# ginolhac/mapDamage

Hardware: AMD Instinct MI355X
Metric: reads/sec (misincorporation+comp tables) (higher is better)
Workload: dtype u8

## Files before the change

include/mdx.h:

```cpp
#ifndef MDX_H
#define MDX_H

#include <stdint.h>

#ifdef __cplusplus
extern "C" {
#endif

#define MDX_ABI_VERSION 6

#define MDX_OK 0
#define MDX_ERR_ARG (-1)
#define MDX_ERR_HIP (-2)
#define MDX_ERR_STATE (-3)
#define MDX_ERR_MASK_INDEX (-4)
#define MDX_ERR_LGD_OVERFLOW (-5)
#define MDX_ERR_BAD_READ (-6)

#define MDX_ERR_UNSUPPORTED (-8)
#define MDX_ERR_COMM (-7)

#define MDX_FLAG_QUAL_ABOVE_MIN 0x8000
#define MDX_FLAG_HAS_QUAL 0x4000

// ... 85 lines not shown
                           const int32_t *iv_start, const int32_t *iv_end, const int32_t *iv_group, int32_t rest_group);
int mdx_strata_groups(const mdx_ctx *ctx);
int mdx_strata_kept(mdx_ctx *ctx, uint64_t *kept);
int64_t mdx_merged_words(const mdx_ctx *ctx);
int mdx_finish_merged(mdx_ctx *ctx, const uint64_t *d_tables, uint64_t *d_merged);
int mdx_finish_merged_host(mdx_ctx *ctx, uint64_t *merged);
int mdx_lgd_copies(const mdx_ctx *ctx);

int mdx_reset(mdx_ctx *ctx);

int mdx_timing_enable(mdx_ctx *ctx, int enable);
int mdx_timing_read(mdx_ctx *ctx, int64_t *n_launches, double *total_ms);

int mdx_genome_composition(mdx_ctx *ctx, uint64_t *counts);

int mdx_rescale_set_model(mdx_ctx *ctx, const uint8_t *lut, const double *term, int32_t len5p, int32_t len3p);
int mdx_rescale_host(mdx_ctx *ctx, const mdx_batch *batch, const int32_t *mtid, const int32_t *mpos,
                     uint8_t *qual_out, double *mr_raw, uint8_t *status);
int mdx_rescale_device(mdx_ctx *ctx, const mdx_batch *dev_batch, const int32_t *d_mtid, const int32_t *d_mpos,
                       uint8_t *d_qual_out, double *d_mr_raw, uint8_t *d_status);
int mdx_tabulate_rescale_device(mdx_ctx *ctx, const mdx_batch *dev_batch, const int32_t *d_mtid, const int32_t *d_mpos,
                                uint8_t *d_qual_out, double *d_mr_raw, uint8_t *d_status);
int mdx_rescale_patches_device(mdx_ctx *ctx, const mdx_batch *dev_batch, const int32_t *d_mtid, const int32_t *d_mpos,
                               uint64_t *d_patch, int64_t patch_cap, int32_t n_parts, uint64_t *d_n_patch, double *d_mr_raw,
                               uint8_t *d_status);
int mdx_tabulate_rescale_patches_device(mdx_ctx *ctx, const mdx_batch *dev_batch, const int32_t *d_mtid, const int32_t *d_mpos,
                                        uint64_t *d_patch, int64_t patch_cap, int32_t n_parts, uint64_t *d_n_patch, double *d_mr_raw,
                                        uint8_t *d_status);
int mdx_rescale_expand_device(mdx_ctx *ctx, const mdx_batch *dev_batch, const uint64_t *d_patch, int64_t patch_cap, int32_t n_parts,
                              const uint64_t *d_n_patch, uint8_t *d_qual_out);
int mdx_rescale_timing_read(mdx_ctx *ctx, int64_t *n_launches, double *total_ms);
int64_t mdx_fused_launches(const mdx_ctx *ctx);
int64_t mdx_packed_launches(const mdx_ctx *ctx);
int64_t mdx_geo_spec_launches(const mdx_ctx *ctx);
int64_t mdx_libsorts(const mdx_ctx *ctx);
int mdx_last_launch_geometry(const mdx_ctx *ctx, int32_t out[4]);
int64_t mdx_rescale_summary_words(const mdx_ctx *ctx);
int mdx_rescale_summary(mdx_ctx *ctx, uint64_t *words);

typedef struct mdx_source mdx_source;
int mdx_source_open(const char *path, mdx_source **out);
const char *mdx_source_error(const mdx_source *source);
int mdx_source_is_stream(const mdx_source *source);
int mdx_source_peek(mdx_source *source, uint8_t *buf, int32_t n, int32_t *got);
int64_t mdx_source_read(mdx_source *source, uint8_t *buf, int64_t cap);
int mdx_source_seek(mdx_source *source, int64_t offset);
void mdx_source_close(mdx_source *source);

typedef struct mdx_bam mdx_bam;
int mdx_bam_read(const char *path, int threads, mdx_bam **out);
int mdx_bam_read_source(mdx_source *source, int threads, mdx_bam **out);
void mdx_bam_free(mdx_bam *bam);
const char *mdx_bam_error(const mdx_bam *bam);
const char *mdx_bam_header_text(const mdx_bam *bam);
int32_t mdx_bam_n_ref(const mdx_bam *bam);
const char *mdx_bam_ref_name(const mdx_bam *bam, int32_t i);
int64_t mdx_bam_ref_length(const mdx_bam *bam, int32_t i);
int mdx_bam_batch(const mdx_bam *bam, mdx_batch *view, const int32_t **mtid, const int32_t **mpos,
                  const int32_t **rg_index, const uint8_t **has_mr);
const uint8_t *mdx_bam_qmin(const mdx_bam *bam);

typedef struct mdx_record_filter {
    int32_t min_mapq;
    uint32_t require_flags, exclude_flags;
    int32_t min_length, max_length;
} mdx_record_filter;
// ... 99 lines not shown
```

mapdamage_amd/csrc/mdx_bamio.cpp:

```cpp
#include "../../include/mdx.h"
#ifndef MDX_HOST_ONLY
#include "mdx_internal.h"
#endif
#include "mdx_filter.h"
#include "mdx_crc32.h"

#include <fcntl.h>
#include <poll.h>
#include <sys/mman.h>
#include <sys/stat.h>
#include <unistd.h>
#include <zlib.h>

#include <algorithm>
#include <atomic>
#include <cerrno>
#include <chrono>
#include <condition_variable>
#include <functional>
#include <cstdlib>
#include <cstdio>
#include <cstring>
#include <mutex>
#include <string>
// ... 1363 lines not shown
    int pf_cur = -1;
    size_t pf_in0 = 0, pf_bytes = 0;
    void *d_crc_tables = nullptr;
    struct Buf { void *p = nullptr; size_t cap = 0; };
    struct Slab {
        bool ready = false;
        int64_t chunk_bytes = 0;
        size_t b0 = 0, b1 = 0, b2 = 0;
        size_t slab_bytes = 0, unc_bytes = 0, out0 = 0, in0 = 0, nh = 0, ahead = 0;
        size_t rec_cap = 0, cig_cap = 0, seq_cap = 0;
        bool more_file = false;
        std::vector<uint32_t> blk, crcs;
        int pf_used = -1;
        hipEvent_t ev_infl0 = nullptr, ev_infl = nullptr;
        double t_host = 0, frac_host = 0;
        bool timed = false;
        Buf comp, blk_d, crc, status, unc, cnt, pre, rec_off, flag, lib, tid, pos, tlen, mtid, mpos,
            cigar_off, cigar, seq_off, seq, qual, small, info, forced, arena;
    } slab[2];
    int cur = 0;
    int view_slab = 0;
    mdx_batch last_view{};
    const int32_t *last_mtid = nullptr, *last_mpos = nullptr;
    bool reserve(Buf &b, size_t bytes) {
        if (bytes <= b.cap) return true;
        if (b.p) (void)hipFree(b.p);
        b.p = nullptr; b.cap = 0;
        const size_t want = bytes + bytes / 8 + 256;
        if (hipMalloc(&b.p, want) != hipSuccess) { error = "out of device memory"; return false; }
        b.cap = want;
        return true;
    }
    bool drain() {
        bool ok = true;
        if (infl_stream) ok = hipStreamSynchronize(infl_stream) == hipSuccess && ok;
        if (copy_stream) ok = hipStreamSynchronize(copy_stream) == hipSuccess && ok;
        if (stream) ok = hipStreamSynchronize(stream) == hipSuccess && ok;
        return ok;
    }
};

int mdx_gbam_open_source(mdx_ctx *ctx, mdx_source *source, mdx_gbam **out) {
    try {
        if (!ctx || !source || !out) return MDX_ERR_ARG;
        mdx_gbam *g = new (std::nothrow) mdx_gbam();
        if (!g) return MDX_ERR_ARG;
        *out = g;
        g->ctx = ctx;
        void *st = nullptr;
        if (mdx_ctx_stream(ctx, &st, &g->device) != MDX_OK) { g->error = "no context"; return MDX_ERR_ARG; }
        g->stream = (hipStream_t)st;
        int rc = mdx_bam_open_source(source, 4, &g->hs);
        if (rc != MDX_OK) { g->error = g->hs ? g->hs->head.error : "cannot open"; return rc; }
        size_t k = 0;
        for (;;) {
            while (k < g->blocks.size() && g->blocks[k].out_off + g->blocks[k].out_size <= g->hs->header_bytes) k++;
            if (k < g->blocks.size() || g->whole_file_scanned()) break;
            if (!g->scan_to(g->scanned + ((size_t)1 << 20))) return MDX_ERR_ARG;
        }
        g->next_block = k;
        g->phase = k < g->blocks.size() ? g->hs->header_bytes - g->blocks[k].out_off : 0;
        g->host_share = g_host_share.load();
        if (const char *e = std::getenv("MDX_GBAM_HOST_SHARE")) {
            g->host_share = std::min(0.9, std::max(0.0, std::atof(e)));
            g->host_share_fixed = true;
        }
        if (const char *e = std::getenv("MDX_GBAM_NO_LOOKAHEAD")) g->no_ahead = *e && *e != '0';
// ... 38 lines not shown
            void *st = nullptr;
            (void)mdx_ctx_stream(ctx, &st, &g->device);
            g->stream = (hipStream_t)st;
            g->error = err;
            return MDX_ERR_ARG;
        }
        const int rc = mdx_gbam_open_source(ctx, file, out);
        mdx_source_close(file);
        return rc;
    } catch (const std::exception &e) {
        if (out && *out) (*out)->error = std::string("mdx_gbam_open: ") + e.what();
        return MDX_ERR_ARG;
    } catch (...) {
        return MDX_ERR_ARG;
    }
}

const mdx_bam *mdx_gbam_header(const mdx_gbam *g) { return (g && g->hs) ? &g->hs->head : nullptr; }
const char *mdx_gbam_error(const mdx_gbam *g) { return g ? g->error.c_str() : "null handle"; }

int mdx_gbam_configure(mdx_gbam *g, int32_t n_rg, const char *const *rg_ids, const int32_t *lib_of_rg, int32_t lib_default,
                       int want_qual, int want_mate) {
    try {
        if (!g || n_rg < 0 || (n_rg > 0 && (!rg_ids || !lib_of_rg))) return MDX_ERR_ARG;
        g->rg_names.clear(); g->rg_off.assign(1, 0); g->lib_of_rg.clear();
        for (int i = 0; i < n_rg; i++) {
            const size_t len = std::strlen(rg_ids[i]);
            g->rg_names.insert(g->rg_names.end(), (const uint8_t *)rg_ids[i], (const uint8_t *)rg_ids[i] + len);
            g->rg_off.push_back((uint32_t)g->rg_names.size());
            g->lib_of_rg.push_back(lib_of_rg[i]);
        }
        g->lib_default = lib_default;
        g->want_qual = want_qual != 0; g->want_mate = want_mate != 0;
        if (hipSetDevice(g->device) != hipSuccess) return MDX_ERR_HIP;
        g->d_rg_names = g->d_rg_off = g->d_lib_of_rg = nullptr;
        if (n_rg > 0) {
            const size_t b_off = g->rg_off.size() * 4, b_lib = g->lib_of_rg.size() * 4, b_nm = g->rg_names.size() + 1;
            const size_t need = b_off + b_lib + b_nm;
            if (g->d_rg && g->d_rg_cap < need) { rg_buffer_give(g->device, g->d_rg, g->d_rg_cap); g->d_rg = nullptr; g->d_rg_cap = 0; }
            if (!g->d_rg) g->d_rg = rg_buffer_take(g->device, need, g->d_rg_cap);
            if (!g->d_rg) { g->error = "out of device memory"; return MDX_ERR_HIP; }
            std::vector<uint8_t> img(need, 0);
            std::memcpy(img.data(), g->rg_off.data(), b_off);
            std::memcpy(img.data() + b_off, g->lib_of_rg.data(), b_lib);
            std::memcpy(img.data() + b_off + b_lib, g->rg_names.data(), g->rg_names.size());
            if (hipMemcpy(g->d_rg, img.data(), need, hipMemcpyHostToDevice) != hipSuccess) { g->error = "upload of the read-group tables failed"; return MDX_ERR_HIP; }
            g->d_rg_off = g->d_rg; g->d_lib_of_rg = (char *)g->d_rg + b_off; g->d_rg_names = (char *)g->d_rg + b_off + b_lib;
        }
        return MDX_OK;
    } catch (...) {
        return MDX_ERR_ARG;
    }
}

static size_t slab_want(const mdx_gbam *g, size_t b0, int64_t chunk_bytes) {
    size_t want = chunk_bytes < 65536 ? 65536 : (size_t)chunk_bytes;
    if (g->hs->file->is_stream()) return want;
    const size_t fsz = g->hs->file->size();
    const size_t in0 = b0 < g->blocks.size() ? (size_t)g->blocks[b0].in_off : g->scanned;
    if (fsz > in0) {
        const size_t rem = fsz - in0, n = (rem + want - 1) / want;
        if (n > 1) want = (rem + n - 1) / n;
        if (want < 65536) want = 65536;
    }
    return want;
}
static size_t slab_end_block(const mdx_gbam *g, size_t b0, size_t want, size_t *slab_bytes_out) {
// ... 419 lines not shown
    view->flag = c.flag; view->lib = c.lib; view->tid = c.tid; view->pos = c.pos; view->tlen = c.tlen;
    view->cigar_off = c.cigar_off; view->cigar = c.cigar; view->seq_off = c.seq_off; view->seq = c.seq; view->qual = c.qual;
    view->seq_format = c.fold ? MDX_SEQ_4BITQ : g->seq_format; view->reserved = 0; view->lowq = nullptr; view->libsort = nullptr;
    if (c.minqual > 0) {
        uint32_t counters[2] = {0, 0};
        if (hipMemcpyAsync(counters, d_counters, 8, hipMemcpyDeviceToHost, st) != hipSuccess || hipStreamSynchronize(st) != hipSuccess) return MDX_ERR_HIP;
        if (counters[0]) g->no_qual_seen = true;
        if (counters[1] == 0) { view->qual = nullptr; view->seq_format = g->seq_format; }
    }
    g->records_read += tot[0];
    if (d_mtid) *d_mtid = c.mtid;
    if (d_mpos) *d_mpos = c.mpos;
    g->last_view = *view; g->last_mtid = c.mtid; g->last_mpos = c.mpos;
    g->next_block = b1;
    g->phase = next_phase;
    g->phase_known = have;
    g->slabs_done++;
    g->view_reads = view->n_reads;
    s.ready = false;
    return MDX_OK;
}

int mdx_gbam_next(mdx_gbam *g, int64_t chunk_bytes, mdx_batch *view, const int32_t **d_mtid, const int32_t **d_mpos) {
    try {
        if (!g || !view) return MDX_ERR_ARG;
        std::memset(view, 0, sizeof(*view));
        if (d_mtid) *d_mtid = nullptr;
        if (d_mpos) *d_mpos = nullptr;
        if (!g->scan_to((g->next_block < g->blocks.size() ? g->blocks[g->next_block].in_off : g->scanned) + slab_want(g, g->next_block, chunk_bytes) + 65536)) return MDX_ERR_ARG;
        if (g->next_block >= g->blocks.size()) {
            if (g->phase_known && g->phase != 0) { g->error = "truncated BAM file: the last record is incomplete"; return MDX_ERR_ARG; }
            return MDX_OK;
        }
        if (hipSetDevice(g->device) != hipSuccess) return MDX_ERR_HIP;
        if (const char *fail = std::getenv("MDX_GBAM_FAIL_AT")) {
            if (g->slabs_done == std::atoi(fail)) { g->error = "MDX_GBAM_FAIL_AT"; return MDX_ERR_UNSUPPORTED; }
        }
        GbamLaps laps(g);
        GbamTrace tr;
        mdx_gbam::Slab &s = g->slab[g->cur], &n = g->slab[g->cur ^ 1];
        size_t ahead = (size_t)256 << 10;
        for (;;) {
            if (!(s.ready && s.b0 == g->next_block && s.chunk_bytes == chunk_bytes && s.ahead == ahead)) {
                const int rc = gbam_half_a(g, s, g->next_block, chunk_bytes, ahead, laps, tr);
                if (rc != MDX_OK) { (void)g->drain(); return rc; }
            }
            tr.mark("A");
            if (!g->no_ahead && !laps.on && s.b1 < g->blocks.size() && !(n.ready && n.b0 == s.b1 && n.chunk_bytes == chunk_bytes)) {
                const std::string keep = g->error;
                if (gbam_half_a(g, n, s.b1, chunk_bytes, (size_t)256 << 10, laps, tr) != MDX_OK) {
                    (void)g->drain();
                    n.ready = false; g->pf_cur = -1; g->error = keep;
                }
                tr.mark("A-next");
            }
            bool grow = false;
            const int rc = gbam_half_b(g, s, view, d_mtid, d_mpos, &grow, laps, tr);
            if (rc != MDX_OK) { (void)g->drain(); s.ready = n.ready = false; return rc; }
            if (!grow) break;
            if (!g->drain()) return MDX_ERR_HIP;
            s.ready = false;
            ahead *= 8;
        }
        g->view_slab = g->cur;
        g->cur ^= 1;
        mdx_source *src = g->hs->file;
        int64_t keep = 0, ph = 0;
// ... 81 lines not shown
            if (g->slab[0].ready || g->slab[1].ready) {
                (void)hipSetDevice(g->device);
                if (!g->drain()) return MDX_ERR_HIP;
                g->slab[0].ready = g->slab[1].ready = false;
            }
        }
        const size_t want = slab_want(g, g->next_block, chunk_bytes);
        if (!g->scan_to((g->next_block < g->blocks.size() ? g->blocks[g->next_block].in_off : g->scanned) + want + 65536)) return MDX_ERR_ARG;
        if (g->next_block >= g->blocks.size()) return MDX_OK;
        if (g->phase_known && !g->next_verified) {
            g->error = "the first record behind BGZF block " + std::to_string(g->next_block) + " cannot be found without the slab in front of it";
            return MDX_ERR_UNSUPPORTED;
        }
        const size_t b0 = g->next_block, in0 = g->blocks[b0].in_off;
        size_t b1 = b0, unc_bytes = 0;
        while (b1 < g->blocks.size() && (b1 == b0 || (g->blocks[b1].in_off - in0 < want && unc_bytes + g->blocks[b1].out_size < 0xE0000000ull))) {
            unc_bytes += g->blocks[b1].out_size;
            b1++;
        }
        g->next_block = b1;
        g->phase_known = false;
        g->phase = 0;
        return MDX_OK;
    } catch (...) {
        return MDX_ERR_ARG;
    }
}

int mdx_gbam_fixups(const mdx_gbam *g) { return g ? g->fixups : 0; }

int mdx_gbam_view_flags(mdx_gbam *g, uint16_t *flags, int64_t n) {
    if (!g || n < 0 || n != g->view_reads || (n > 0 && !flags)) return MDX_ERR_ARG;
    if (n == 0) return MDX_OK;
    if (hipSetDevice(g->device) != hipSuccess) return MDX_ERR_HIP;
    if (hipMemcpyAsync(flags, g->slab[g->view_slab].flag.p, (size_t)n * 2, hipMemcpyDeviceToHost, g->stream) != hipSuccess ||
        hipStreamSynchronize(g->stream) != hipSuccess) { g->error = "copy of the flag column failed"; return MDX_ERR_HIP; }
    return MDX_OK;
}

int mdx_gbam_view_set_flags(mdx_gbam *g, const uint16_t *flags, int64_t n) {
    if (!g || n < 0 || n != g->view_reads || (n > 0 && !flags)) return MDX_ERR_ARG;
    if (n == 0) return MDX_OK;
    if (hipSetDevice(g->device) != hipSuccess) return MDX_ERR_HIP;
    if (hipMemcpyAsync(g->slab[g->view_slab].flag.p, flags, (size_t)n * 2, hipMemcpyHostToDevice, g->stream) != hipSuccess ||
        hipStreamSynchronize(g->stream) != hipSuccess) { g->error = "copy of the flag column failed"; return MDX_ERR_HIP; }
    return MDX_OK;
}

int mdx_gbam_tell(const mdx_gbam *g, int64_t *comp_off, int64_t *phase) {
    if (!g || !comp_off || !phase || !g->hs) return MDX_ERR_ARG;
    if (!g->phase_known) return MDX_ERR_STATE;
    const size_t k = g->next_block;
    *comp_off = k >= g->blocks.size() ? (int64_t)g->scanned : (k == 0 ? 0 : (int64_t)(g->blocks[k - 1].in_off + g->blocks[k - 1].in_size + 8));
    *phase = (int64_t)g->phase;
    return MDX_OK;
}

int mdx_gbam_set_seq_format(mdx_gbam *g, int32_t seq_format) {
    if (!g || (seq_format != MDX_SEQ_ASCII && seq_format != MDX_SEQ_4BIT)) return MDX_ERR_ARG;
    g->seq_format = seq_format;
    return MDX_OK;
}

int mdx_gbam_missing_qualities(const mdx_gbam *g) { return (g && g->no_qual_seen) ? 1 : 0; }

int mdx_gbam_set_record_filter(mdx_gbam *g, const mdx_record_filter *filter) {
    if (!g) return MDX_ERR_ARG;
    if (!mdx_record_filter_valid(filter)) { g->error = "mdx_gbam_set_record_filter: a value out of range (MAPQ 0..255, flags 0..65535, lengths >= 0, min <= max)"; return MDX_ERR_ARG; }
    if (g->slabs_done > 0 || g->records_read > 0) { g->error = "mdx_gbam_set_record_filter: behind the first mdx_gbam_next"; return MDX_ERR_STATE; }
    const bool on = mdx_record_filter_active(filter);
    if (on && !g->d_filter_counts) {
        if (hipSetDevice(g->device) != hipSuccess || hipMalloc((void **)&g->d_filter_counts, 5 * sizeof(unsigned long long)) != hipSuccess ||
            hipMemset(g->d_filter_counts, 0, 5 * sizeof(unsigned long long)) != hipSuccess) {
            g->error = "mdx_gbam_set_record_filter: no device memory for the counts";
            return MDX_ERR_HIP;
        }
    }
    g->filter_on = on;
    g->filter = on ? *filter : mdx_record_filter{};
    return MDX_OK;
}

int mdx_gbam_filter_counts(const mdx_gbam *g, uint64_t out[6]) {
    if (!g || !out) return MDX_ERR_ARG;
    unsigned long long dropped[5] = {0, 0, 0, 0, 0};
    if (g->d_filter_counts) {
        if (hipSetDevice(g->device) != hipSuccess || hipStreamSynchronize(g->stream) != hipSuccess ||
            hipMemcpy(dropped, g->d_filter_counts, sizeof(dropped), hipMemcpyDeviceToHost) != hipSuccess) return MDX_ERR_HIP;
    }
    out[0] = g->records_read;
    for (int k = 0; k < 5; k++) out[1 + k] = dropped[k];
    return MDX_OK;
}

int mdx_gbam_at_end(const mdx_gbam *g) { return (!g || (g->next_block >= g->blocks.size() && g->whole_file_scanned())) ? 1 : 0; }

void mdx_gbam_close(mdx_gbam *g) {
    if (!g) return;
    const bool timing = std::getenv("MDX_BAM_TIMING") != nullptr;
    auto t_last = std::chrono::steady_clock::now();
    auto lap = [&](const char *what) {
        if (!timing) return;
        const auto now = std::chrono::steady_clock::now();
        std::fprintf(stderr, "mdx_gbam_close %-11s %.2f ms\n", what, std::chrono::duration<double, std::milli>(now - t_last).count());
        t_last = now;
    };
    (void)hipSetDevice(g->device);
    (void)g->drain();
    lap("sync");
    host_buffer_give(g->hbuf, g->hbuf_cap);
    for (auto &sl : g->slab) {
        if (sl.ev_infl0) (void)hipEventDestroy(sl.ev_infl0);
        if (sl.ev_infl) (void)hipEventDestroy(sl.ev_infl);
    }
    if (g->ev_free) (void)hipEventDestroy(g->ev_free);
    if (g->infl_stream) (void)hipStreamDestroy(g->infl_stream);
    pin_give(g->pin_bad);
    {
        const int big = g->slab[1].arena.cap > g->slab[0].arena.cap ? 1 : 0;
        mdx_ctx_scratch_give(g->ctx, g->slab[big].arena.p, g->slab[big].arena.cap, g->d_crc_tables, g->copy_stream, nullptr);
// ... 72 lines not shown
            }
            if (rc != MDX_OK) break;
            if (written + (int64_t)at > out_cap) { rc = MDX_ERR_ARG; break; }
            if (!ok(hipMemcpyAsync(B.d_off, offs.data(), (size_t)nb * 8, hipMemcpyHostToDevice, st))) break;
            mdx_k_bgzf_gather(src, bytes, B.d_slots, B.d_sizes, B.d_off, nb, B.d_tab, B.d_out, st);
            if (!ok(hipGetLastError()) || !ok(hipMemcpyAsync(out + written, B.d_out, (size_t)at, hipMemcpyDeviceToHost, st)) ||
                !ok(hipStreamSynchronize(st))) break;
            written += (int64_t)at;
        }
        if (rc == MDX_OK) *out_len = written;
    } catch (...) {
        rc = MDX_ERR_ARG;
    }
    return rc;
}

int mdx_bgzf_deflate(mdx_ctx *ctx, const uint8_t *data, int64_t n, uint8_t *out, int64_t out_cap, int64_t *out_len) {
    if (!ctx || n < 0 || (n > 0 && !data) || !out || !out_len) return MDX_ERR_ARG;
    void *st_ = nullptr;
    int device = 0;
    if (mdx_ctx_stream(ctx, &st_, &device) != MDX_OK) return MDX_ERR_ARG;
    return bgzf_deflate_impl((hipStream_t)st_, device, data, nullptr, n, out, out_cap, out_len);
}

int mdx_gbam_write_rescaled(mdx_gbam *g, const uint64_t *d_patch, int64_t patch_cap, int32_t n_parts, const uint64_t *d_n_patch,
                            const float *mr, const uint8_t *rescaled, uint8_t *out, int64_t out_cap, int64_t *out_len, int64_t *mr_clash) {
    if (!g || !out || !out_len || patch_cap < 0 || (n_parts > 0 && (!d_patch || !d_n_patch))) return MDX_ERR_ARG;
    *out_len = 0;
    if (mr_clash) *mr_clash = -1;
    const int64_t n = g->view_reads;
    if (n == 0) return MDX_OK;
    if (!mr || !rescaled) return MDX_ERR_ARG;
    try {
        if (hipSetDevice(g->device) != hipSuccess) return MDX_ERR_HIP;
        hipStream_t st = g->stream;
        mdx_gbam::Slab &s = g->slab[g->view_slab];
        uint8_t *d_resc = nullptr, *d_stream = nullptr;
        float *d_mr = nullptr;
        uint32_t *d_sizes = nullptr;
        unsigned long long *d_off = nullptr;
        int *d_clash = nullptr;
        int rc = MDX_OK;
        auto ok = [&](hipError_t e) { if (e != hipSuccess) { rc = MDX_ERR_HIP; g->error = std::string("write_rescaled: ") + hipGetErrorString(e); (void)hipGetLastError(); } return e == hipSuccess; };
        std::vector<uint32_t> sizes((size_t)n);
        std::vector<unsigned long long> offs((size_t)n);
        const int no_clash = 0x7FFFFFFF;
        int clash = no_clash;
        if (ok(hipMalloc((void **)&d_resc, (size_t)n)) && ok(hipMalloc((void **)&d_mr, (size_t)n * 4)) && ok(hipMalloc((void **)&d_sizes, (size_t)n * 4)) &&
            ok(hipMalloc((void **)&d_off, (size_t)n * 8)) && ok(hipMalloc((void **)&d_clash, 4)) &&
            ok(hipMemcpyAsync(d_resc, rescaled, (size_t)n, hipMemcpyHostToDevice, st)) && ok(hipMemcpyAsync(d_mr, mr, (size_t)n * 4, hipMemcpyHostToDevice, st)) &&
            ok(hipMemcpyAsync(d_clash, &no_clash, 4, hipMemcpyHostToDevice, st))) {
            if (n_parts > 0)
                mdx_k_gbam_patch_qual((uint8_t *)s.unc.p, (const uint32_t *)s.rec_off.p, (const uint32_t *)s.seq_off.p, (uint32_t)n,
                                      (const unsigned long long *)d_patch, (const unsigned long long *)d_n_patch, patch_cap, n_parts, st);
            mdx_k_gbam_out_sizes((const uint8_t *)s.unc.p, (const uint32_t *)s.rec_off.p, d_resc, (uint32_t)n, d_sizes, st);
            if (ok(hipGetLastError()) && ok(hipMemcpyAsync(sizes.data(), d_sizes, (size_t)n * 4, hipMemcpyDeviceToHost, st)) && ok(hipStreamSynchronize(st))) {
                unsigned long long total = 0;
                for (int64_t i = 0; i < n; i++) { offs[(size_t)i] = total; total += sizes[(size_t)i]; }
                if (ok(hipMalloc((void **)&d_stream, (size_t)total + 64)) && ok(hipMemcpyAsync(d_off, offs.data(), (size_t)n * 8, hipMemcpyHostToDevice, st))) {
                    mdx_k_gbam_write_back((const uint8_t *)s.unc.p, (const uint32_t *)s.rec_off.p, d_off, d_resc, d_mr, (uint32_t)n, d_stream, d_clash, st);
                    if (ok(hipGetLastError()) && ok(hipMemcpyAsync(&clash, d_clash, 4, hipMemcpyDeviceToHost, st)) && ok(hipStreamSynchronize(st))) {
                        if (clash != no_clash) {
                            if (mr_clash) *mr_clash = clash;
                            g->error = "record " + std::to_string(clash) + " of the slab is to be rescaled and has an MR tag already";
                            rc = MDX_ERR_BAD_READ;
                        } else {
                            rc = bgzf_deflate_impl(st, g->device, nullptr, d_stream, (int64_t)total, out, out_cap, out_len);
                            if (rc != MDX_OK) g->error = "the BGZF writer failed (output buffer too small?)";
                        }
                    }
                }
            }
        }
        for (void *p : {(void *)d_resc, (void *)d_mr, (void *)d_sizes, (void *)d_off, (void *)d_clash, (void *)d_stream}) if (p) (void)hipFree(p);
        return rc;
    } catch (const std::exception &e) {
        g->error = std::string("mdx_gbam_write_rescaled: ") + e.what();
        return MDX_ERR_ARG;
    }
}

int mdx_gbam_record_name(mdx_gbam *g, int64_t index, char *buf, int32_t cap) {
    if (!g || !buf || cap < 1 || index < 0 || index >= g->view_reads) return MDX_ERR_ARG;
    buf[0] = 0;
    if (hipSetDevice(g->device) != hipSuccess) return MDX_ERR_HIP;
    mdx_gbam::Slab &s = g->slab[g->view_slab];
    uint32_t off = 0;
    uint8_t head[12];
    if (hipMemcpy(&off, (const uint32_t *)s.rec_off.p + index, 4, hipMemcpyDeviceToHost) != hipSuccess ||
        hipMemcpy(head, (const uint8_t *)s.unc.p + off, 12, hipMemcpyDeviceToHost) != hipSuccess) return MDX_ERR_HIP;
    const int len = std::min<int>(head[8], cap - 1);
    if (len > 0 && hipMemcpy(buf, (const uint8_t *)s.unc.p + off + 32, (size_t)len, hipMemcpyDeviceToHost) != hipSuccess) return MDX_ERR_HIP;
    buf[len] = 0;
    return MDX_OK;
}

int mdx_gbam_rescale_slab(mdx_gbam *g, uint8_t *out, int64_t out_cap, int64_t *out_len, int64_t *counts, int64_t *mr_clash) {
    if (!g || !out || !out_len) return MDX_ERR_ARG;
    *out_len = 0;
    if (mr_clash) *mr_clash = -1;
    const int64_t n = g->view_reads;
    if (n == 0) return MDX_OK;
    const mdx_batch &v = g->last_view;
    if (!v.qual || !g->last_mtid || !g->last_mpos || v.seq_format != MDX_SEQ_ASCII) {
        g->error = "mdx_gbam_rescale_slab: the handle must be configured with qualities and mate columns, the seq column ASCII";
        return MDX_ERR_STATE;
    }
    try {
        if (hipSetDevice(g->device) != hipSuccess) return MDX_ERR_HIP;
        hipStream_t st = g->stream;
        const int parts = 256;
        const int64_t cap = std::max<int64_t>(4096, 8 * n / parts);
        uint64_t *d_patch = nullptr, *d_count = nullptr;
        double *d_mr = nullptr;
        uint8_t *d_status = nullptr;
        int rc = MDX_OK;
        auto ok = [&](hipError_t e) { if (e != hipSuccess) { rc = MDX_ERR_HIP; g->error = std::string("rescale_slab: ") + hipGetErrorString(e); (void)hipGetLastError(); } return e == hipSuccess; };
        std::vector<double> mr_raw((size_t)n);
        std::vector<uint8_t> status((size_t)n), rescaled((size_t)n);
        std::vector<float> mr((size_t)n);
        std::vector<uint64_t> cnt((size_t)parts);
        if (ok(hipMalloc((void **)&d_count, (size_t)parts * 8)) && ok(hipMalloc((void **)&d_mr, (size_t)n * 8)) && ok(hipMalloc((void **)&d_status, (size_t)n))) {
            if (ok(hipMalloc((void **)&d_patch, (size_t)parts * (size_t)cap * 8))) {
                rc = mdx_rescale_patches_device(g->ctx, &v, g->last_mtid, g->last_mpos, d_patch, cap, parts, d_count, d_mr, d_status);
                if (rc != MDX_OK) g->error = std::string("rescale kernels: ") + mdx_last_error(g->ctx);
                else if (ok(hipMemcpyAsync(cnt.data(), d_count, (size_t)parts * 8, hipMemcpyDeviceToHost, st)) && ok(hipStreamSynchronize(st))) {
                    uint64_t fullest = 0;
                    for (uint64_t c_ : cnt) fullest = std::max(fullest, c_);
                    if ((int64_t)fullest > cap) { g->error = "rescale_slab: more rescaled bytes than the list holds"; rc = MDX_ERR_ARG; }
                }
            }
        }
        if (rc == MDX_OK) {
            int64_t bad = -1;
            rc = mdx_sync(g->ctx, &bad);
            if (rc != MDX_OK) { g->error = std::string("rescale kernels: ") + mdx_last_error(g->ctx); if (mr_clash && rc == MDX_ERR_BAD_READ) *mr_clash = -2 - bad; }
        }
        if (rc == MDX_OK && ok(hipMemcpyAsync(mr_raw.data(), d_mr, (size_t)n * 8, hipMemcpyDeviceToHost, st)) &&
            ok(hipMemcpyAsync(status.data(), d_status, (size_t)n, hipMemcpyDeviceToHost, st)) && ok(hipStreamSynchronize(st))) {
            for (int64_t i = 0; i < n; i++) {
                const uint8_t stv = status[(size_t)i];
                rescaled[(size_t)i] = (stv == 2 || stv == 3) ? 1 : 0;
// ... 56 lines not shown
```

mapdamage_amd/csrc/mdx_capi.cpp:

```cpp
#include "../../include/mdx.h"
#include "mdx_internal.h"

#include <dlfcn.h>

#include <chrono>

#include <cstdio>
#include <cstdlib>
#include <cstring>
#include <mutex>
#include <new>
#include <string>
#include <thread>
#include <utility>
#include <vector>

namespace {

constexpr size_t kLdsLimit = MDX_LDS_LIMIT;
#ifdef MDX_WAVE_CLK
static unsigned long long *g_dbg_clk = nullptr;
extern "C" int mdx_dbg_clk_read(unsigned long long *out, int n) {
    if (!g_dbg_clk) return -1;
    (void)hipDeviceSynchronize();
    return (int)hipMemcpy(out, g_dbg_clk, (size_t)n * 24, hipMemcpyDeviceToHost);
}
extern "C" int mdx_dbg_phase_read(unsigned long long *out, int reset) {
    if (!g_dbg_clk) return -1;
    (void)hipDeviceSynchronize();
    std::vector<unsigned long long> h((size_t)16 * 8192);
    int rc = (int)hipMemcpy(h.data(), g_dbg_clk + 3 * 20000, h.size() * 8, hipMemcpyDeviceToHost);
    for (int q = 0; q < 16; q++) out[q] = 0;
    for (size_t w = 0; w < 8192; w++) for (int q = 0; q < 16; q++) out[q] += h[16 * w + q];
    if (reset) rc |= (int)hipMemset(g_dbg_clk + 3 * 20000, 0, h.size() * 8);
    return rc;
}
#endif
// ... 99 lines not shown
    MdxPkConfig pk = {512, 0};
    bool tile_ctr_clean = false;
    bool pkm_prepared = false;
    DevBuf lowq;
    DevBuf libsort;
    DevBuf libsort_scratch;
    const void *libsort_checked = nullptr;
    uint64_t libsort_checked_sig = 0;
    DevBuf ml_partials;
    int n_groups = 0;
    int32_t *d_group_of_tid = nullptr;
    unsigned long long *d_strata_kept = nullptr;
    int strata_n_contig = 0;
    void *d_regions = nullptr;
    MdxRegions regions = {};
    DevBuf strata_key;
    bool counted = false;
    int lgd_copies = MDX_LGD_COPIES;
    int64_t n_libsorts = 0;
    int64_t n_fused = 0;
    int64_t n_packed = 0;
    int64_t n_geo_spec = 0;
    int64_t fuse_list_cap = 0;
    int32_t last_geom[4] = {0, 0, 0, 0};
    void *pin[2] = {nullptr, nullptr};
    hipEvent_t pin_done[2] = {nullptr, nullptr};
    bool pin_busy[2] = {false, false};
    uint8_t *d_lut = nullptr;
    double *d_term = nullptr;
    unsigned long long *d_subs = nullptr;
    std::vector<uint8_t> h_lut;
    bool key0_plain = false;
    int len5p = 0, len3p = 0;
    bool timing = false;
    std::vector<std::pair<hipEvent_t, hipEvent_t>> events;
    std::vector<std::pair<hipEvent_t, hipEvent_t>> rs_events;
    std::string err;
};

namespace {

int fail(mdx_ctx *c, int code, const std::string &msg) {
    if (c) c->err = msg;
    return code;
}

#define RCCL_TRY(ctx, r, call)                                                                  \
    do {                                                                                        \
        int e_ = (call);                                                                        \
        if (e_ != 0)                                                                            \
            return fail((ctx), MDX_ERR_COMM, std::string(#call) + ": " + (r)->GetErrorString(e_)); \
    } while (0)

#define HIP_TRY(ctx, call)                                                                     \
    do {                                                                                       \
        hipError_t e_ = (call);                                                                \
        if (e_ != hipSuccess)                                                                  \
            return fail((ctx), MDX_ERR_HIP, std::string(#call) + ": " + hipGetErrorString(e_)); \
    } while (0)

int64_t lgd_words(const mdx_ctx *c) { return (int64_t)c->cfg.nlib * 4 * c->cfg.lgd_max; }
int64_t mis_words(const mdx_ctx *c) { return (int64_t)c->cfg.nlib * 4 * c->cfg.length * MDX_N_MIS_COLS; }
int64_t comp_words(const mdx_ctx *c) { return (int64_t)c->cfg.nlib * 4 * (c->cfg.length + c->cfg.around) * 4; }

int zero_accumulators(mdx_ctx *c) {
    HIP_TRY(c, hipMemsetAsync(c->d_raw, 0, (size_t)c->dims.w_total * 8, c->stream));
    HIP_TRY(c, hipMemsetAsync(c->d_lgd_dense, 0, (size_t)lgd_words(c) * 8 * c->lgd_copies, c->stream));
    HIP_TRY(c, hipMemsetAsync(c->d_n_lgd_over, 0, 8, c->stream));
    HIP_TRY(c, hipMemsetAsync(c->d_err, 0xFF, 8, c->stream));
    if (c->d_strata_kept) HIP_TRY(c, hipMemsetAsync(c->d_strata_kept, 0, (size_t)c->cfg.nlib * 8, c->stream));
    return MDX_OK;
}

}

extern "C" {

int mdx_abi_version(void) { return MDX_ABI_VERSION; }

int mdx_pack_seq(const uint8_t *ascii, int64_t n_bases, uint8_t *packed, int32_t threads) {
    if (n_bases < 0 || (n_bases > 0 && (!ascii || !packed))) return MDX_ERR_ARG;
    uint8_t lut[256];
    std::memset(lut, 0, sizeof lut);
    lut['A'] = 1; lut['C'] = 2; lut['T'] = 4; lut['G'] = 8;
    const int64_t nb = (n_bases + 1) / 2;
    int nt = threads > 0 ? threads : (int)std::thread::hardware_concurrency();
    if (nt < 1) nt = 1;
    if (nb < (int64_t)1 << 20) nt = 1;
    auto work = [&](int64_t lo, int64_t hi) {
        for (int64_t i = lo; i < hi; i++) {
            const uint8_t a = lut[ascii[2 * i]], b = 2 * i + 1 < n_bases ? lut[ascii[2 * i + 1]] : 0;
            packed[i] = (uint8_t)(a | (b << 4));
        }
    };
    if (nt == 1) { work(0, nb); return MDX_OK; }
    std::vector<std::thread> pool;
    for (int t = 0; t < nt; t++) pool.emplace_back(work, nb * t / nt, nb * (t + 1) / nt);
    for (auto &th : pool) th.join();
    return MDX_OK;
}

const char *mdx_strerror(int code) {
    switch (code) {
// ... 15 lines not shown
    if (cfg->length < 1 || cfg->around < 0 || cfg->minqual < 0 || cfg->minqual > 93 || cfg->nlib < 1 ||
        cfg->lgd_max < 1 || cfg->lgd_over_cap < 0)
        return MDX_ERR_ARG;
    mdx_ctx *c = new (std::nothrow) mdx_ctx();
    if (!c) return MDX_ERR_ARG;
    c->cfg = *cfg;
    const bool trace = getenv("MDX_INIT_TRACE") != nullptr;
    auto t_last = std::chrono::steady_clock::now();
    auto lap = [&](const char *what) {
        if (!trace) return;
        const auto now = std::chrono::steady_clock::now();
        std::fprintf(stderr, "mdx_create %-14s %.1f ms\n", what, std::chrono::duration<double, std::milli>(now - t_last).count());
        t_last = now;
    };
    int ndev = 0;
    if (hipGetDeviceCount(&ndev) != hipSuccess || ndev <= 0 || cfg->device < 0 || cfg->device >= ndev) {
        delete c;
        return MDX_ERR_HIP;
    }
    *out = c;
    if (cfg->nlib > 65535)
        return fail(c, MDX_ERR_ARG, "more than 65535 tables (libraries x reference groups): the 16-bit library column names "
                                    "no more, 0xFFFF being the record without a library");
    HIP_TRY(c, hipSetDevice(cfg->device));
    hipDeviceProp_t prop;
    HIP_TRY(c, hipGetDeviceProperties(&prop, cfg->device));
    c->n_cu = prop.multiProcessorCount > 0 ? prop.multiProcessorCount : 256;
    if (const char *e = getenv("MDX_TEST_CUS")) {
        const int n = atoi(e);
        if (n >= 1 && n < c->n_cu) c->n_cu = n;
    }
    HIP_TRY(c, hipStreamCreateWithFlags(&c->own_stream, hipStreamNonBlocking));
    c->stream = c->own_stream;
    lap("context, stream");

    const int lgd_lds = mdx_k_lgd_lds(cfg->length, cfg->around, cfg->lgd_max);
    if ((int64_t)cfg->nlib * (4LL * cfg->length * 29 + 8LL * (2LL * cfg->around + 512) +
                              4LL * lgd_lds + 128) > 0x7FFFFFF0LL || cfg->length > (1 << 24) || cfg->around > (1 << 24))
        return fail(c, MDX_ERR_ARG, "table too large (nlib * length)");
    c->dims = mdx_make_dims(cfg->length, cfg->around, cfg->nlib, cfg->lgd_max, lgd_lds);
    int group = cfg->nlib;
    while (group > 1 && mdx_k_lds_bytes(mdx_make_dims(cfg->length, cfg->around, group, cfg->lgd_max, lgd_lds)) > kLdsLimit)
        group--;
    const MdxDims gdims = mdx_make_dims(cfg->length, cfg->around, group, cfg->lgd_max, lgd_lds);
    c->lds_bytes = mdx_k_lds_bytes(gdims);
    if (c->lds_bytes <= kLdsLimit) {
        c->mode = MDX_MODE_LDS;
        c->lib_group = group;
        c->max_grid = c->n_cu * (2048 / mdx_k_block_threads());
        HIP_TRY(c, mdx_k_prepare(c->lds_bytes));
        {
            const MdxDims d1 = mdx_make_dims(cfg->length, cfg->around, 1, cfg->lgd_max, lgd_lds);
            c->pk = mdx_k_pk_config(d1, kLdsLimit);
            HIP_TRY(c, mdx_k_prepare_packed(mdx_k_pk_lds_bytes(d1, c->pk)));
            if (const char *e = getenv("MDX_DEBUG_PK")) if (*e && *e != '0')
                fprintf(stderr, "[mdx] packed kernels: blocks of %d threads, %zu bytes of LDS, columns %s\n", c->pk.threads, mdx_k_pk_lds_bytes(d1, c->pk),
                        c->pk.pfl ? "prefetched into the LDS" : "by plain loads");
        }
        lap("kernels");
        HIP_TRY(c, hipMalloc((void **)&c->d_partials, (size_t)c->max_grid * gdims.w_total * 4));
    } else {
        c->mode = MDX_MODE_GLOBAL;
        c->max_grid = c->n_cu * (2048 / mdx_k_block_threads());
    }
    HIP_TRY(c, hipMalloc((void **)&c->d_raw, (size_t)c->dims.w_total * 8));
    c->lgd_copies = mdx_lgd_copies_for(cfg->nlib, cfg->lgd_max);
    HIP_TRY(c, hipMalloc((void **)&c->d_lgd_dense, (size_t)lgd_words(c) * 8 * c->lgd_copies));
    HIP_TRY(c, hipMalloc((void **)&c->d_lgd_over, (size_t)(cfg->lgd_over_cap > 0 ? cfg->lgd_over_cap : 1) * 32));
    HIP_TRY(c, hipMalloc((void **)&c->d_n_lgd_over, 8));
    HIP_TRY(c, hipMalloc((void **)&c->d_err, 8));
    int rc = zero_accumulators(c);
    if (rc != MDX_OK) return rc;
    HIP_TRY(c, hipStreamSynchronize(c->stream));
    lap("accumulators");
    return MDX_OK;
}

void mdx_destroy(mdx_ctx *c) {
    if (!c) return;
    (void)hipSetDevice(c->cfg.device);
    if (c->stream) (void)hipStreamSynchronize(c->stream);
    if (c->comm && c->comm_owned && rccl()) (void)rccl()->CommDestroy(c->comm);
    for (auto &ev : c->events) { (void)hipEventDestroy(ev.first); (void)hipEventDestroy(ev.second); }
    for (auto &ev : c->rs_events) { (void)hipEventDestroy(ev.first); (void)hipEventDestroy(ev.second); }
    for (auto &set : c->st) for (auto &b : set) b.release();
    for (int i = 0; i < 2; i++) {
        if (c->st_copied[i]) (void)hipEventDestroy(c->st_copied[i]);
        if (c->st_done[i]) (void)hipEventDestroy(c->st_done[i]);
    }
    if (c->copy_stream) (void)hipStreamDestroy(c->copy_stream);
    if (c->gbam_arena) (void)hipFree(c->gbam_arena);
    if (c->gbam_tables) (void)hipFree(c->gbam_tables);
    if (c->gbam_stream) (void)hipStreamDestroy((hipStream_t)c->gbam_stream);
    if (c->gbam_event) (void)hipEventDestroy((hipEvent_t)c->gbam_event);
    c->lists.release();
    c->unpacked.release();
    c->lowq.release();
    c->libsort.release();
    c->libsort_scratch.release();
    c->strata_key.release();
    c->ml_partials.release();
    c->rs_part.release();
    c->rs_lists.release();
    c->rs_in.release();
    for (int i = 0; i < 2; i++) {
        if (c->pin[i]) (void)hipHostFree(c->pin[i]);
        if (c->pin_done[i]) (void)hipEventDestroy(c->pin_done[i]);
    }
    void *ptrs[] = {c->d_ref, c->d_ref4, c->d_contig_off, c->d_raw, c->d_lgd_dense, c->d_lgd_over,
                    c->d_n_lgd_over, c->d_err, c->d_partials, c->d_lut, c->d_term, c->d_subs, c->d_tile_ctr, c->d_group_of_tid, c->d_regions, c->d_strata_kept};
    for (void *p : ptrs) if (p) (void)hipFree(p);
    if (c->own_stream) (void)hipStreamDestroy(c->own_stream);
    delete c;
}

const char *mdx_last_error(const mdx_ctx *c) { return c ? c->err.c_str() : "null context"; }

int mdx_set_stream(mdx_ctx *c, void *hip_stream) {
    if (!c) return MDX_ERR_ARG;
    HIP_TRY(c, hipStreamSynchronize(c->stream));
    c->stream = hip_stream ? (hipStream_t)hip_stream : c->own_stream;
    return MDX_OK;
}

static const size_t kRefPad = 256;
static int ref_begin(mdx_ctx *c, int64_t n, int32_t n_contig) {
    HIP_TRY(c, hipSetDevice(c->cfg.device));
    HIP_TRY(c, hipStreamSynchronize(c->stream));
    if (c->d_ref) { (void)hipFree(c->d_ref); c->d_ref = nullptr; }
    if (c->d_ref4) { (void)hipFree(c->d_ref4); c->d_ref4 = nullptr; }
    if (c->d_contig_off) { (void)hipFree(c->d_contig_off); c->d_contig_off = nullptr; }
    c->n_contig = 0; c->ref_len = 0;
    HIP_TRY(c, hipMalloc((void **)&c->d_ref, (size_t)n + 2 * kRefPad + 1));
    HIP_TRY(c, hipMalloc((void **)&c->d_contig_off, (size_t)(n_contig + 1) * 8));
    HIP_TRY(c, hipMemsetAsync(c->d_ref, 0x85, (size_t)n + 2 * kRefPad + 1, c->stream));
    return MDX_OK;
}
static int ref_finish(mdx_ctx *c, const int64_t *contig_off, int32_t n_contig, int64_t n) {
    const size_t n4 = ((size_t)n + 2 * kRefPad + 1) / 2;
    static const bool no_ref2 = [] { const char *e = getenv("MDX_NO_REF2"); return e && *e && *e != '0'; }();
    const size_t kCopyB = ((size_t)1 << 31) + 64;
    static const size_t ref2_min = [] { const char *e = getenv("MDX_REF2_MIN"); return e && *e ? (size_t)strtoull(e, nullptr, 10) : (size_t)64 << 20; }();
    c->ref2 = n4 >= ref2_min && n4 + 128 <= ((size_t)1 << 31) - 64 && !no_ref2;
    hipError_t e = hipMemcpyAsync(c->d_contig_off, contig_off, (size_t)(n_contig + 1) * 8, hipMemcpyHostToDevice, c->stream);
    if (e == hipSuccess) {
        e = hipMalloc((void **)&c->d_ref4, (c->ref2 ? kCopyB : 0) + n4 + 64);
        if (e != hipSuccess && c->ref2) { (void)hipGetLastError(); c->ref2 = false; e = hipMalloc((void **)&c->d_ref4, n4 + 64); }
    }
    if (e == hipSuccess) e = hipMemsetAsync(c->d_ref4, 0, n4 + 64, c->stream);
    if (e == hipSuccess) { mdx_k_encode_ref4(c->d_ref, c->d_ref4, (int64_t)(2 * n4), c->stream); e = hipGetLastError(); }
    if (e == hipSuccess && c->ref2) e = hipMemcpyAsync(c->d_ref4 + kCopyB, c->d_ref4, n4 + 64, hipMemcpyDeviceToDevice, c->stream);
    if (e == hipSuccess) e = hipStreamSynchronize(c->stream);
    if (e != hipSuccess) {
        (void)hipFree(c->d_ref); c->d_ref = nullptr;
        return fail(c, MDX_ERR_HIP, std::string("set_reference: ") + hipGetErrorString(e));
    }
    c->n_contig = n_contig;
    c->ref_len = n;
    return MDX_OK;
}

int mdx_set_reference(mdx_ctx *c, const uint8_t *bases, const int64_t *contig_off, int32_t n_contig) {
    if (!c || !contig_off || n_contig < 1) return fail(c, MDX_ERR_ARG, "set_reference: bad arguments");
    for (int i = 0; i < n_contig; i++)
        if (contig_off[i + 1] < contig_off[i]) return fail(c, MDX_ERR_ARG, "contig_off not monotone");
    const int64_t n = contig_off[n_contig];
    if (contig_off[0] != 0 || (n > 0 && !bases)) return fail(c, MDX_ERR_ARG, "set_reference: bad arguments");
    int rc = ref_begin(c, n, n_contig);
    if (rc != MDX_OK) return rc;
    uint8_t *tmp = nullptr;
    HIP_TRY(c, hipMalloc((void **)&tmp, (size_t)n + 1));
    hipError_t e = n > 0 ? hipMemcpyAsync(tmp, bases, (size_t)n, hipMemcpyHostToDevice, c->stream) : hipSuccess;
    if (e == hipSuccess) { mdx_k_encode_ref(tmp, c->d_ref + kRefPad, n, c->stream); e = hipGetLastError(); }
    rc = e == hipSuccess ? ref_finish(c, contig_off, n_contig, n) : fail(c, MDX_ERR_HIP, std::string("set_reference: ") + hipGetErrorString(e));
    (void)hipStreamSynchronize(c->stream);
    (void)hipFree(tmp);
    return rc;
}

int mdx_set_reference_fasta(mdx_ctx *c, const char *fasta_path, int32_t n_contig, const char *const *names, int32_t missing_ok,
                            int64_t *lengths) {
    if (!c || !fasta_path || !names || n_contig < 1) return fail(c, MDX_ERR_ARG, "set_reference_fasta: bad arguments");
    try {
        HIP_TRY(c, hipSetDevice(c->cfg.device));
        struct Arg { mdx_ctx *c; int32_t n_contig; int rc; } arg{c, n_contig, MDX_OK};
        std::vector<int64_t> contig_off;
        std::string err;
        const int rc = mdx_fasta_to_device(fasta_path, n_contig, names, missing_ok, lengths, contig_off, err, c->stream,
            [](void *a_, int64_t n) -> uint8_t * {
                Arg *a = (Arg *)a_;
                a->rc = ref_begin(a->c, n, a->n_contig);
                return a->rc == MDX_OK ? a->c->d_ref + kRefPad : nullptr;
            }, &arg);
        if (arg.rc != MDX_OK) return arg.rc;
        if (rc != MDX_OK) {
            if (c->d_ref) { (void)hipFree(c->d_ref); c->d_ref = nullptr; }
            return fail(c, rc, "set_reference_fasta: " + err);
        }
        return ref_finish(c, contig_off.data(), n_contig, contig_off[(size_t)n_contig]);
    } catch (const std::exception &e) {
        return fail(c, MDX_ERR_ARG, std::string("set_reference_fasta: ") + e.what());
    }
}

int mdx_reference_fetch(mdx_ctx *c, int32_t tid, int64_t start, int64_t end, uint8_t *out) {
    if (!c || !out) return MDX_ERR_ARG;
    if (!c->d_ref) return fail(c, MDX_ERR_STATE, "mdx_set_reference has not been called");
    if (tid < 0 || tid >= c->n_contig || start < 0 || end < start) return fail(c, MDX_ERR_ARG, "reference_fetch: bad range");
    HIP_TRY(c, hipSetDevice(c->cfg.device));
    int64_t off[2];
    HIP_TRY(c, hipMemcpy(off, c->d_contig_off + tid, 16, hipMemcpyDeviceToHost));
    if (start + off[0] > off[1] || end + off[0] > off[1]) return fail(c, MDX_ERR_ARG, "reference_fetch: beyond the contig's end");
    if (end > start) HIP_TRY(c, hipMemcpy(out, c->d_ref + kRefPad + off[0] + start, (size_t)(end - start), hipMemcpyDeviceToHost));
    for (int64_t i = 0; i < end - start; i++) if (out[i] & 0x80) out[i] = out[i] == 0x84 ? '-' : 'N';
    return MDX_OK;
}

// ... 33 lines not shown
}
static int strata_view(mdx_ctx *c, const mdx_batch *b, mdx_batch *out, bool count) {
    *out = *b;
    if (c->n_groups <= 0 || b->n_reads == 0) return MDX_OK;
    HIP_TRY(c, c->strata_key.reserve((size_t)b->n_reads * 2 + 64));
    if (c->d_regions)
        mdx_k_strata_region_key(b->n_reads, b->flag, b->lib, b->tid, b->pos, b->cigar_off, b->cigar, b->n_cigar, c->regions, c->n_groups,
                                c->cfg.nlib / c->n_groups, (uint16_t *)c->strata_key.p, count ? c->d_strata_kept : nullptr, c->stream);
    else
        mdx_k_strata_key(b->n_reads, b->flag, b->lib, b->tid, c->d_group_of_tid, c->strata_n_contig, c->n_groups, c->cfg.nlib / c->n_groups,
                         (uint16_t *)c->strata_key.p, count ? c->d_strata_kept : nullptr, c->stream);
    HIP_TRY(c, hipGetLastError());
    out->lib = (const uint16_t *)c->strata_key.p;
    return MDX_OK;
}

static int build_libsort(mdx_ctx *c, const mdx_batch *b, void *blob) {
    MdxLibSort ls;
    mdx_k_libsort_layout(blob, b->n_reads, b->n_cigar, b->n_bases, c->cfg.nlib, &ls);
    const uint64_t sig = libsort_signature(b->n_reads, b->n_cigar, b->n_bases, c->cfg.nlib, c->n_groups);
    HIP_TRY(c, hipMemcpyAsync((char *)blob + 8, &sig, 8, hipMemcpyHostToDevice, c->stream));
    HIP_TRY(c, c->libsort_scratch.reserve(mdx_k_libsort_scratch_bytes(b->n_reads, c->cfg.nlib)));
    mdx_k_libsort(b->n_reads, b->n_cigar, b->n_bases, b->flag, b->lib, b->tid, b->pos, b->tlen, b->cigar_off, b->cigar, b->seq_off, b->seq,
                  c->cfg.nlib, c->libsort_scratch.p, ls, c->stream);
    HIP_TRY(c, hipGetLastError());
    return MDX_OK;
}

int mdx_batch_upload(mdx_ctx *c, const mdx_batch *h, mdx_batch *dv) {
    int rc = check_batch(c, h);
    if (rc != MDX_OK) return rc;
    if (!dv) return MDX_ERR_ARG;
    HIP_TRY(c, hipSetDevice(c->cfg.device));
    std::memset(dv, 0, sizeof(*dv));
    dv->n_reads = h->n_reads; dv->n_cigar = h->n_cigar; dv->n_bases = h->n_bases;
    dv->seq_format = h->seq_format;
    const int64_t n = h->n_reads;
    struct Col { const void *src; const void **dst; size_t bytes; } cols[] = {
        {h->flag, (const void **)&dv->flag, (size_t)n * 2},
        {h->lib, (const void **)&dv->lib, (size_t)n * 2},
        {h->tid, (const void **)&dv->tid, (size_t)n * 4},
        {h->pos, (const void **)&dv->pos, (size_t)n * 4},
        {h->tlen, (const void **)&dv->tlen, (size_t)n * 4},
        {h->cigar_off, (const void **)&dv->cigar_off, (size_t)(n + 1) * 4},
        {h->cigar, (const void **)&dv->cigar, (size_t)h->n_cigar * 4},
        {h->seq_off, (const void **)&dv->seq_off, (size_t)(n + 1) * 4},
        {h->seq, (const void **)&dv->seq, seq_bytes(h)},
        {h->qual, (const void **)&dv->qual, h->qual ? (size_t)h->n_bases : 0},
    };
    for (auto &col : cols) {
        if (!col.src || n == 0) continue;
        void *p = nullptr;
        HIP_TRY(c, hipMalloc(&p, col.bytes + 64));
        *col.dst = p;
        HIP_TRY(c, hipMemcpyAsync(p, col.src, col.bytes, hipMemcpyHostToDevice, c->stream));
    }
    if (dv->qual && n > 0) {
        mdx_k_mark_has_qual(const_cast<uint16_t *>(dv->flag), dv->seq_off, dv->qual, n, c->stream);
        HIP_TRY(c, hipGetLastError());
    }
    static const bool no_batch_lowq = [] { const char *e = getenv("MDX_NO_BATCH_LOWQ"); return e && *e && *e != '0'; }();
    if (c->cfg.minqual > 0 && dv->qual && h->seq_format == MDX_SEQ_4BIT && h->n_bases > 0 && c->mode == MDX_MODE_LDS && !no_batch_lowq) {
        mdx_k_fold_mask(dv->seq, const_cast<uint8_t *>(dv->seq), dv->qual, nullptr, h->n_bases, c->cfg.minqual, c->stream);
        HIP_TRY(c, hipGetLastError());
        dv->seq_format = MDX_SEQ_4BITQ;
    }
    static const bool no_batch_sort = [] { const char *e = getenv("MDX_NO_BATCH_LIBSORT"); return e && *e && *e != '0'; }();
    if (c->cfg.nlib > 1 && h->seq_format != MDX_SEQ_ASCII && n > 0 && c->mode == MDX_MODE_LDS && !no_batch_sort) {
        void *p = nullptr;
        HIP_TRY(c, hipMalloc(&p, mdx_k_libsort_bytes(n, h->n_cigar, h->n_bases, c->cfg.nlib)));
        dv->libsort = (const uint8_t *)p;
        mdx_batch keyed;
        rc = strata_view(c, dv, &keyed, false);
        if (rc != MDX_OK) return rc;
        rc = build_libsort(c, &keyed, p);
        if (rc != MDX_OK) return rc;
    }
    HIP_TRY(c, hipStreamSynchronize(c->stream));
    return MDX_OK;
}

int mdx_batch_fold(mdx_ctx *c, mdx_batch *b) {
    int rc = check_batch(c, b);
    if (rc != MDX_OK) return rc;
    if (c->cfg.minqual <= 0) return fail(c, MDX_ERR_STATE, "mdx_batch_fold: the context has no --min-basequal");
    if (b->seq_format == MDX_SEQ_4BITQ) return MDX_OK;
    if (b->seq_format != MDX_SEQ_4BIT) return fail(c, MDX_ERR_ARG, "mdx_batch_fold: the seq column is not MDX_SEQ_4BIT");
    if (!b->qual && !b->lowq) return fail(c, MDX_ERR_ARG, "mdx_batch_fold: neither qualities nor a bitmap of the low ones");
    if (b->libsort) return fail(c, MDX_ERR_ARG, "mdx_batch_fold: the batch brings mdx_batch::libsort, built from the column as it was");
    if (b->n_bases == 0) { b->seq_format = MDX_SEQ_4BITQ; return MDX_OK; }
    HIP_TRY(c, hipSetDevice(c->cfg.device));
    mdx_k_fold_mask(b->seq, const_cast<uint8_t *>(b->seq), b->qual, b->lowq, b->n_bases, c->cfg.minqual, c->stream);
    HIP_TRY(c, hipGetLastError());
    b->seq_format = MDX_SEQ_4BITQ;
    return MDX_OK;
}

int mdx_batch_free(mdx_ctx *c, mdx_batch *dv) {
    if (!c || !dv) return MDX_ERR_ARG;
    HIP_TRY(c, hipStreamSynchronize(c->stream));
    if (dv->libsort && dv->libsort == c->libsort_checked) c->libsort_checked = nullptr;
    const void *ptrs[] = {dv->flag, dv->lib, dv->tid, dv->pos, dv->tlen, dv->cigar_off,
                          dv->cigar, dv->seq_off, dv->seq, dv->qual, dv->lowq, dv->libsort};
    for (const void *p : ptrs) if (p) (void)hipFree(const_cast<void *>(p));
    std::memset(dv, 0, sizeof(*dv));
    return MDX_OK;
}

static int tabulate_impl(mdx_ctx *c, const mdx_batch *b_in, const MdxFuse *fuse, int *fused_grid) {
    int rc = check_batch(c, b_in);
    if (rc != MDX_OK) return rc;
    if (!c->d_ref) return fail(c, MDX_ERR_STATE, "mdx_set_reference has not been called");
    if (b_in->n_reads == 0) return MDX_OK;
    HIP_TRY(c, hipSetDevice(c->cfg.device));
    const bool force_ref64 = [] { const char *e = getenv("MDX_FORCE_REF64"); return e && *e && *e != '0'; }();
    const bool ref32 = c->ref_len + 1024 < (int64_t)0xFFFFFFFFLL && !force_ref64;
    static const bool no_packed = [] { const char *e = getenv("MDX_NO_PACKED"); return e && *e && *e != '0'; }();
    static const bool no_pkm = [] { const char *e = getenv("MDX_NO_PACKED_MASK"); return e && *e && *e != '0'; }();
    const bool folded = b_in->seq_format == MDX_SEQ_4BITQ;
    const bool want_mask = c->cfg.minqual > 0 && (b_in->qual != nullptr || folded);
    const bool packed = b_in->seq_format != MDX_SEQ_ASCII && c->mode == MDX_MODE_LDS && c->dims.fast_ok() && ref32 &&
                        (fuse ? (c->cfg.nlib == 1 && !folded) : !(want_mask && no_pkm)) && !no_packed;
    const bool pmask = packed && !fuse && want_mask;
    static const bool no_ml = [] { const char *e = getenv("MDX_NO_ML"); return e && *e && *e != '0'; }();
    const bool ml = packed && !fuse && c->cfg.nlib > 1 && !no_ml;
    mdx_batch b_key;
    if (c->n_groups > 0) {
        if (fuse) return fail(c, MDX_ERR_ARG, "the fused tabulate-and-rescale calls count one library: not on a context with mdx_set_strata");
        if (c->strata_n_contig != c->n_contig)
            return fail(c, MDX_ERR_ARG, std::string(c->d_regions ? "mdx_set_strata_regions" : "mdx_set_strata") + " named " + std::to_string(c->strata_n_contig) + " sequences, the reference has " +
                                        std::to_string(c->n_contig));
        if (!(ml && b_in->libsort)) {
            rc = strata_view(c, b_in, &b_key, true);
            if (rc != MDX_OK) return rc;
            b_in = &b_key;
        }
    }
    c->counted = true;
    mdx_batch b_ascii;
    const mdx_batch *b = b_in;
    if (!packed) {
        rc = ascii_view(c, b_in, &b_ascii);
        if (rc != MDX_OK) return rc;
        b = &b_ascii;
    }
    MdxTabArgs a{};
    a.ref4 = c->d_ref4;
    a.ref2 = c->ref2 ? 1 : 0;
    a.seq_packed = packed ? 1 : 0;
    a.n_reads = b->n_reads;
    a.flag = b->flag; a.lib = b->lib; a.tid = b->tid; a.pos = b->pos; a.tlen = b->tlen;
    a.cigar_off = b->cigar_off; a.cigar = b->cigar; a.seq_off = b->seq_off; a.seq = b->seq; a.qual = b->qual;
    a.ref = c->d_ref + 256;
    a.contig_off = c->d_contig_off;
    a.n_contig = c->n_contig;
    a.minqual = c->cfg.minqual;
    a.dims = c->dims;
    a.partials = c->d_partials;
// ... 1 lines not shown
    a.lgd_dense = c->d_lgd_dense;
    a.lgd_copies = c->lgd_copies;
    a.lgd_over = c->d_lgd_over;
    a.lgd_over_cap = c->cfg.lgd_over_cap;
    a.n_lgd_over = c->d_n_lgd_over;
    a.err = c->d_err;
    a.record_base = c->record_base;
#ifdef MDX_WAVE_CLK
    if (!g_dbg_clk) {
        (void)hipMalloc((void **)&g_dbg_clk, 3 * 8 * 20000 + 16 * 8 * 8192);
        (void)hipMemset(g_dbg_clk, 0, 3 * 8 * 20000 + 16 * 8 * 8192);
    }
    a.dbg_clk = g_dbg_clk;
#endif
    a.stage_off = mdx_k_stage_off(c->dims);
    a.queue_off = mdx_k_queue_off(c->dims);
    a.n_bases = b->n_bases;
    a.ref32 = ref32 ? 1 : 0;
    const bool mask = c->cfg.minqual > 0 && b->qual != nullptr;
    const int wpb = (packed ? c->pk.threads : mdx_k_block_threads()) / 64;
    const int64_t ntiles = (b->n_reads + 63) / 64;
    const int64_t want = (ntiles + wpb - 1) / wpb;
    if (b->n_reads >= (int64_t)1 << 30) return fail(c, MDX_ERR_ARG, "batch of 2^30 records or more; split it");
    a.nlib_total = c->cfg.nlib;
    int group = packed ? 1 : (c->mode == MDX_MODE_LDS ? c->lib_group : c->cfg.nlib);
    const MdxDims dims1 = mdx_make_dims(c->cfg.length, c->cfg.around, 1, c->cfg.lgd_max, c->dims.lgd_lds);
    if (ml) {
        group = c->cfg.nlib < MDX_ML_MAX_LIBS ? c->cfg.nlib : MDX_ML_MAX_LIBS;
        int per_cu = (int)(kLdsLimit / mdx_k_pk_lds_bytes(dims1, c->pk));
        if (per_cu > mdx_k_pk_blocks_per_cu(c->pk.threads)) per_cu = mdx_k_pk_blocks_per_cu(c->pk.threads);
        const int pools = (c->n_cu * per_cu) / 2;
        if (group > pools) group = pools > 0 ? pools : 1;
    }
    for (int lo = 0; lo < c->cfg.nlib; lo += group) {
        const int gn = c->cfg.nlib - lo < group ? c->cfg.nlib - lo : group;
        a.lib_lo = lo;
        a.n_libs = ml ? gn : 0;
        size_t lds = 0;
        int max_grid = c->max_grid;
        if (c->mode == MDX_MODE_LDS) {
            a.dims = ml ? dims1 : (gn == c->cfg.nlib ? c->dims : mdx_make_dims(c->cfg.length, c->cfg.around, gn, c->cfg.lgd_max, c->dims.lgd_lds));
            a.raw = c->d_raw + (size_t)lo * c->dims.w_lib;
            a.lgd_dense = c->d_lgd_dense + (size_t)lo * 4 * c->cfg.lgd_max;
            lds = packed ? mdx_k_pk_lds_bytes(a.dims, c->pk) : mdx_k_lds_bytes(a.dims);
            int per_cu = (int)(kLdsLimit / lds);
            const int by_threads = packed ? mdx_k_pk_blocks_per_cu(c->pk.threads) : 2048 / mdx_k_block_threads();
            if (per_cu > by_threads) per_cu = by_threads;
            max_grid = c->n_cu * per_cu;
        }
        a.stage_off = mdx_k_stage_off(a.dims);
        a.queue_off = packed ? mdx_k_pk_queue_off(a.dims, c->pk.threads) : mdx_k_queue_off(a.dims);
        a.pfl_off = packed && !fuse && c->pk.pfl ? mdx_k_pk_pfl_off(a.dims, c->pk.threads) : 0;
        int grid = (int)(want < max_grid ? want : max_grid);
        if (ml && grid < 2 * gn) grid = 2 * gn < max_grid ? 2 * gn : max_grid;
        if (ml && (grid & 1)) grid += grid + 1 <= max_grid ? 1 : -1;
        int wpb_l = wpb;
        if (fuse) {
            const int npos = 1 + fuse->len5p + fuse->len3p;
            a.rs = *fuse;
            a.queue_off = mdx_k_fuse_queue_off(a.dims);
            if (packed) {
                a.rs.qcap = MDX_PK_QCAP;
                a.rs.tcb_off = mdx_k_pkf_tcb_off(a.dims);
                lds = mdx_k_pkf_lds_bytes(a.dims, npos);
            } else {
                a.rs.qcap = mdx_k_fuse_qcap(a.dims, npos, kLdsLimit);
                a.rs.tcb_off = mdx_k_fuse_tcb_off(a.dims, a.rs.qcap);
                lds = mdx_k_fuse_lds_bytes(a.dims, npos, a.rs.qcap);
            }
            wpb_l = mdx_k_fuse_block_threads() / 64;
            const int64_t want_f = (ntiles + wpb_l - 1) / wpb_l;
            grid = (int)(want_f < c->n_cu ? want_f : c->n_cu);
            size_t &prepared = packed ? c->pkf_prepared : c->fuse_prepared;
            if (!prepared || prepared < lds) {
                HIP_TRY(c, packed ? mdx_k_pkf_prepare(lds) : mdx_k_fuse_prepare(lds));
                prepared = lds;
            }
        }
        {
            const int64_t nwaves = (int64_t)grid * wpb_l;
            const int64_t T = mdx_tile_records(a.dims, a.pfl_off != 0);
            const int64_t n_tiles = (b->n_reads + T - 1) / T;
            const int64_t n_pools = mdx_n_pools((unsigned)grid);
            const int64_t chunk = MDX_POOL_CHUNK;
            const int64_t pool_tiles = ((n_tiles + n_pools * chunk - 1) / (n_pools * chunk)) * chunk, pool_waves = (grid / n_pools) * wpb_l;
            const bool quota = fuse || (pmask && !ml);
            a.tile_quota = quota ? (int)(2 * ((pool_tiles + pool_waves - 1) / pool_waves) + 2) : 0x7FFFFFFF;
            a.list_cap = fuse ? (int64_t)a.tile_quota * T + 128 : 0;
            a.round_tiles = MDX_ROUND_TILES;
            a.ring_size = MDX_LIST_RING;
            if (quota) while ((int64_t)a.ring_size < (int64_t)a.tile_quota * T + 128) a.ring_size *= 2;
            if (!c->d_tile_ctr) {
                HIP_TRY(c, hipMalloc((void **)&c->d_tile_ctr, (size_t)MDX_CTR_WORDS * 4));
                HIP_TRY(c, hipMemsetAsync(c->d_tile_ctr, 0, (size_t)MDX_CTR_WORDS * 4, c->stream));
            }
            if (n_pools * MDX_CTR_PAD > MDX_CTR_WORDS / 2 || n_pools * MDX_CTR_PAD > MDX_CTR_WORDS) return fail(c, MDX_ERR_STATE, "more blocks than tile counters");
            a.tile_ctr = c->d_tile_ctr;
            {
                const size_t list_bytes = (size_t)nwaves * (size_t)MDX_WAVE_SCRATCH(a.ring_size) * 16;
                if (c->lists.reserve(list_bytes) != hipSuccess)
                    return fail(c, MDX_ERR_HIP, "the per-wavefront lists of this launch (" + std::to_string(list_bytes >> 20) + " MiB) could not be allocated" +
                                (quota ? ": tabulate the batch in smaller pieces" : ""));
            }
            a.lists = (uint4 *)c->lists.p;
            c->last_geom[0] = grid; c->last_geom[1] = wpb_l; c->last_geom[2] = (int32_t)n_tiles; c->last_geom[3] = (int32_t)n_pools;
        }
        hipEvent_t e0 = nullptr, e1 = nullptr;
        if (c->timing) {
            HIP_TRY(c, hipEventCreate(&e0));
            HIP_TRY(c, hipEventCreate(&e1));
            HIP_TRY(c, hipEventRecord(e0, c->stream));
        }
        mdx_batch b_fold;
        const mdx_batch *bs = b;
        if (pmask && !folded) {
            if (lo == 0) {
                HIP_TRY(c, c->lowq.reserve(((size_t)b->n_bases + 1) / 2 + 64));
                const bool bits = b->lowq != nullptr;
                if (b->libsort) return fail(c, MDX_ERR_ARG, "mdx_batch::libsort of a MDX_SEQ_4BIT batch under --min-basequal: upload the batch with the context it is tabulated with");
                mdx_k_fold_mask(b->seq, (uint8_t *)c->lowq.p, b->qual, bits ? b->lowq : nullptr, b->n_bases, c->cfg.minqual, c->stream);
                HIP_TRY(c, hipGetLastError());
            }
            a.seq = (const uint8_t *)c->lowq.p;
            b_fold = *b;
            b_fold.seq = a.seq;
            bs = &b_fold;
        }
        if (pmask && !c->pkm_prepared) {
            HIP_TRY(c, mdx_k_prepare_packed_masked(mdx_k_pk_lds_bytes(dims1, c->pk)));
            c->pkm_prepared = true;
        }
        if (ml) {
            const void *blob = b->libsort;
            if (blob) {
                if (blob != c->libsort_checked) {
                    uint64_t sig = 0;
                    HIP_TRY(c, hipMemcpyAsync(&sig, (const char *)blob + 8, 8, hipMemcpyDeviceToHost, c->stream));
                    HIP_TRY(c, hipStreamSynchronize(c->stream));
                    c->libsort_checked = blob;
                    c->libsort_checked_sig = sig;
                }
                if (c->libsort_checked_sig != libsort_signature(b->n_reads, b->n_cigar, b->n_bases, c->cfg.nlib, c->n_groups))
                    return fail(c, MDX_ERR_ARG, "mdx_batch::libsort was built for another batch or a context with another number of libraries: "
                                                "upload the batch with the context that tabulates it, whole");
            }
            if (!blob) {
                if (lo == 0) {
                    HIP_TRY(c, c->libsort.reserve(mdx_k_libsort_bytes(b->n_reads, b->n_cigar, b->n_bases, c->cfg.nlib)));
                    rc = build_libsort(c, bs, c->libsort.p);
                    if (rc != MDX_OK) return rc;
                    c->n_libsorts++;
                }
                blob = c->libsort.p;
            }
            MdxLibSort ls;
            mdx_k_libsort_layout(const_cast<void *>(blob), b->n_reads, b->n_cigar, b->n_bases, c->cfg.nlib, &ls);
            if (c->n_groups > 0 && b->libsort && lo == 0) mdx_k_strata_kept_from_sort(ls.lib_start, c->cfg.nlib, c->d_strata_kept, c->stream);
            a.flag = ls.flag; a.tid = ls.tid; a.pos = ls.pos; a.tlen = ls.tlen;
            a.cigar_off = ls.cigar_off; a.cigar = ls.cigar; a.seq_off = ls.seq_off; a.seq = ls.seq;
            a.perm = ls.perm; a.lib_start = ls.lib_start; a.sort_bad = ls.bad;
            HIP_TRY(c, c->ml_partials.reserve((size_t)mdx_n_pools((unsigned)grid) * 16));
            a.ml_plan = (const uint4 *)c->ml_partials.p;
            mdx_k_ml_plan(ls.lib_start, lo, gn, mdx_tile_records(a.dims, a.pfl_off != 0), grid, c->ml_partials.p, c->stream);
        }
        const size_t n_ctr = (size_t)mdx_n_pools((unsigned)grid);
        if (!c->tile_ctr_clean || n_ctr > 4096) HIP_TRY(c, hipMemsetAsync(c->d_tile_ctr, 0, n_ctr * MDX_CTR_PAD * 4, c->stream));
        c->tile_ctr_clean = false;
        if (fuse) {
            HIP_TRY(c, hipMemsetAsync(fuse->mr_raw, 0xFF, (size_t)b->n_reads * 8, c->stream));
            const int64_t nwaves = (int64_t)grid * wpb_l;
            HIP_TRY(c, c->rs_in.reserve((size_t)nwaves * (size_t)(a.list_cap + 1) * 4));
            a.rs.gen_count = (uint32_t *)c->rs_in.p;
            a.rs.gen_list = a.rs.gen_count + nwaves;
            if (packed) { mdx_k_tabulate_packed_fused(a, grid, lds, c->stream); c->n_packed++; }
            else mdx_k_tabulate_fused(a, grid, lds, c->stream);
            c->fuse_list_cap = a.list_cap;
            if (fused_grid) *fused_grid = grid;
        } else if (packed) {
            if (pmask) mdx_k_tabulate_packed_masked(a, grid, c->pk.threads, lds, c->stream);
            else if (mdx_k_tabulate_packed(a, grid, c->pk.threads, lds, c->stream)) c->n_geo_spec++;
            c->n_packed++;
        } else {
            mdx_k_tabulate(a, c->mode, mask, grid, lds, c->stream);
        }
        if (c->timing) {
            HIP_TRY(c, hipEventRecord(e1, c->stream));
            c->events.emplace_back(e0, e1);
        }
        HIP_TRY(c, hipGetLastError());
        if (c->mode == MDX_MODE_LDS) {
            if (ml) mdx_k_reduce_partials(c->d_partials, a.raw, c->d_raw + c->dims.w_total - 1, a.dims.w_total, grid, c->stream, c->d_tile_ctr, gn, c->dims.w_lib, a.ml_plan);
            else
            mdx_k_reduce_partials(c->d_partials, a.raw, c->d_raw + c->dims.w_total - 1, a.dims.w_total, grid, c->stream, c->d_tile_ctr);
            c->tile_ctr_clean = a.dims.w_total >= 4096 && n_ctr <= 4096;
            HIP_TRY(c, hipGetLastError());
        }
    }
    return MDX_OK;
}

int mdx_tabulate_device(mdx_ctx *c, const mdx_batch *b) { return tabulate_impl(c, b, nullptr, nullptr); }

int mdx_tabulate_host(mdx_ctx *c, const mdx_batch *h) {
    int rc = check_batch(c, h);
    if (rc != MDX_OK) return rc;
    if (h->n_reads == 0) return MDX_OK;
    HIP_TRY(c, hipSetDevice(c->cfg.device));
    const int64_t n = h->n_reads;
    const void *src[10] = {h->flag, h->lib, h->tid, h->pos, h->tlen, h->cigar_off, h->cigar, h->seq_off, h->seq, h->qual};
    const size_t bytes[10] = {(size_t)n * 2, (size_t)n * 2, (size_t)n * 4, (size_t)n * 4, (size_t)n * 4,
                              (size_t)(n + 1) * 4, (size_t)h->n_cigar * 4, (size_t)(n + 1) * 4,
                              seq_bytes(h), h->qual ? (size_t)h->n_bases : 0};
    constexpr size_t PIN_BYTES = (size_t)16 << 20;
    if (!c->copy_stream) HIP_TRY(c, hipStreamCreateWithFlags(&c->copy_stream, hipStreamNonBlocking));
    for (int i = 0; i < 2; i++) {
        if (!c->pin[i]) HIP_TRY(c, hipHostMalloc(&c->pin[i], PIN_BYTES, hipHostMallocDefault));
        if (!c->pin_done[i]) HIP_TRY(c, hipEventCreateWithFlags(&c->pin_done[i], hipEventDisableTiming));
        if (!c->st_copied[i]) HIP_TRY(c, hipEventCreateWithFlags(&c->st_copied[i], hipEventDisableTiming));
        if (!c->st_done[i]) HIP_TRY(c, hipEventCreateWithFlags(&c->st_done[i], hipEventDisableTiming));
    }
    const int s = c->st_turn;
    DevBuf *const st = c->st[s];
    const bool stage_fold = c->cfg.minqual > 0 && h->qual && h->seq_format == MDX_SEQ_4BIT && h->n_bases > 0 && c->mode == MDX_MODE_LDS;
    bool grow = false;
    for (int i = 0; i < 10; i++) grow = grow || (src[i] && bytes[i] + 64 > st[i].cap);
    if (c->st_busy[s]) {
        if (grow) HIP_TRY(c, hipEventSynchronize(c->st_done[s]));
        else HIP_TRY(c, hipStreamWaitEvent(c->copy_stream, c->st_done[s], 0));
    }
    int turn = 0;
    for (int i = 0; i < 10; i++) {
        if (!src[i] || bytes[i] == 0) continue;
        HIP_TRY(c, st[i].reserve(bytes[i] + 64));
        for (size_t off = 0; off < bytes[i]; off += PIN_BYTES) {
            const size_t len = bytes[i] - off < PIN_BYTES ? bytes[i] - off : PIN_BYTES;
            if (c->pin_busy[turn]) HIP_TRY(c, hipEventSynchronize(c->pin_done[turn]));
            std::memcpy(c->pin[turn], (const uint8_t *)src[i] + off, len);
            HIP_TRY(c, hipMemcpyAsync((uint8_t *)st[i].p + off, c->pin[turn], len, hipMemcpyHostToDevice, c->copy_stream));
            HIP_TRY(c, hipEventRecord(c->pin_done[turn], c->copy_stream));
            c->pin_busy[turn] = true;
            turn ^= 1;
        }
    }
    if (stage_fold) {
        mdx_k_fold_mask((const uint8_t *)st[8].p, (uint8_t *)st[8].p, (const uint8_t *)st[9].p, nullptr, h->n_bases, c->cfg.minqual, c->copy_stream);
        HIP_TRY(c, hipGetLastError());
    }
    HIP_TRY(c, hipEventRecord(c->st_copied[s], c->copy_stream));
    HIP_TRY(c, hipStreamWaitEvent(c->stream, c->st_copied[s], 0));
    mdx_batch dv = *h;
    dv.lowq = nullptr;
    dv.libsort = nullptr;
    if (stage_fold) dv.seq_format = MDX_SEQ_4BITQ;
    dv.flag = (const uint16_t *)st[0].p; dv.lib = (const uint16_t *)st[1].p;
    dv.tid = (const int32_t *)st[2].p; dv.pos = (const int32_t *)st[3].p;
    dv.tlen = (const int32_t *)st[4].p; dv.cigar_off = (const uint32_t *)st[5].p;
    dv.cigar = (const uint32_t *)st[6].p; dv.seq_off = (const uint32_t *)st[7].p;
    dv.seq = (const uint8_t *)st[8].p; dv.qual = h->qual ? (const uint8_t *)st[9].p : nullptr;
    rc = mdx_tabulate_device(c, &dv);
    HIP_TRY(c, hipEventRecord(c->st_done[s], c->stream));
    c->st_busy[s] = true;
    c->st_turn = s ^ 1;
    return rc;
}

int mdx_set_record_base(mdx_ctx *c, int64_t base) {
    if (!c || base < 0) return MDX_ERR_ARG;
    c->record_base = base;
    return MDX_OK;
}

int mdx_sync(mdx_ctx *c, int64_t *bad_read) {
    if (!c) return MDX_ERR_ARG;
    HIP_TRY(c, hipSetDevice(c->cfg.device));
    HIP_TRY(c, hipStreamSynchronize(c->stream));
    unsigned long long err = 0, nover = 0;
    HIP_TRY(c, hipMemcpy(&err, c->d_err, 8, hipMemcpyDeviceToHost));
    HIP_TRY(c, hipMemcpy(&nover, c->d_n_lgd_over, 8, hipMemcpyDeviceToHost));
    if (err != ~0ull) {
        if (bad_read) *bad_read = (int64_t)(err >> 8);
        const int code = -(int)(err & 0xFF);
        char msg[160];
        std::snprintf(msg, sizeof msg, "record %lld (index within its batch + the record base): %s", (long long)(err >> 8), mdx_strerror(code));
        return fail(c, code, msg);
    }
    if ((int64_t)nover > c->cfg.lgd_over_cap) return fail(c, MDX_ERR_LGD_OVERFLOW, mdx_strerror(MDX_ERR_LGD_OVERFLOW));
    return MDX_OK;
}

int64_t mdx_table_words(const mdx_ctx *c) {
    if (!c) return 0;
    return mis_words(c) + comp_words(c) + lgd_words(c) + 2;
}

int mdx_finish_device(mdx_ctx *c, uint64_t *d_tables) {
    if (!c || !d_tables) return MDX_ERR_ARG;
    HIP_TRY(c, hipSetDevice(c->cfg.device));
    mdx_k_finalize(c->d_raw, c->d_lgd_dense, c->d_n_lgd_over, c->dims, c->lgd_copies, (unsigned long long *)d_tables, c->stream);
    HIP_TRY(c, hipGetLastError());
    return MDX_OK;
}

int mdx_comm_unique_id(uint8_t *id) {
    if (!id) return MDX_ERR_ARG;
    const Rccl *r = rccl();
    if (!r) return MDX_ERR_COMM;
    RcclId u;
    if (r->GetUniqueId(&u) != 0) return MDX_ERR_COMM;
    std::memcpy(id, u.internal, MDX_COMM_ID_BYTES);
    return MDX_OK;
}

int mdx_comm_init(mdx_ctx *c, const uint8_t *id, int32_t nranks, int32_t rank) {
    if (!c || !id || nranks < 1 || rank < 0 || rank >= nranks) return fail(c, MDX_ERR_ARG, "comm_init: bad arguments");
    if (c->comm) return fail(c, MDX_ERR_STATE, "a communicator is already attached");
    const Rccl *r = rccl();
    if (!r) return fail(c, MDX_ERR_COMM, g_rccl.err);
    HIP_TRY(c, hipSetDevice(c->cfg.device));
    RcclId u;
    std::memcpy(u.internal, id, MDX_COMM_ID_BYTES);
    void *comm = nullptr;
    RCCL_TRY(c, r, r->CommInitRank(&comm, nranks, u, rank));
    c->comm = comm; c->comm_owned = true; c->comm_size = nranks; c->comm_rank = rank;
    return MDX_OK;
}

int mdx_comm_adopt(mdx_ctx *c, void *rccl_comm, int32_t nranks, int32_t rank) {
    if (!c || !rccl_comm || nranks < 1 || rank < 0 || rank >= nranks) return fail(c, MDX_ERR_ARG, "comm_adopt: bad arguments");
    if (c->comm) return fail(c, MDX_ERR_STATE, "a communicator is already attached");
    if (!rccl()) return fail(c, MDX_ERR_COMM, g_rccl.err);
    c->comm = rccl_comm; c->comm_owned = false; c->comm_size = nranks; c->comm_rank = rank;
    return MDX_OK;
}

int mdx_comm_size(const mdx_ctx *c) { return c && c->comm ? c->comm_size : 0; }

int mdx_comm_count(mdx_ctx *c) {
    if (!c) return MDX_ERR_ARG;
    if (!c->comm) return 0;
    const Rccl *r = rccl();
    if (!r) return fail(c, MDX_ERR_COMM, g_rccl.err);
    int n = 0;
    RCCL_TRY(c, r, r->CommCount(c->comm, &n));
    return n;
}

int mdx_finish_allreduce(mdx_ctx *c, uint64_t *d_tables) {
    if (!c || !d_tables) return MDX_ERR_ARG;
    if (!c->comm) return fail(c, MDX_ERR_STATE, "mdx_comm_init / mdx_comm_adopt first");
    const Rccl *r = rccl();
    int rc = mdx_finish_device(c, d_tables);
    if (rc != MDX_OK) return rc;
    RCCL_TRY(c, r, r->AllReduce(d_tables, d_tables, (size_t)mdx_table_words(c), kNcclUint64, kNcclSum, c->comm, c->stream));
    return MDX_OK;
}

int mdx_finish(mdx_ctx *c, uint64_t *mis, uint64_t *comp, uint64_t *lgd, int64_t *lgd_over,
               int64_t lgd_over_cap, int64_t *n_lgd_over, int64_t *n_kept) {
    if (!c) return MDX_ERR_ARG;
    int rc = mdx_sync(c, nullptr);
    const Rccl *r = c->comm ? rccl() : nullptr;
    const int64_t words = mdx_table_words(c);
    uint64_t *d = nullptr;
// ... 60 lines not shown
        if (e == hipSuccess && lgd) e = hipMemcpy(lgd, d + nm + nc, (size_t)nl * 8, hipMemcpyDeviceToHost);
        uint64_t tail[2] = {0, 0};
        if (e == hipSuccess) e = hipMemcpy(tail, d + nm + nc + nl, 16, hipMemcpyDeviceToHost);
        if (e == hipSuccess) {
            if (n_kept) *n_kept = (int64_t)tail[0];
            int64_t nov = (int64_t)tail[1];
            if (n_lgd_over) *n_lgd_over = nov;
            if (lgd_over && nov > 0) {
                if (r) {
                    nov = (int64_t)gathered.size() / 4;
                    if (nov > lgd_over_cap) {
                        if (n_lgd_over) *n_lgd_over = nov;
                        (void)hipFree(d);
                        return fail(c, MDX_ERR_LGD_OVERFLOW, "the out-of-range fragment lengths of all ranks exceed the "
                                    "caller's lgd_over buffer (give it comm_size x lgd_over_cap entries)");
                    }
                    if (n_lgd_over) *n_lgd_over = nov;
                    std::memcpy(lgd_over, gathered.data(), (size_t)nov * 32);
                } else {
                    if (nov > lgd_over_cap) nov = lgd_over_cap;
                    e = hipMemcpy(lgd_over, c->d_lgd_over, (size_t)nov * 32, hipMemcpyDeviceToHost);
                }
            }
        }
        if (e != hipSuccess) rc = fail(c, MDX_ERR_HIP, hipGetErrorString(e));
    }
    (void)hipFree(d);
    return rc;
}

int mdx_reset(mdx_ctx *c) {
    if (!c) return MDX_ERR_ARG;
    HIP_TRY(c, hipSetDevice(c->cfg.device));
    int rc = zero_accumulators(c);
    if (rc != MDX_OK) return rc;
    HIP_TRY(c, hipStreamSynchronize(c->stream));
    c->err.clear();
    c->counted = false;
    return MDX_OK;
}

int mdx_set_strata(mdx_ctx *c, int32_t n_groups, const int32_t *group_of_tid, int32_t n_contig) {
    if (!c) return MDX_ERR_ARG;
    if (n_groups < 1 || n_contig < 1 || !group_of_tid) return fail(c, MDX_ERR_ARG, "set_strata: bad arguments");
    if (c->cfg.nlib % n_groups != 0)
        return fail(c, MDX_ERR_ARG, "set_strata: the context's " + std::to_string(c->cfg.nlib) + " tables are no multiple of " +
                                    std::to_string(n_groups) + " groups (create it with nlib = libraries x groups)");
    for (int32_t t = 0; t < n_contig; t++)
        if (group_of_tid[t] < 0 || group_of_tid[t] >= n_groups)
            return fail(c, MDX_ERR_ARG, "set_strata: the group of sequence " + std::to_string(t) + " is outside [0, n_groups)");
    if (c->counted) return fail(c, MDX_ERR_STATE, "set_strata: records have been counted already (mdx_reset first)");
    if (c->d_regions) return fail(c, MDX_ERR_STATE, "set_strata: the context has region strata (mdx_set_strata_regions); a context has one kind");
    HIP_TRY(c, hipSetDevice(c->cfg.device));
    HIP_TRY(c, hipStreamSynchronize(c->stream));
    if (c->d_group_of_tid) { (void)hipFree(c->d_group_of_tid); c->d_group_of_tid = nullptr; }
    c->n_groups = 0;
    HIP_TRY(c, hipMalloc((void **)&c->d_group_of_tid, (size_t)n_contig * 4));
    HIP_TRY(c, hipMemcpy(c->d_group_of_tid, group_of_tid, (size_t)n_contig * 4, hipMemcpyHostToDevice));
    if (!c->d_strata_kept) {
        HIP_TRY(c, hipMalloc((void **)&c->d_strata_kept, (size_t)c->cfg.nlib * 8));
        HIP_TRY(c, hipMemset(c->d_strata_kept, 0, (size_t)c->cfg.nlib * 8));
    }
    c->n_groups = n_groups;
    c->strata_n_contig = n_contig;
    return MDX_OK;
}

int mdx_set_strata_regions(mdx_ctx *c, int32_t n_groups, int32_t n_contig, const int64_t *iv_off, const int32_t *iv_start,
                           const int32_t *iv_end, const int32_t *iv_group, int32_t rest_group) {
    if (!c) return MDX_ERR_ARG;
    if (n_groups < 1 || n_contig < 1 || !iv_off) return fail(c, MDX_ERR_ARG, "set_strata_regions: bad arguments");
    if (c->cfg.nlib % n_groups != 0)
        return fail(c, MDX_ERR_ARG, "set_strata_regions: the context's " + std::to_string(c->cfg.nlib) + " tables are no multiple of " +
                                    std::to_string(n_groups) + " groups (create it with nlib = libraries x groups)");
    if (rest_group < 0 || rest_group >= n_groups) return fail(c, MDX_ERR_ARG, "set_strata_regions: rest_group is outside [0, n_groups)");
    if (iv_off[0] != 0) return fail(c, MDX_ERR_ARG, "set_strata_regions: iv_off[0] is not 0");
    for (int32_t t = 0; t < n_contig; t++)
        if (iv_off[t + 1] < iv_off[t])
            return fail(c, MDX_ERR_ARG, "set_strata_regions: the offsets decrease at sequence " + std::to_string(t));
    const int64_t n_iv = iv_off[n_contig];
    if (n_iv > 0 && (!iv_start || !iv_end || !iv_group)) return fail(c, MDX_ERR_ARG, "set_strata_regions: bad arguments");
    for (int32_t t = 0; t < n_contig; t++)
        for (int64_t k = iv_off[t]; k < iv_off[t + 1]; k++) {
            const std::string which = "set_strata_regions: interval " + std::to_string(k) + " (sequence " + std::to_string(t) + ", [" +
                                      std::to_string(iv_start[k]) + ", " + std::to_string(iv_end[k]) + ")) ";
            if (iv_start[k] < 0 || iv_start[k] >= iv_end[k]) return fail(c, MDX_ERR_ARG, which + "is not 0 <= start < end");
            if (k > iv_off[t] && iv_end[k - 1] > iv_start[k])
                return fail(c, MDX_ERR_ARG, which + "begins before interval " + std::to_string(k - 1) + " ends: not sorted and disjoint");
            if (iv_group[k] < 0 || iv_group[k] >= n_groups)
                return fail(c, MDX_ERR_ARG, which + "has group " + std::to_string(iv_group[k]) + ", outside [0, n_groups)");
        }
    if (c->counted) return fail(c, MDX_ERR_STATE, "set_strata_regions: records have been counted already (mdx_reset first)");
    if (c->d_group_of_tid) return fail(c, MDX_ERR_STATE, "set_strata_regions: the context has tid strata (mdx_set_strata); a context has one kind");
    HIP_TRY(c, hipSetDevice(c->cfg.device));
    HIP_TRY(c, hipStreamSynchronize(c->stream));
    if (c->d_regions) { (void)hipFree(c->d_regions); c->d_regions = nullptr; }
    c->n_groups = 0;
    const size_t off_bytes = ((size_t)(n_contig + 1) * 8 + 15) & ~(size_t)15, col_bytes = ((size_t)n_iv * 4 + 15) & ~(size_t)15;
    HIP_TRY(c, hipMalloc(&c->d_regions, off_bytes + 3 * col_bytes + 64));
    char *p = (char *)c->d_regions;
    HIP_TRY(c, hipMemcpy(p, iv_off, (size_t)(n_contig + 1) * 8, hipMemcpyHostToDevice));
    const int32_t *cols[3] = {iv_start, iv_end, iv_group};
    for (int k = 0; k < 3 && n_iv > 0; k++)
        HIP_TRY(c, hipMemcpy(p + off_bytes + k * col_bytes, cols[k], (size_t)n_iv * 4, hipMemcpyHostToDevice));
    c->regions.iv_off = (const int64_t *)p;
    c->regions.iv_start = (const int32_t *)(p + off_bytes);
    c->regions.iv_end = (const int32_t *)(p + off_bytes + col_bytes);
    c->regions.iv_group = (const int32_t *)(p + off_bytes + 2 * col_bytes);
    c->regions.rest_group = rest_group;
    c->regions.n_contig = n_contig;
    if (!c->d_strata_kept) {
        HIP_TRY(c, hipMalloc((void **)&c->d_strata_kept, (size_t)c->cfg.nlib * 8));
        HIP_TRY(c, hipMemset(c->d_strata_kept, 0, (size_t)c->cfg.nlib * 8));
    }
    c->n_groups = n_groups;
    c->strata_n_contig = n_contig;
    return MDX_OK;
}

int mdx_strata_groups(const mdx_ctx *c) { return c ? c->n_groups : 0; }

int mdx_strata_kept(mdx_ctx *c, uint64_t *kept) {
    if (!c || !kept) return MDX_ERR_ARG;
    if (c->n_groups <= 0) return fail(c, MDX_ERR_STATE, "strata_kept: mdx_set_strata has not been called");
    HIP_TRY(c, hipSetDevice(c->cfg.device));
    HIP_TRY(c, hipStreamSynchronize(c->stream));
    HIP_TRY(c, hipMemcpy(kept, c->d_strata_kept, (size_t)c->cfg.nlib * 8, hipMemcpyDeviceToHost));
    return MDX_OK;
}
int mdx_lgd_copies(const mdx_ctx *c) { return c ? c->lgd_copies : 0; }

int64_t mdx_merged_words(const mdx_ctx *c) {
    if (!c) return 0;
    const int64_t g = c->n_groups > 0 ? c->n_groups : 1;
    return (mis_words(c) + comp_words(c) + lgd_words(c)) / g + 2;
}

int mdx_finish_merged_host(mdx_ctx *c, uint64_t *merged) {
    if (!c || !merged) return MDX_ERR_ARG;
    int rc = mdx_sync(c, nullptr);
    if (rc != MDX_OK) return rc;
    const int64_t words = mdx_table_words(c), m_words = mdx_merged_words(c);
    uint64_t *d = nullptr;
    HIP_TRY(c, hipMalloc((void **)&d, (size_t)(words + m_words) * 8));
    rc = mdx_finish_device(c, d);
    if (rc == MDX_OK) rc = mdx_finish_merged(c, d, d + words);
    if (rc == MDX_OK) {
        hipError_t e = hipStreamSynchronize(c->stream);
        if (e == hipSuccess) e = hipMemcpy(merged, d + words, (size_t)m_words * 8, hipMemcpyDeviceToHost);
        if (e != hipSuccess) rc = fail(c, MDX_ERR_HIP, hipGetErrorString(e));
    }
    (void)hipFree(d);
    return rc;
}

int mdx_finish_merged(mdx_ctx *c, const uint64_t *d_tables, uint64_t *d_merged) {
    if (!c || !d_tables || !d_merged) return MDX_ERR_ARG;
    if (d_tables == d_merged) return fail(c, MDX_ERR_ARG, "finish_merged: the merged block needs a buffer of its own");
    HIP_TRY(c, hipSetDevice(c->cfg.device));
    const int g = c->n_groups > 0 ? c->n_groups : 1;
    mdx_k_merge_strata((const unsigned long long *)d_tables, (unsigned long long *)d_merged, c->cfg.nlib / g, g,
                       (int64_t)4 * c->cfg.length * MDX_N_MIS_COLS, (int64_t)4 * (c->cfg.length + c->cfg.around) * 4,
                       (int64_t)4 * c->cfg.lgd_max, c->stream);
    HIP_TRY(c, hipGetLastError());
    return MDX_OK;
}

int mdx_timing_enable(mdx_ctx *c, int enable) {
    if (!c) return MDX_ERR_ARG;
    c->timing = enable != 0;
    return MDX_OK;
}

int mdx_timing_read(mdx_ctx *c, int64_t *n_launches, double *total_ms) {
    if (!c) return MDX_ERR_ARG;
    HIP_TRY(c, hipStreamSynchronize(c->stream));
    double tot = 0;
    int64_t n = 0;
    for (auto &ev : c->events) {
        float ms = 0;
        if (hipEventElapsedTime(&ms, ev.first, ev.second) == hipSuccess) { tot += ms; n++; }
        (void)hipEventDestroy(ev.first);
        (void)hipEventDestroy(ev.second);
    }
    c->events.clear();
    if (n_launches) *n_launches = n;
    if (total_ms) *total_ms = tot;
    return MDX_OK;
}

int mdx_table_mode(const mdx_ctx *c) { return c ? c->mode : -1; }

void mdx_ctx_scratch_give(mdx_ctx *c, void *arena, size_t cap, void *tables, void *stream, void *event) {
    if (!c) {
        if (arena) (void)hipFree(arena);
        if (tables) (void)hipFree(tables);
        if (stream) (void)hipStreamDestroy((hipStream_t)stream);
        if (event) (void)hipEventDestroy((hipEvent_t)event);
        return;
    }
    if (arena) {
        if (c->gbam_arena && c->gbam_arena_cap >= cap) (void)hipFree(arena);
        else { if (c->gbam_arena) (void)hipFree(c->gbam_arena); c->gbam_arena = arena; c->gbam_arena_cap = cap; }
    }
    if (tables) { if (c->gbam_tables) (void)hipFree(tables); else c->gbam_tables = tables; }
    if (stream) { if (c->gbam_stream) (void)hipStreamDestroy((hipStream_t)stream); else c->gbam_stream = stream; }
    if (event) { if (c->gbam_event) (void)hipEventDestroy((hipEvent_t)event); else c->gbam_event = event; }
}
void mdx_ctx_scratch_take(mdx_ctx *c, void **arena, size_t *cap, void **tables, void **stream, void **event) {
    *arena = nullptr; *cap = 0; *tables = nullptr; *stream = nullptr; *event = nullptr;
    if (!c) return;
    *arena = c->gbam_arena; *cap = c->gbam_arena_cap; *tables = c->gbam_tables; *stream = c->gbam_stream; *event = c->gbam_event;
    c->gbam_arena = nullptr; c->gbam_arena_cap = 0; c->gbam_tables = nullptr; c->gbam_stream = nullptr; c->gbam_event = nullptr;
}

int mdx_ctx_minqual(const mdx_ctx *c) { return c ? c->cfg.minqual : -1; }

int mdx_ctx_stream(mdx_ctx *c, void **stream, int *device) {
    if (!c) return MDX_ERR_ARG;
    if (stream) *stream = (void *)c->stream;
    if (device) *device = c->cfg.device;
    return MDX_OK;
}

int mdx_rescale_set_model(mdx_ctx *c, const uint8_t *lut, const double *term, int32_t len5p, int32_t len3p) {
    if (!c || !lut || !term || len5p < 0 || len3p < 0 || len5p + len3p > 100000) return fail(c, MDX_ERR_ARG, "rescale model");
    HIP_TRY(c, hipSetDevice(c->cfg.device));
    HIP_TRY(c, hipStreamSynchronize(c->stream));
    if (c->d_lut) { (void)hipFree(c->d_lut); c->d_lut = nullptr; }
    if (c->d_term) { (void)hipFree(c->d_term); c->d_term = nullptr; }
    if (c->d_subs) { (void)hipFree(c->d_subs); c->d_subs = nullptr; }
    const size_t npos = (size_t)1 + len5p + len3p;
    HIP_TRY(c, hipMalloc((void **)&c->d_lut, 2 * npos * 94));
    HIP_TRY(c, hipMalloc((void **)&c->d_term, 2 * npos * 8));
    HIP_TRY(c, hipMemcpy(c->d_lut, lut, 2 * npos * 94, hipMemcpyHostToDevice));
    HIP_TRY(c, hipMemcpy(c->d_term, term, 2 * npos * 8, hipMemcpyHostToDevice));
    c->len5p = len5p; c->len3p = len3p;
    c->h_lut.assign(lut, lut + 2 * npos * 94);
    c->key0_plain = true;
    for (int sub = 0; sub < 2; sub++) {
        if (term[(size_t)sub * npos] != 0.0) c->key0_plain = false;
        for (int q = 0; q < 94; q++)
            if (lut[((size_t)sub * npos) * 94 + q] != (uint8_t)q) c->key0_plain = false;
    }
    const size_t sub_bytes = (size_t)(756 + 2 * npos * 94) * 8;
    HIP_TRY(c, hipMalloc((void **)&c->d_subs, sub_bytes));
    HIP_TRY(c, hipMemset(c->d_subs, 0, sub_bytes));
    return MDX_OK;
}

int64_t mdx_rescale_summary_words(const mdx_ctx *c) {
    return (c && c->d_subs) ? 756 + 2 * (int64_t)(1 + c->len5p + c->len3p) * 94 : 0;
}

int mdx_rescale_summary(mdx_ctx *c, uint64_t *words) {
    if (!c || !words) return MDX_ERR_ARG;
    if (!c->d_subs) return fail(c, MDX_ERR_STATE, "rescale_set_model first");
    HIP_TRY(c, hipSetDevice(c->cfg.device));
    HIP_TRY(c, hipStreamSynchronize(c->stream));
    const int64_t nw = mdx_rescale_summary_words(c);
    HIP_TRY(c, hipMemcpy(words, c->d_subs, (size_t)nw * 8, hipMemcpyDeviceToHost));
    const int64_t npos = 1 + (int64_t)c->len5p + c->len3p;
    for (int t4 = 0; t4 < 4; t4++) {
        uint64_t *before = words + 4 + (t4 * 2 + 0) * 94, *after = words + 4 + (t4 * 2 + 1) * 94;
        if (t4 & 1) {
            for (int q = 0; q < 94; q++) after[q] = before[q];
            continue;
        }
        for (int q = 0; q < 94; q++) before[q] = after[q] = 0;
        const int sub = t4 >> 1;
        for (int64_t key = 0; key < npos; key++)
            for (int q = 0; q < 94; q++) {
                const uint64_t n = words[756 + (sub * npos + key) * 94 + q];
                if (!n) continue;
                before[q] += n;
                const uint8_t nq = c->h_lut[(size_t)((sub * npos + key) * 94 + q)];
                after[nq < 94 ? nq : 93] += n;
            }
    }
    return MDX_OK;
}

struct RsOut { uint8_t *qual_out; uint64_t *patch; int64_t patch_cap; int32_t parts; uint64_t *n_patch; };
static bool parts_ok(int32_t n) { return n >= 1 && n <= 65535 && (n & (n - 1)) == 0; }

static int rescale_device_impl(mdx_ctx *c, const mdx_batch *b_in, const int32_t *d_mtid, const int32_t *d_mpos, const RsOut &o,
                               double *d_mr_raw, uint8_t *d_status, bool zero_count) {
    uint8_t *const d_qual_out = o.qual_out;
    int rc = check_batch(c, b_in);
    if (rc != MDX_OK) return rc;
    mdx_batch b_ascii;
    rc = ascii_view(c, b_in, &b_ascii);
    if (rc != MDX_OK) return rc;
    const mdx_batch *b = &b_ascii;
    if (!c->d_ref || !c->d_lut) return fail(c, MDX_ERR_STATE, "set_reference and rescale_set_model first");
    if (!b->qual || !d_mtid || !d_mpos || !d_mr_raw || !d_status) return fail(c, MDX_ERR_ARG, "null column");
    if (o.patch ? (!o.n_patch || o.patch_cap < 0 || !parts_ok(o.parts) || d_qual_out) : !d_qual_out) return fail(c, MDX_ERR_ARG, "null column");
    if (d_qual_out == b->qual) return fail(c, MDX_ERR_ARG, "qual_out must not be the batch's own quality column");
    if (b->n_bases > 0xFFFF0000LL) return fail(c, MDX_ERR_ARG, "batch exceeds 32-bit offsets; split it");
    if (b->n_reads == 0) return MDX_OK;
    HIP_TRY(c, hipSetDevice(c->cfg.device));
    MdxRescaleArgs a{};
    a.n_reads = b->n_reads; a.n_bases = b->n_bases; a.flag = b->flag; a.tid = b->tid; a.pos = b->pos; a.mtid = d_mtid; a.mpos = d_mpos;
    a.cigar_off = b->cigar_off; a.cigar = b->cigar; a.seq_off = b->seq_off; a.seq = b->seq; a.qual = b->qual;
    a.ref = c->d_ref + 256; a.contig_off = c->d_contig_off; a.n_contig = c->n_contig;
    a.lut = c->d_lut; a.term = c->d_term; a.len5p = c->len5p; a.len3p = c->len3p; a.key0_plain = c->key0_plain ? 1 : 0;
    a.qual_out = d_qual_out; a.mr_raw = d_mr_raw; a.status = d_status; a.err = c->d_err; a.subs = c->d_subs;
    a.patch = (unsigned long long *)o.patch; a.n_patch = (unsigned long long *)o.n_patch; a.patch_cap = o.patch_cap; a.patch_parts = o.parts;
    if (o.patch && zero_count) HIP_TRY(c, hipMemsetAsync(o.n_patch, 0, (size_t)o.parts * 8, c->stream));
    HIP_TRY(c, c->rs_part.reserve(mdx_k_rescale_part_bytes(c->len5p, c->len3p, c->n_cu)));
    a.subs_part = (uint32_t *)c->rs_part.p;
    int64_t list_waves = 0, list_cap = 0;
    mdx_k_rescale_lists(b->n_reads, c->n_cu, &list_waves, &list_cap);
    HIP_TRY(c, c->rs_lists.reserve((size_t)list_waves * (size_t)(list_cap + 1) * 4));
    a.gen_count = (uint32_t *)c->rs_lists.p;
    a.gen_list = a.gen_count + list_waves;
    a.gen_cap = list_cap;
    hipEvent_t e0 = nullptr, e1 = nullptr;
    if (c->timing && hipEventCreate(&e0) == hipSuccess && hipEventCreate(&e1) == hipSuccess)
        (void)hipEventRecord(e0, c->stream);
    mdx_k_rescale(a, c->n_cu, c->stream);
    if (e0 && e1) {
        (void)hipEventRecord(e1, c->stream);
        c->rs_events.emplace_back(e0, e1);
    }
    HIP_TRY(c, hipGetLastError());
    return MDX_OK;
}

int mdx_rescale_device(mdx_ctx *c, const mdx_batch *b_in, const int32_t *d_mtid, const int32_t *d_mpos, uint8_t *d_qual_out,
                       double *d_mr_raw, uint8_t *d_status) {
    if (!d_qual_out) return fail(c, MDX_ERR_ARG, "null column");
    return rescale_device_impl(c, b_in, d_mtid, d_mpos, RsOut{d_qual_out, nullptr, 0, 0, nullptr}, d_mr_raw, d_status, true);
}

int mdx_rescale_patches_device(mdx_ctx *c, const mdx_batch *b_in, const int32_t *d_mtid, const int32_t *d_mpos, uint64_t *d_patch,
                               int64_t patch_cap, int32_t n_parts, uint64_t *d_n_patch, double *d_mr_raw, uint8_t *d_status) {
    if (!d_patch || !d_n_patch || patch_cap < 0 || !parts_ok(n_parts)) return fail(c, MDX_ERR_ARG, "patch list: null, or n_parts not a power of two");
    return rescale_device_impl(c, b_in, d_mtid, d_mpos, RsOut{nullptr, d_patch, patch_cap, n_parts, d_n_patch}, d_mr_raw, d_status, true);
}

int mdx_rescale_expand_device(mdx_ctx *c, const mdx_batch *b, const uint64_t *d_patch, int64_t patch_cap, int32_t n_parts,
                              const uint64_t *d_n_patch, uint8_t *d_qual_out) {
    int rc = check_batch(c, b);
    if (rc != MDX_OK) return rc;
    if (!b->qual || !d_patch || !d_n_patch || !d_qual_out || patch_cap < 0 || !parts_ok(n_parts)) return fail(c, MDX_ERR_ARG, "null column");
    HIP_TRY(c, hipSetDevice(c->cfg.device));
    mdx_k_rescale_expand(b->qual, d_qual_out, b->n_bases, (const unsigned long long *)d_patch, (const unsigned long long *)d_n_patch, patch_cap, n_parts, c->stream);
    HIP_TRY(c, hipGetLastError());
    return MDX_OK;
}

static bool fuse_applies(const mdx_ctx *c, const mdx_batch *b, bool packed_form = false) {
    const char *env = getenv("MDX_NO_FUSE");
    const bool off = env && *env && *env != '0';
    if (off || c->mode != MDX_MODE_LDS || c->lib_group != c->cfg.nlib || !c->dims.fast_ok()) return false;
    { const char *e = getenv("MDX_FORCE_REF64"); if (e && *e && *e != '0') return false; }
    if (c->cfg.minqual > 0 || !(c->ref_len + 1024 < (int64_t)0xFFFFFFFFLL)) return false;
    const int npos = 1 + c->len5p + c->len3p;
    if (!c->key0_plain || npos > 32 || !c->d_subs) return false;
    if (packed_form) {
        static const bool no_packed = [] { const char *e = getenv("MDX_NO_PACKED"); return e && *e && *e != '0'; }();
        static const bool no_pkf = [] { const char *e = getenv("MDX_NO_PACKED_FUSE"); return e && *e && *e != '0'; }();
        if (no_packed || no_pkf || c->cfg.nlib != 1 || mdx_k_pkf_lds_bytes(c->dims, npos) > kLdsLimit) return false;
        return b->n_reads > 0 && b->n_bases <= 0xFFFF0000LL;
    }
    if (mdx_k_fuse_lds_bytes(c->dims, npos, 64) > kLdsLimit) return false;
    if ((size_t)mdx_k_fuse_tcb_off(c->dims, 160) * 4 + (size_t)c->dims.nlib * c->dims.w_tc * 4 > ((size_t)1 << 18)) return false;
    return b->n_reads > 0 && b->n_bases <= 0xFFFF0000LL;
}

static int tabulate_rescale_impl(mdx_ctx *c, const mdx_batch *b_in, const int32_t *d_mtid, const int32_t *d_mpos,
                                 const RsOut &o, double *d_mr_raw, uint8_t *d_status) {
    uint8_t *const d_qual_out = o.qual_out;
    int rc = check_batch(c, b_in);
    if (rc != MDX_OK) return rc;
    if (c->n_groups > 0) return fail(c, MDX_ERR_ARG, "the fused tabulate-and-rescale calls count one library: not on a context with mdx_set_strata");
    const bool args_ok = c->d_ref && c->d_lut && b_in->qual && d_mtid && d_mpos && d_mr_raw && d_status &&
                         (o.patch ? (o.n_patch != nullptr && !d_qual_out && parts_ok(o.parts))
                                  : (d_qual_out && d_qual_out != b_in->qual && (((uintptr_t)d_qual_out ^ (uintptr_t)b_in->qual) & 15) == 0));
    if (o.patch && o.n_patch && parts_ok(o.parts)) HIP_TRY(c, hipMemsetAsync(o.n_patch, 0, (size_t)o.parts * 8, c->stream));
    const bool pkf = args_ok && b_in->seq_format == MDX_SEQ_4BIT && b_in->n_bases > 0 && fuse_applies(c, b_in, true);
    mdx_batch b_ascii;
    if (pkf) {
        b_ascii = *b_in;
        HIP_TRY(c, c->unpacked.reserve((size_t)b_in->n_bases + 64));
        b_ascii.seq = (const uint8_t *)c->unpacked.p;
        b_ascii.seq_format = MDX_SEQ_ASCII;
    } else {
        rc = ascii_view(c, b_in, &b_ascii);
        if (rc != MDX_OK) return rc;
    }
    const mdx_batch *b = &b_ascii;
    if (!pkf && (!args_ok || !fuse_applies(c, b))) {
        rc = mdx_tabulate_device(c, b_in);
        if (rc != MDX_OK) return rc;
        return rescale_device_impl(c, b, d_mtid, d_mpos, o, d_mr_raw, d_status, false);
    }
    HIP_TRY(c, hipSetDevice(c->cfg.device));
    const int npos = 1 + c->len5p + c->len3p, n_cnt = 752 + 2 * npos * 94;
    MdxFuse f{};
    f.mtid = d_mtid; f.mpos = d_mpos; f.qual_out = d_qual_out; f.mr_raw = d_mr_raw; f.status = d_status;
    f.patch = (unsigned long long *)o.patch; f.n_patch = (unsigned long long *)o.n_patch; f.patch_cap = o.patch_cap; f.patch_parts = o.parts;
    f.lut = c->d_lut; f.term = c->d_term; f.len5p = c->len5p; f.len3p = c->len3p;
    HIP_TRY(c, c->rs_part.reserve(mdx_k_rescale_part_bytes(c->len5p, c->len3p, c->n_cu) + (size_t)c->n_cu * n_cnt * 4));
    f.subs_part = (uint32_t *)c->rs_part.p;
    int fgrid = 0;
    rc = tabulate_impl(c, pkf ? b_in : b, &f, &fgrid);
    if (rc != MDX_OK) return rc;
    MdxRescaleArgs a{};
// ... 50 lines not shown
    HIP_TRY(c, hipSetDevice(c->cfg.device));
    mdx_batch dv;
    rc = mdx_batch_upload(c, h, &dv);
    if (rc != MDX_OK) return rc;
    const int64_t n = h->n_reads;
    int32_t *d_mtid = nullptr, *d_mpos = nullptr;
    uint8_t *d_qout = nullptr, *d_status = nullptr;
    double *d_mr = nullptr;
    hipError_t e = hipMalloc((void **)&d_mtid, (size_t)n * 4);
    if (e == hipSuccess) e = hipMalloc((void **)&d_mpos, (size_t)n * 4);
    if (e == hipSuccess) e = hipMalloc((void **)&d_qout, (size_t)h->n_bases + 64);
    if (e == hipSuccess) e = hipMalloc((void **)&d_status, (size_t)n);
    if (e == hipSuccess) e = hipMalloc((void **)&d_mr, (size_t)n * 8);
    if (e == hipSuccess) e = hipMemcpyAsync(d_mtid, mtid, (size_t)n * 4, hipMemcpyHostToDevice, c->stream);
    if (e == hipSuccess) e = hipMemcpyAsync(d_mpos, mpos, (size_t)n * 4, hipMemcpyHostToDevice, c->stream);
    if (e == hipSuccess) {
        rc = mdx_rescale_device(c, &dv, d_mtid, d_mpos, d_qout, d_mr, d_status);
        if (rc != MDX_OK) e = hipErrorUnknown;
    }
    if (e == hipSuccess) e = hipStreamSynchronize(c->stream);
    if (e == hipSuccess) e = hipMemcpy(qual_out, d_qout, (size_t)h->n_bases, hipMemcpyDeviceToHost);
    if (e == hipSuccess) e = hipMemcpy(mr_raw, d_mr, (size_t)n * 8, hipMemcpyDeviceToHost);
    if (e == hipSuccess) e = hipMemcpy(status, d_status, (size_t)n, hipMemcpyDeviceToHost);
    void *tmp[] = {d_mtid, d_mpos, d_qout, d_status, d_mr};
    for (void *p : tmp) if (p) (void)hipFree(p);
    (void)mdx_batch_free(c, &dv);
    if (rc != MDX_OK) return rc;
    if (e != hipSuccess) return fail(c, MDX_ERR_HIP, hipGetErrorString(e));
    return mdx_sync(c, nullptr);
}

int64_t mdx_fused_launches(const mdx_ctx *c) { return c ? c->n_fused : -1; }
int64_t mdx_packed_launches(const mdx_ctx *c) { return c ? c->n_packed : -1; }
int64_t mdx_geo_spec_launches(const mdx_ctx *c) { return c ? c->n_geo_spec : -1; }
int64_t mdx_libsorts(const mdx_ctx *c) { return c ? c->n_libsorts : -1; }
int mdx_last_launch_geometry(const mdx_ctx *c, int32_t out[4]) {
    if (!c || !out) return MDX_ERR_ARG;
    for (int i = 0; i < 4; i++) out[i] = c->last_geom[i];
    return MDX_OK;
}

int mdx_rescale_timing_read(mdx_ctx *c, int64_t *n_launches, double *total_ms) {
    if (!c) return MDX_ERR_ARG;
    HIP_TRY(c, hipStreamSynchronize(c->stream));
    double tot = 0;
    int64_t n = 0;
    for (auto &ev : c->rs_events) {
        float ms = 0;
        if (hipEventElapsedTime(&ms, ev.first, ev.second) == hipSuccess) { tot += ms; n++; }
        (void)hipEventDestroy(ev.first);
        (void)hipEventDestroy(ev.second);
    }
    c->rs_events.clear();
    if (n_launches) *n_launches = n;
    if (total_ms) *total_ms = tot;
    return MDX_OK;
}

int mdx_genome_composition(mdx_ctx *c, uint64_t *counts) {
    if (!c || !counts) return MDX_ERR_ARG;
    if (!c->d_ref) return fail(c, MDX_ERR_STATE, "mdx_set_reference has not been called");
    HIP_TRY(c, hipSetDevice(c->cfg.device));
    unsigned long long *d_out = nullptr;
    const size_t bytes = (size_t)c->n_contig * 4 * 8;
    HIP_TRY(c, hipMalloc((void **)&d_out, bytes));
    hipError_t e = hipMemsetAsync(d_out, 0, bytes, c->stream);
    if (e == hipSuccess) {
        mdx_k_genome_comp(c->d_ref + 256, c->d_contig_off, c->n_contig, d_out, c->stream);
        e = hipGetLastError();
    }
    if (e == hipSuccess) e = hipStreamSynchronize(c->stream);
    if (e == hipSuccess) e = hipMemcpy(counts, d_out, bytes, hipMemcpyDeviceToHost);
    (void)hipFree(d_out);
    if (e != hipSuccess) return fail(c, MDX_ERR_HIP, hipGetErrorString(e));
    return MDX_OK;
}

}
```

mapdamage_amd/csrc/mdx_internal.h:

```cpp
#pragma once

#include <hip/hip_runtime.h>
#include <stdint.h>

#include <string>
#include <vector>

struct MdxDims {
    int L, A, nlib, lgd_max, lgd_lds;
    int nl8;
    int G, R;
    int nl16, G4, H4;
    int t_pad;
    int w_mis, w_cmp, w_mc, w_tc, w_dmp, w_lgd, w_lib;
    int64_t w_total;
    __host__ __device__ int off_tc() const { return 0; }
    __host__ __device__ int off_mis() const { return w_tc; }
    __host__ __device__ int off_cmp() const { return w_tc + w_mis; }
    __host__ __device__ int off_dmp() const { return w_tc + w_mc; }
    __host__ __device__ int off_lgd() const { return w_tc + w_mc + w_dmp; }
    __host__ __device__ int tau_left(int p) const { const int b = p + A; return 64 * (b & 7) + (b >> 3); }
    __host__ __device__ int tau_right(int p) const { const int e = p + A; return 64 * (7 - (e & 7)) + nl8 + (e >> 3); }
    __host__ __device__ int tau_lflank(int dist) const {
        if (nl8 == 0) return dist - 1;
// ... 244 lines not shown
    int n_contig;
    const uint8_t *lut;
    const double *term;
    int len5p, len3p;
    int key0_plain;
    int lds_tables;
    uint8_t *qual_out;
    unsigned long long *patch, *n_patch;
    long long patch_cap;
    int patch_parts;
    double *mr_raw;
    uint8_t *status;
    unsigned long long *err;
    unsigned long long *subs;
    uint32_t *subs_part;
    uint32_t *gen_list;
    uint32_t *gen_count;
    int64_t gen_cap;
    const uint32_t *in_list, *in_count;
    int64_t in_cap;
    int n_in;
    int row_base;
    int copy_qual;
};
void mdx_k_rescale(const MdxRescaleArgs &a, int n_cu, hipStream_t s);
void mdx_k_rescale_expand(const uint8_t *qual, uint8_t *qual_out, int64_t n_bases, const unsigned long long *patch,
                          const unsigned long long *n_patch, long long patch_cap, int patch_parts, hipStream_t s);
void mdx_k_rescale_lists_pass(const MdxRescaleArgs &a, int fused_rows, int n_cu, hipStream_t s);
size_t mdx_k_rescale_part_bytes(int len5p, int len3p, int n_cu);
void mdx_k_rescale_lists(int64_t n_reads, int n_cu, int64_t *n_waves, int64_t *cap);

struct mdx_ctx;
extern "C" int mdx_ctx_minqual(const mdx_ctx *c);
extern "C" void mdx_ctx_scratch_give(mdx_ctx *c, void *arena, size_t cap, void *tables, void *stream, void *event);
extern "C" void mdx_ctx_scratch_take(mdx_ctx *c, void **arena, size_t *cap, void **tables, void **stream, void **event);

#include "mdx_filter.h"

struct MdxGbamCols {
    uint16_t *flag, *lib;
    int32_t *tid, *pos, *tlen, *mtid, *mpos;
    uint32_t *cigar_off, *cigar, *seq_off;
    uint8_t *seq, *qual;
    int seq_packed;
    const uint8_t *rg_names;
    const uint32_t *rg_off;
    const int32_t *lib_of_rg;
    int n_rg, lib_default;
    int minqual;
    uint32_t *counters;
    int fold;
    MdxFilterArgs filter;
};
size_t mdx_k_gbam_inflate_lds();
hipError_t mdx_k_gbam_prepare();
void mdx_k_gbam_inflate(const uint8_t *comp, const uint4 *blk, int n_blocks, uint8_t *unc, int *status, hipStream_t s);
void mdx_k_gbam_crc(const uint8_t *unc, const uint4 *blk, const uint32_t *want, const void *tables, int n_blocks, int *bad, hipStream_t s);
void mdx_k_gbam_scan(const uint8_t *unc, const uint4 *blk, const int *status, int n_blocks, int first, const int *forced,
                     uint32_t start0, uint32_t total, int n_ref, uint4 *info, uint4 *cnt, hipStream_t s);
void mdx_k_gbam_unpack(const uint8_t *unc, const uint4 *pre, const uint4 *cnt, int n_blocks, uint32_t n_rec, uint32_t n_cig,
                       uint32_t n_seq, uint32_t *rec_off, const MdxGbamCols &c, hipStream_t s);

int mdx_fasta_to_device(const char *fasta_path, int32_t n_contig, const char *const *names, int missing_ok, int64_t *lengths,
                        std::vector<int64_t> &contig_off, std::string &err, hipStream_t stream,
                        uint8_t *(*alloc_out)(void *, int64_t), void *alloc_arg);

// ... 65 lines not shown
```

mapdamage_amd/csrc/mdx_samio.cpp:

```cpp
#include "../../include/mdx.h"
#include "mdx_internal.h"
#include "mdx_crc32.h"

#include <zlib.h>

#include <algorithm>
#include <cstdio>
#include <cstdlib>
#include <cstring>
#include <mutex>
#include <string>
#include <thread>
#include <unordered_set>
#include <vector>

namespace {

struct DBuf {
    void *p = nullptr;
    size_t cap = 0;
};

bool reserve(DBuf &b, size_t bytes) {
    if (bytes <= b.cap) return true;
// ... 127 lines not shown
    MdxGsamNames refs{}, rgs{};
    struct Slot {
        bool ready = false, last = false, used = false;
        int rc = MDX_OK;
        std::string err;
        size_t start = 0, len = 0, next = 0;
        int64_t chunk = 0;
        std::vector<int64_t> coff;
        std::vector<uint32_t> uoff;
        uint32_t ulen = 0, gap = 0, skip = 0, tail = 0, tail_out = 0, tail_from = 0;
        int64_t tail_at[2] = {0, 0};
        bool no_lines = false;
        DBuf comp, stat;
        std::vector<int> hstat;
        uint8_t *pin = nullptr;
        size_t pin_cap = 0;
        DBuf txt;
        hipEvent_t ev_copied = nullptr, ev_used = nullptr;
    } slot[2];
    int cur = 0;
    DBuf nl, tab, blk, part, line_end, cnt, ldata, status, flag, lib, tid, pos_c, tlen, cigar_off, cigar, seq_off, seq, qual;
    bool bgzf = false;
    size_t first_block = 0;
    uint32_t skip0 = 0;
    int64_t tell[2] = {0, 0};
    void *d_crc_tables = nullptr;

    int stage(Slot &s, size_t start, int64_t chunk);
    int stage_bgzf(Slot &s, size_t start, int64_t chunk);
    int bgzf_header(std::string &text);
    int carry(Slot &s, Slot *nx);
    int parse(Slot &s, mdx_batch *view);
    bool drain() {
        bool ok = hipStreamSynchronize(copy_stream) == hipSuccess;
        return hipStreamSynchronize(stream) == hipSuccess && ok;
    }
};

int mdx_gsam::stage(Slot &s, size_t start, int64_t chunk) {
    if (bgzf) return stage_bgzf(s, start, chunk);
    s.ready = false; s.rc = MDX_OK; s.err.clear();
    s.start = start; s.chunk = chunk; s.last = false;
    size_t want = chunk < 65536 ? 65536 : (size_t)chunk;
    const uint8_t *base = nullptr;
    size_t body = 0;
    bool add_nl = false;
    for (;;) {
        size_t have = 0;
        base = mdx_source_bytes(src, start + want + 1, &have);
        if (have <= start) { s.len = 0; s.next = start; s.last = true; s.ready = true; return MDX_OK; }
        if (have <= start + want) {
            body = have - start;
            add_nl = base[have - 1] != '\n';
            s.last = true;
            break;
        }
        const void *nlp = memrchr(base + start, '\n', want);
        if (nlp) { body = (size_t)((const uint8_t *)nlp - (base + start)) + 1; break; }
        if (want >= ((size_t)1 << 30)) { s.rc = MDX_ERR_UNSUPPORTED; s.err = "a SAM line of more than a gigabyte"; return s.rc; }
        want *= 2;
    }
    s.len = body + (add_nl ? 1 : 0);
    s.next = start + body;
    if (s.len > 0xF0000000ull) { s.rc = MDX_ERR_UNSUPPORTED; s.err = "a slab of more than 3.75 GB"; return s.rc; }
    const size_t room = (s.len + 31) / 32 * 32 + 64;
    if (s.used && hipEventSynchronize(s.ev_copied) != hipSuccess) { s.rc = MDX_ERR_HIP; s.err = "HIP event failed"; return s.rc; }
    if (s.pin_cap < room) {
// ... 379 lines not shown
        if (out && *out) (*out)->error = std::string("mdx_gsam_open: ") + e.what();
        return MDX_ERR_ARG;
    } catch (...) {
        return MDX_ERR_ARG;
    }
}

int mdx_gsam_open(mdx_ctx *ctx, const char *path, mdx_gsam **out) {
    if (!ctx || !path || !out) return MDX_ERR_ARG;
    *out = nullptr;
    mdx_source *src = nullptr;
    if (mdx_source_open(path, &src) != MDX_OK) {
        mdx_gsam *g = new (std::nothrow) mdx_gsam();
        if (g) { g->ctx = ctx; g->error = src ? mdx_source_error(src) : "cannot open"; *out = g; }
        mdx_source_close(src);
        return MDX_ERR_ARG;
    }
    const int rc = mdx_gsam_open_source(ctx, src, out);
    mdx_source_close(src);
    return rc;
}

const mdx_bam *mdx_gsam_header(const mdx_gsam *g) { return g ? g->head : nullptr; }
const char *mdx_gsam_error(const mdx_gsam *g) { return g ? g->error.c_str() : "null handle"; }

int mdx_gsam_configure(mdx_gsam *g, int32_t n_rg, const char *const *rg_ids, const int32_t *lib_of_rg, int32_t lib_default, int want_qual) {
    try {
        if (!g || n_rg < 0 || (n_rg > 0 && (!rg_ids || !lib_of_rg))) return MDX_ERR_ARG;
        std::vector<std::string> ids;
        std::vector<int32_t> libs;
        for (int i = 0; i < n_rg; i++) { ids.emplace_back(rg_ids[i]); libs.push_back(lib_of_rg[i]); }
        g->lib_default = lib_default;
        g->want_qual = want_qual != 0;
        if (hipSetDevice(g->device) != hipSuccess) return MDX_ERR_HIP;
        if (!upload_names(ids, libs, g->d_rgs, g->rgs)) { g->error = "upload of the read-group tables failed"; return MDX_ERR_HIP; }
        return MDX_OK;
    } catch (...) {
        return MDX_ERR_ARG;
    }
}

int mdx_gsam_set_seq_format(mdx_gsam *g, int32_t seq_format) {
    if (!g || (seq_format != MDX_SEQ_ASCII && seq_format != MDX_SEQ_4BIT)) return MDX_ERR_ARG;
    g->seq_format = seq_format;
    return MDX_OK;
}

int mdx_gsam_set_min_basequal(mdx_gsam *g, int32_t minqual) {
    if (!g || minqual < 0 || minqual > 93) return MDX_ERR_ARG;
    if (minqual != 0 && minqual != mdx_ctx_minqual(g->ctx)) {
        g->error = "mdx_gsam_set_min_basequal: " + std::to_string(minqual) + " is not the --min-basequal of the context the file was opened on (" +
                   std::to_string(mdx_ctx_minqual(g->ctx)) + ")";
        return MDX_ERR_ARG;
    }
    g->minqual = minqual;
    return MDX_OK;
}

int mdx_gsam_next(mdx_gsam *g, int64_t chunk_bytes, mdx_batch *view) {
    try {
        if (!g || !view || !g->head || !g->copy_stream) return MDX_ERR_ARG;
        std::memset(view, 0, sizeof(*view));
        g->view_reads = 0;
        if (g->ended) return MDX_OK;
        if (hipSetDevice(g->device) != hipSuccess) return MDX_ERR_HIP;
        for (;;) {
            mdx_source_release_to(g->src, g->bgzf ? (size_t)g->tell[0] : g->pos);
            mdx_gsam::Slot &s = g->slot[g->cur], &nx = g->slot[g->cur ^ 1];
            bool anew = false;
            if (!(s.ready && s.start == g->pos && s.chunk == chunk_bytes)) { g->stage(s, g->pos, chunk_bytes); anew = true; }
            if (s.rc != MDX_OK) { g->error = s.err; s.ready = false; (void)g->drain(); return s.rc; }
            if (g->bgzf && anew && g->pos != g->first_block && (g->tell[0] != (int64_t)g->pos || g->tell[1] != 0)) {
                g->error = "the slab at compressed offset " + std::to_string(g->pos) + " was staged twice: the line it starts within is the host's";
                s.ready = false; (void)g->drain();
                return MDX_ERR_UNSUPPORTED;
            }
            if (!g->bgzf && s.len == 0) { g->ended = true; s.ready = false; return MDX_OK; }
            std::thread helper;
            if (!s.last && !(nx.ready && nx.start == s.next && nx.chunk == chunk_bytes)) {
                const int device = g->device;
                const size_t next = s.next;
                helper = std::thread([g, &nx, device, next, chunk_bytes] {
                    if (hipSetDevice(device) != hipSuccess) { nx.rc = MDX_ERR_HIP; nx.ready = false; return; }
                    g->stage(nx, next, chunk_bytes);
                });
            }
            int rc = g->parse(s, view);
            if (helper.joinable()) helper.join();
            if (nx.rc != MDX_OK) nx.ready = false;
            s.ready = false;
            if (rc == MDX_OK && g->bgzf) rc = g->carry(s, (!s.last && nx.ready) ? &nx : nullptr);
            if (rc == MDX_OK && hipEventRecord(s.ev_used, g->stream) != hipSuccess) { g->error = "GPU SAM decode: HIP event failed"; rc = MDX_ERR_HIP; }
            if (rc != MDX_OK) {
                std::memset(view, 0, sizeof(*view));
                g->view_reads = 0;
                (void)g->drain();
                nx.ready = false;
                return rc;
// ... 2 lines not shown
            g->ended = s.last;
            g->cur ^= 1;
            if (g->bgzf && s.no_lines && !s.last) continue;
            return MDX_OK;
        }
    } catch (const std::exception &e) {
        if (g) g->error = std::string("mdx_gsam_next: ") + e.what();
        return MDX_ERR_ARG;
    } catch (...) {
        return MDX_ERR_ARG;
    }
}

int mdx_gsam_at_end(const mdx_gsam *g) { return (!g || g->ended) ? 1 : 0; }

int mdx_gsam_is_bgzf(const mdx_gsam *g) { return (g && g->bgzf) ? 1 : 0; }

int mdx_gsam_tell_bgzf(const mdx_gsam *g, int64_t *comp_off, int64_t *phase) {
    if (!g || !comp_off || !phase || !g->head || !g->bgzf) return MDX_ERR_ARG;
    *comp_off = g->tell[0];
    *phase = g->tell[1];
    return MDX_OK;
}

int mdx_gsam_tell(const mdx_gsam *g, int64_t *offset) {
    if (!g || !offset || !g->head || g->bgzf) return MDX_ERR_ARG;
    *offset = (int64_t)g->pos;
    return MDX_OK;
}

int mdx_gsam_view_flags(mdx_gsam *g, uint16_t *flags, int64_t n) {
    if (!g || n < 0 || n != g->view_reads || (n > 0 && !flags)) return MDX_ERR_ARG;
    if (n == 0) return MDX_OK;
    if (hipSetDevice(g->device) != hipSuccess) return MDX_ERR_HIP;
    if (hipMemcpyAsync(flags, g->flag.p, (size_t)n * 2, hipMemcpyDeviceToHost, g->stream) != hipSuccess ||
        hipStreamSynchronize(g->stream) != hipSuccess) { g->error = "copy of the flag column failed"; return MDX_ERR_HIP; }
    return MDX_OK;
}

int mdx_gsam_view_set_flags(mdx_gsam *g, const uint16_t *flags, int64_t n) {
    if (!g || n < 0 || n != g->view_reads || (n > 0 && !flags)) return MDX_ERR_ARG;
    if (n == 0) return MDX_OK;
    if (hipSetDevice(g->device) != hipSuccess) return MDX_ERR_HIP;
    if (hipMemcpyAsync(g->flag.p, flags, (size_t)n * 2, hipMemcpyHostToDevice, g->stream) != hipSuccess ||
        hipStreamSynchronize(g->stream) != hipSuccess) { g->error = "copy of the flag column failed"; return MDX_ERR_HIP; }
    return MDX_OK;
}

int mdx_gsam_missing_qualities(const mdx_gsam *g) { return (g && g->no_qual_seen) ? 1 : 0; }

int mdx_gsam_set_record_filter(mdx_gsam *g, const mdx_record_filter *f) {
    if (!g) return MDX_ERR_ARG;
    if (!mdx_record_filter_valid(f)) {
        g->error = "mdx_gsam_set_record_filter: a value out of range (MAPQ 0..255, flags 0..65535, lengths >= 0, min <= max)";
        return MDX_ERR_ARG;
    }
    if (g->began) { g->error = "mdx_gsam_set_record_filter: behind the first mdx_gsam_next"; return MDX_ERR_STATE; }
    g->filter_on = mdx_record_filter_active(f);
    g->filter = g->filter_on ? *f : mdx_record_filter{};
    return MDX_OK;
}

int mdx_gsam_filter_counts(const mdx_gsam *g, uint64_t out[6]) {
    if (!g || !out) return MDX_ERR_ARG;
    for (int k = 0; k < 6; k++) out[k] = g->filter_counts[k];
    return MDX_OK;
}

void mdx_gsam_close(mdx_gsam *g) {
    if (!g) return;
    (void)hipSetDevice(g->device);
    if (g->copy_stream) (void)g->drain();
    for (auto &s : g->slot) {
        if (s.pin) (void)hipHostFree(s.pin);
        release(s.txt); release(s.comp); release(s.stat);
        if (s.ev_copied) (void)hipEventDestroy(s.ev_copied);
// ... 14 lines not shown
```

mapdamage_amd/engine.py:

```python

import ctypes
import os
import pathlib

import numpy as np

from . import layout as L
from .batch import ReadBatch, Reference
from .tables import TableSet

_HERE = pathlib.Path(__file__).resolve().parent
_LIBPATH = _HERE / "libmdx.so"
_lib = None

EXPORTS = (
    "mdx_abi_version", "mdx_strerror", "mdx_create", "mdx_destroy", "mdx_last_error",
    "mdx_set_stream", "mdx_set_reference", "mdx_batch_upload", "mdx_batch_free",
    "mdx_tabulate_host", "mdx_tabulate_device", "mdx_sync", "mdx_table_words",
    "mdx_finish_device", "mdx_finish", "mdx_reset", "mdx_timing_enable", "mdx_timing_read",
    "mdx_table_mode", "mdx_genome_composition", "mdx_rescale_set_model", "mdx_rescale_host",
    "mdx_rescale_summary_words", "mdx_rescale_summary",
    "mdx_comm_unique_id", "mdx_comm_init", "mdx_comm_adopt", "mdx_comm_size", "mdx_finish_allreduce",
    "mdx_rescale_device", "mdx_tabulate_rescale_device", "mdx_rescale_timing_read", "mdx_fused_launches",
    "mdx_bam_read", "mdx_bam_free", "mdx_bam_error", "mdx_bam_header_text", "mdx_bam_n_ref", "mdx_bam_ref_name",
    "mdx_bam_ref_length", "mdx_bam_batch", "mdx_bam_n_rg", "mdx_bam_rg_name", "mdx_bam_qnames",
    "mdx_bam_open", "mdx_bam_stream_header", "mdx_bam_next", "mdx_bam_close",
    "mdx_bam_stream_keep_raw", "mdx_bam_raw", "mdx_bam_patch_rescaled", "mdx_bam_qmin",
    "mdx_ctx_stream", "mdx_gbam_open", "mdx_gbam_header", "mdx_gbam_error", "mdx_gbam_configure", "mdx_gbam_next",
    "mdx_gbam_at_end", "mdx_gbam_close", "mdx_gbam_set_min_basequal", "mdx_gbam_missing_qualities",
    "mdx_gbam_inflate_blocks", "mdx_set_record_base", "mdx_pack_seq", "mdx_gbam_set_seq_format", "mdx_packed_launches", "mdx_geo_spec_launches",
    "mdx_gbam_skip", "mdx_comm_count", "mdx_gbam_tell", "mdx_gbam_fixups", "mdx_bam_seek", "mdx_libsorts",
    "mdx_gbam_view_flags", "mdx_gbam_view_set_flags",
    "mdx_rescale_patches_device", "mdx_tabulate_rescale_patches_device", "mdx_rescale_expand_device", "mdx_mr_round", "mdx_batch_fold", "mdx_bgzf_deflate",
    "mdx_gbam_rescale_slab", "mdx_gbam_write_rescaled", "mdx_gbam_record_name",
    "mdx_fasta_index", "mdx_set_reference_fasta", "mdx_fasta_load_stats", "mdx_reference_fetch", "mdx_host_threads", "mdx_host_pool_threads", "mdx_warm",
    "mdx_source_open", "mdx_source_error", "mdx_source_is_stream", "mdx_source_peek", "mdx_source_read", "mdx_source_close",
    "mdx_bam_read_source", "mdx_bam_open_source", "mdx_gbam_open_source",
    "mdx_source_seek", "mdx_gsam_open", "mdx_gsam_open_source", "mdx_gsam_header", "mdx_gsam_error", "mdx_gsam_configure",
    "mdx_gsam_set_seq_format", "mdx_gsam_set_min_basequal", "mdx_gsam_next", "mdx_gsam_at_end", "mdx_gsam_tell",
    "mdx_gsam_view_flags", "mdx_gsam_view_set_flags", "mdx_gsam_missing_qualities", "mdx_gsam_close",
    "mdx_gsam_is_bgzf", "mdx_gsam_tell_bgzf",
    "mdx_last_launch_geometry",
    "mdx_set_strata", "mdx_set_strata_regions", "mdx_strata_groups", "mdx_strata_kept", "mdx_merged_words", "mdx_finish_merged", "mdx_finish_merged_host", "mdx_lgd_copies",
    "mdx_stats_loglik", "mdx_stats_run", "mdx_stats_pmat",
    "mdx_bam_apply_record_filter", "mdx_gbam_set_record_filter", "mdx_gbam_filter_counts", "mdx_gsam_set_record_filter",
    "mdx_gsam_filter_counts",
)

SEQ_ASCII, SEQ_4BIT, SEQ_4BITQ = 0, 1, 2


class MdxConfig(ctypes.Structure):
    _fields_ = [("length", ctypes.c_int32), ("around", ctypes.c_int32),
                ("minqual", ctypes.c_int32), ("nlib", ctypes.c_int32),
                ("lgd_max", ctypes.c_int32), ("device", ctypes.c_int32),
                ("lgd_over_cap", ctypes.c_int64)]


class MdxBatch(ctypes.Structure):
    _fields_ = [("n_reads", ctypes.c_int64), ("n_cigar", ctypes.c_int64),
                ("n_bases", ctypes.c_int64),
                ("flag", ctypes.c_void_p), ("lib", ctypes.c_void_p), ("tid", ctypes.c_void_p),
                ("pos", ctypes.c_void_p), ("tlen", ctypes.c_void_p),
# ... 21 lines not shown
def load_library(path=None):
    global _lib
    if _lib is not None and path is None:
        return _lib
    p = pathlib.Path(path) if path else pathlib.Path(os.environ.get("MDX_LIBPATH") or _LIBPATH)
    if not p.exists():
        raise RuntimeError("%s is missing: build it with `python -m mapdamage_amd.build` "
                           "(hipcc, gfx950); there is no CPU fallback" % p)
    lib = ctypes.CDLL(str(p))
    lib.mdx_strerror.restype = ctypes.c_char_p
    lib.mdx_last_error.restype = ctypes.c_char_p
    lib.mdx_last_error.argtypes = [ctypes.c_void_p]
    lib.mdx_table_words.restype = ctypes.c_int64
    lib.mdx_table_words.argtypes = [ctypes.c_void_p]
    lib.mdx_destroy.restype = None
    lib.mdx_destroy.argtypes = [ctypes.c_void_p]
    for name in ("mdx_set_stream", "mdx_set_reference", "mdx_batch_upload", "mdx_batch_free",
                 "mdx_tabulate_host", "mdx_tabulate_device", "mdx_sync", "mdx_finish_device",
                 "mdx_finish", "mdx_reset", "mdx_timing_enable", "mdx_timing_read",
                 "mdx_table_mode", "mdx_genome_composition", "mdx_rescale_set_model", "mdx_rescale_host",
                 "mdx_rescale_summary", "mdx_comm_unique_id", "mdx_comm_init", "mdx_comm_adopt", "mdx_comm_size",
                 "mdx_finish_allreduce", "mdx_rescale_device", "mdx_tabulate_rescale_device", "mdx_rescale_timing_read",
                 "mdx_set_record_base"):
        getattr(lib, name).restype = ctypes.c_int
    lib.mdx_comm_size.argtypes = [ctypes.c_void_p]
    lib.mdx_comm_count.argtypes = [ctypes.c_void_p]
    lib.mdx_comm_adopt.argtypes = [ctypes.c_void_p, ctypes.c_void_p, ctypes.c_int32, ctypes.c_int32]
    lib.mdx_rescale_summary_words.restype = ctypes.c_int64
    lib.mdx_rescale_summary_words.argtypes = [ctypes.c_void_p]
    lib.mdx_fused_launches.restype = ctypes.c_int64
    lib.mdx_fused_launches.argtypes = [ctypes.c_void_p]
    lib.mdx_packed_launches.restype = ctypes.c_int64
    lib.mdx_packed_launches.argtypes = [ctypes.c_void_p]
    lib.mdx_geo_spec_launches.restype = ctypes.c_int64
    lib.mdx_geo_spec_launches.argtypes = [ctypes.c_void_p]
    lib.mdx_libsorts.restype = ctypes.c_int64
    lib.mdx_libsorts.argtypes = [ctypes.c_void_p]
    lib.mdx_last_launch_geometry.restype = ctypes.c_int
    lib.mdx_last_launch_geometry.argtypes = [ctypes.c_void_p, ctypes.c_void_p]
    for name in ("mdx_bam_error", "mdx_bam_header_text", "mdx_bam_ref_name", "mdx_bam_rg_name"):
        getattr(lib, name).restype = ctypes.c_char_p
    lib.mdx_bam_qnames.restype = ctypes.c_void_p
    lib.mdx_bam_qmin.restype = ctypes.c_void_p
    lib.mdx_bam_qmin.argtypes = [ctypes.c_void_p]
    lib.mdx_bam_ref_length.restype = ctypes.c_int64
    lib.mdx_bam_free.restype = None
    for name in ("mdx_bam_error", "mdx_bam_header_text", "mdx_bam_n_ref", "mdx_bam_n_rg", "mdx_bam_free"):
        getattr(lib, name).argtypes = [ctypes.c_void_p]
    for name in ("mdx_bam_ref_name", "mdx_bam_ref_length", "mdx_bam_rg_name"):
        getattr(lib, name).argtypes = [ctypes.c_void_p, ctypes.c_int32]
    lib.mdx_bam_stream_header.restype = ctypes.c_void_p
    lib.mdx_bam_stream_header.argtypes = [ctypes.c_void_p]
    lib.mdx_bam_next.argtypes = [ctypes.c_void_p, ctypes.c_int64, ctypes.c_void_p]
    lib.mdx_bam_close.restype = None
    lib.mdx_bam_close.argtypes = [ctypes.c_void_p]
    lib.mdx_gbam_open.argtypes = [ctypes.c_void_p, ctypes.c_char_p, ctypes.c_void_p]
    lib.mdx_gbam_header.restype = ctypes.c_void_p
    lib.mdx_gbam_header.argtypes = [ctypes.c_void_p]
    lib.mdx_gbam_error.restype = ctypes.c_char_p
    lib.mdx_gbam_error.argtypes = [ctypes.c_void_p]
    lib.mdx_gbam_configure.argtypes = [ctypes.c_void_p, ctypes.c_int32, ctypes.c_void_p, ctypes.c_void_p, ctypes.c_int32,
                                       ctypes.c_int, ctypes.c_int]
    lib.mdx_gbam_next.argtypes = [ctypes.c_void_p, ctypes.c_int64, ctypes.c_void_p, ctypes.c_void_p, ctypes.c_void_p]
    lib.mdx_gbam_at_end.argtypes = [ctypes.c_void_p]
    lib.mdx_gbam_skip.argtypes = [ctypes.c_void_p, ctypes.c_int64]
    lib.mdx_gbam_tell.argtypes = [ctypes.c_void_p, ctypes.c_void_p, ctypes.c_void_p]
# ... 377 lines not shown
                                        _ptr(mr), _ptr(status))
        if rc == L.MDX_ERR_BAD_READ:
            self.sync()
        self._check(rc)
        return qual_out, mr, status

    def rescale_device(self, dbatch, d_mtid, d_mpos, d_qual_out, d_mr, d_status, with_tables=False):
        fn = self._lib.mdx_tabulate_rescale_device if with_tables else self._lib.mdx_rescale_device
        self._set_record_base(0)
        self._check(fn(self._ctx, ctypes.byref(dbatch.dev), ctypes.c_void_p(d_mtid), ctypes.c_void_p(d_mpos),
                       ctypes.c_void_p(d_qual_out), ctypes.c_void_p(d_mr), ctypes.c_void_p(d_status)))

    def rescale_patches(self, dbatch, d_mtid, d_mpos, d_patch, patch_cap, n_parts, d_n_patch, d_mr, d_status, with_tables=False):
        fn = self._lib.mdx_tabulate_rescale_patches_device if with_tables else self._lib.mdx_rescale_patches_device
        fn.restype = ctypes.c_int
        dev = dbatch.dev if isinstance(dbatch, DeviceBatch) else dbatch
        self._set_record_base(0)
        self._check(fn(self._ctx, ctypes.byref(dev), ctypes.c_void_p(d_mtid), ctypes.c_void_p(d_mpos), ctypes.c_void_p(d_patch),
                       ctypes.c_int64(patch_cap), ctypes.c_int32(n_parts), ctypes.c_void_p(d_n_patch), ctypes.c_void_p(d_mr),
                       ctypes.c_void_p(d_status)))

    def rescale_expand(self, dbatch, d_patch, patch_cap, n_parts, d_n_patch, d_qual_out):
        dev = dbatch.dev if isinstance(dbatch, DeviceBatch) else dbatch
        self._lib.mdx_rescale_expand_device.restype = ctypes.c_int
        self._check(self._lib.mdx_rescale_expand_device(self._ctx, ctypes.byref(dev), ctypes.c_void_p(d_patch), ctypes.c_int64(patch_cap),
                                                        ctypes.c_int32(n_parts), ctypes.c_void_p(d_n_patch), ctypes.c_void_p(d_qual_out)))

    def fused_launches(self):
        return int(self._lib.mdx_fused_launches(self._ctx))

    def packed_launches(self):
        return int(self._lib.mdx_packed_launches(self._ctx))

    def geo_spec_launches(self):
        return int(self._lib.mdx_geo_spec_launches(self._ctx))

    def libsorts(self):
        return int(self._lib.mdx_libsorts(self._ctx))

    def last_launch_geometry(self):
        out = np.zeros(4, np.int32)
        self._check(self._lib.mdx_last_launch_geometry(self._ctx, _ptr(out)))
        return dict(zip(("grid", "waves_per_block", "tiles", "pools"), (int(x) for x in out)))

    def rescale_timing_read(self):
        n = ctypes.c_int64(0)
        ms = ctypes.c_double(0)
        self._check(self._lib.mdx_rescale_timing_read(self._ctx, ctypes.byref(n), ctypes.byref(ms)))
        return n.value, ms.value

    def rescale_summary(self):
        n = int(self._lib.mdx_rescale_summary_words(self._ctx))
        words = np.zeros(n, np.uint64)
        self._check(self._lib.mdx_rescale_summary(self._ctx, _ptr(words)))
        return words

    def reset(self):
        self._check(self._lib.mdx_reset(self._ctx))

    def timing(self, enable=True):
        self._check(self._lib.mdx_timing_enable(self._ctx, 1 if enable else 0))

    def timing_read(self):
        n = ctypes.c_int64(0)
        ms = ctypes.c_double(0)
        self._check(self._lib.mdx_timing_read(self._ctx, ctypes.byref(n), ctypes.byref(ms)))
# ... 2 lines not shown
```

Baseline: 27.32 billion.

## Overlap consecutive tabulate launches on side streams with rotating partial buffers

Consecutive packed single-library tabulate launches can now run concurrently. Alternate launches go to a second stream, and a high-priority reduction stream is created. Each overlapped launch gets its own double-buffered wave lists and one of four rotating sets of partials and tile counters, guarded by events. Every other entry point now joins the outstanding side-stream work first. This targets idle GPU time between back-to-back batch kernels, in exchange for more device memory, more event and stream bookkeeping, and a risk of ordering bugs.

Result: faster. 27.73 billion (median of 6 runs) (+1.5%).

```diff
diff --git a/include/mdx.h b/include/mdx.h
--- a/include/mdx.h
+++ b/include/mdx.h
@@ -141,6 +141,7 @@
 int mdx_rescale_timing_read(mdx_ctx *ctx, int64_t *n_launches, double *total_ms);
 int64_t mdx_fused_launches(const mdx_ctx *ctx);
 int64_t mdx_packed_launches(const mdx_ctx *ctx);
+int64_t mdx_overlapped_launches(const mdx_ctx *ctx);
 int64_t mdx_geo_spec_launches(const mdx_ctx *ctx);
 int64_t mdx_libsorts(const mdx_ctx *ctx);
 int mdx_last_launch_geometry(const mdx_ctx *ctx, int32_t out[4]);
diff --git a/mapdamage_amd/csrc/mdx_bamio.cpp b/mapdamage_amd/csrc/mdx_bamio.cpp
--- a/mapdamage_amd/csrc/mdx_bamio.cpp
+++ b/mapdamage_amd/csrc/mdx_bamio.cpp
@@ -1419,7 +1419,8 @@
         return true;
     }
     bool drain() {
-        bool ok = true;
+        bool ok = hipSetDevice(device) == hipSuccess;
+        if (ctx) ok = mdx_ctx_join(ctx) == MDX_OK && ok;
         if (infl_stream) ok = hipStreamSynchronize(infl_stream) == hipSuccess && ok;
         if (copy_stream) ok = hipStreamSynchronize(copy_stream) == hipSuccess && ok;
         if (stream) ok = hipStreamSynchronize(stream) == hipSuccess && ok;
@@ -1524,7 +1525,7 @@
         }
         g->lib_default = lib_default;
         g->want_qual = want_qual != 0; g->want_mate = want_mate != 0;
-        if (hipSetDevice(g->device) != hipSuccess) return MDX_ERR_HIP;
+        if (hipSetDevice(g->device) != hipSuccess || (g->ctx && mdx_ctx_join(g->ctx) != MDX_OK)) return MDX_ERR_HIP;
         g->d_rg_names = g->d_rg_off = g->d_lib_of_rg = nullptr;
         if (n_rg > 0) {
             const size_t b_off = g->rg_off.size() * 4, b_lib = g->lib_of_rg.size() * 4, b_nm = g->rg_names.size() + 1;
@@ -2010,7 +2011,7 @@
             if (g->phase_known && g->phase != 0) { g->error = "truncated BAM file: the last record is incomplete"; return MDX_ERR_ARG; }
             return MDX_OK;
         }
-        if (hipSetDevice(g->device) != hipSuccess) return MDX_ERR_HIP;
+        if (hipSetDevice(g->device) != hipSuccess || (g->ctx && mdx_ctx_join(g->ctx) != MDX_OK)) return MDX_ERR_HIP;
         if (const char *fail = std::getenv("MDX_GBAM_FAIL_AT")) {
             if (g->slabs_done == std::atoi(fail)) { g->error = "MDX_GBAM_FAIL_AT"; return MDX_ERR_UNSUPPORTED; }
         }
@@ -2158,7 +2159,7 @@
 int mdx_gbam_view_flags(mdx_gbam *g, uint16_t *flags, int64_t n) {
     if (!g || n < 0 || n != g->view_reads || (n > 0 && !flags)) return MDX_ERR_ARG;
     if (n == 0) return MDX_OK;
-    if (hipSetDevice(g->device) != hipSuccess) return MDX_ERR_HIP;
+    if (hipSetDevice(g->device) != hipSuccess || (g->ctx && mdx_ctx_join(g->ctx) != MDX_OK)) return MDX_ERR_HIP;
     if (hipMemcpyAsync(flags, g->slab[g->view_slab].flag.p, (size_t)n * 2, hipMemcpyDeviceToHost, g->stream) != hipSuccess ||
         hipStreamSynchronize(g->stream) != hipSuccess) { g->error = "copy of the flag column failed"; return MDX_ERR_HIP; }
     return MDX_OK;
@@ -2167,7 +2168,7 @@
 int mdx_gbam_view_set_flags(mdx_gbam *g, const uint16_t *flags, int64_t n) {
     if (!g || n < 0 || n != g->view_reads || (n > 0 && !flags)) return MDX_ERR_ARG;
     if (n == 0) return MDX_OK;
-    if (hipSetDevice(g->device) != hipSuccess) return MDX_ERR_HIP;
+    if (hipSetDevice(g->device) != hipSuccess || (g->ctx && mdx_ctx_join(g->ctx) != MDX_OK)) return MDX_ERR_HIP;
     if (hipMemcpyAsync(g->slab[g->view_slab].flag.p, flags, (size_t)n * 2, hipMemcpyHostToDevice, g->stream) != hipSuccess ||
         hipStreamSynchronize(g->stream) != hipSuccess) { g->error = "copy of the flag column failed"; return MDX_ERR_HIP; }
     return MDX_OK;
@@ -2211,7 +2212,7 @@
     if (!g || !out) return MDX_ERR_ARG;
     unsigned long long dropped[5] = {0, 0, 0, 0, 0};
     if (g->d_filter_counts) {
-        if (hipSetDevice(g->device) != hipSuccess || hipStreamSynchronize(g->stream) != hipSuccess ||
+        if (hipSetDevice(g->device) != hipSuccess || (g->ctx && mdx_ctx_join(g->ctx) != MDX_OK) || hipStreamSynchronize(g->stream) != hipSuccess ||
             hipMemcpy(dropped, g->d_filter_counts, sizeof(dropped), hipMemcpyDeviceToHost) != hipSuccess) return MDX_ERR_HIP;
     }
     out[0] = g->records_read;
@@ -2350,7 +2351,7 @@
     if (n == 0) return MDX_OK;
     if (!mr || !rescaled) return MDX_ERR_ARG;
     try {
-        if (hipSetDevice(g->device) != hipSuccess) return MDX_ERR_HIP;
+        if (hipSetDevice(g->device) != hipSuccess || (g->ctx && mdx_ctx_join(g->ctx) != MDX_OK)) return MDX_ERR_HIP;
         hipStream_t st = g->stream;
         mdx_gbam::Slab &s = g->slab[g->view_slab];
         uint8_t *d_resc = nullptr, *d_stream = nullptr;
@@ -2401,7 +2402,7 @@
 int mdx_gbam_record_name(mdx_gbam *g, int64_t index, char *buf, int32_t cap) {
     if (!g || !buf || cap < 1 || index < 0 || index >= g->view_reads) return MDX_ERR_ARG;
     buf[0] = 0;
-    if (hipSetDevice(g->device) != hipSuccess) return MDX_ERR_HIP;
+    if (hipSetDevice(g->device) != hipSuccess || (g->ctx && mdx_ctx_join(g->ctx) != MDX_OK)) return MDX_ERR_HIP;
     mdx_gbam::Slab &s = g->slab[g->view_slab];
     uint32_t off = 0;
     uint8_t head[12];
@@ -2425,7 +2426,7 @@
         return MDX_ERR_STATE;
     }
     try {
-        if (hipSetDevice(g->device) != hipSuccess) return MDX_ERR_HIP;
+        if (hipSetDevice(g->device) != hipSuccess || (g->ctx && mdx_ctx_join(g->ctx) != MDX_OK)) return MDX_ERR_HIP;
         hipStream_t st = g->stream;
         const int parts = 256;
         const int64_t cap = std::max<int64_t>(4096, 8 * n / parts);
diff --git a/mapdamage_amd/csrc/mdx_capi.cpp b/mapdamage_amd/csrc/mdx_capi.cpp
--- a/mapdamage_amd/csrc/mdx_capi.cpp
+++ b/mapdamage_amd/csrc/mdx_capi.cpp
@@ -3,6 +3,7 @@
 
 #include <dlfcn.h>
 
+#include <algorithm>
 #include <chrono>
 
 #include <cstdio>
@@ -168,7 +169,26 @@
     std::vector<uint8_t> h_lut;
     bool key0_plain = false;
     int len5p = 0, len3p = 0;
+    static constexpr int kOvSets = 4;
+    bool overlap = true;
+    hipStream_t ov_stream = nullptr;
+    hipStream_t red_stream = nullptr;
+    DevBuf ov_lists;
+    uint32_t *ov_partials[kOvSets] = {nullptr, nullptr, nullptr, nullptr};
+    hipEvent_t ov_kernel_done[kOvSets] = {nullptr, nullptr, nullptr, nullptr};
+    hipEvent_t ov_set_free[kOvSets] = {nullptr, nullptr, nullptr, nullptr};
+    bool ov_set_used[kOvSets] = {false, false, false, false};
+    hipEvent_t ov_fork = nullptr;
+    bool ov_open = false;
+    bool ov_slot1_forked = false;
+    int ov_slot1_last = -1;
+    int ov_last_set = -1;
+    int64_t ov_turn = 0;
+    int64_t ov_set_turn = 0;
+    int64_t n_overlapped = 0;
     bool timing = false;
+    hipEvent_t t_base = nullptr;
+    bool t_side_by_side = false;
     std::vector<std::pair<hipEvent_t, hipEvent_t>> events;
     std::vector<std::pair<hipEvent_t, hipEvent_t>> rs_events;
     std::string err;
@@ -205,6 +225,37 @@
     HIP_TRY(c, hipMemsetAsync(c->d_n_lgd_over, 0, 8, c->stream));
     HIP_TRY(c, hipMemsetAsync(c->d_err, 0xFF, 8, c->stream));
     if (c->d_strata_kept) HIP_TRY(c, hipMemsetAsync(c->d_strata_kept, 0, (size_t)c->cfg.nlib * 8, c->stream));
+    return MDX_OK;
+}
+
+int join_launches(mdx_ctx *c) {
+    if (!c->ov_open) return MDX_OK;
+    if (c->ov_slot1_last >= 0) HIP_TRY(c, hipStreamWaitEvent(c->stream, c->ov_kernel_done[c->ov_slot1_last], 0));
+    if (c->ov_last_set >= 0) HIP_TRY(c, hipStreamWaitEvent(c->stream, c->ov_set_free[c->ov_last_set], 0));
+    c->ov_open = false;
+    c->ov_slot1_forked = false;
+    c->ov_turn = 0;
+    c->ov_slot1_last = c->ov_last_set = -1;
+    return MDX_OK;
+}
+
+#define JOIN_TRY(ctx)                              \
+    do {                                           \
+        const int rc_ = join_launches(ctx);        \
+        if (rc_ != MDX_OK) return rc_;             \
+    } while (0)
+
+int overlap_prepare(mdx_ctx *c, int set) {
+    if (!c->ov_stream) HIP_TRY(c, hipStreamCreateWithFlags(&c->ov_stream, hipStreamNonBlocking));
+    if (!c->red_stream) {
+        int lo = 0, hi = 0;
+        HIP_TRY(c, hipDeviceGetStreamPriorityRange(&lo, &hi));
+        HIP_TRY(c, hipStreamCreateWithPriority(&c->red_stream, hipStreamNonBlocking, hi));
+    }
+    if (!c->ov_fork) HIP_TRY(c, hipEventCreateWithFlags(&c->ov_fork, hipEventDisableTiming));
+    if (!c->ov_kernel_done[set]) HIP_TRY(c, hipEventCreateWithFlags(&c->ov_kernel_done[set], hipEventDisableTiming));
+    if (!c->ov_set_free[set]) HIP_TRY(c, hipEventCreateWithFlags(&c->ov_set_free[set], hipEventDisableTiming));
+    if (!c->ov_partials[set]) HIP_TRY(c, hipMalloc((void **)&c->ov_partials[set], (size_t)c->max_grid * c->dims.w_total * 4));
     return MDX_OK;
 }
 
@@ -286,6 +337,7 @@
     }
     HIP_TRY(c, hipStreamCreateWithFlags(&c->own_stream, hipStreamNonBlocking));
     c->stream = c->own_stream;
+    if (const char *e = getenv("MDX_NO_OVERLAP")) c->overlap = !(*e && *e != '0');
     lap("context, stream");
 
     const int lgd_lds = mdx_k_lgd_lds(cfg->length, cfg->around, cfg->lgd_max);
@@ -333,7 +385,18 @@
 void mdx_destroy(mdx_ctx *c) {
     if (!c) return;
     (void)hipSetDevice(c->cfg.device);
+    (void)join_launches(c);
     if (c->stream) (void)hipStreamSynchronize(c->stream);
+    if (c->ov_stream) { (void)hipStreamSynchronize(c->ov_stream); (void)hipStreamDestroy(c->ov_stream); }
+    if (c->red_stream) { (void)hipStreamSynchronize(c->red_stream); (void)hipStreamDestroy(c->red_stream); }
+    for (int i = 0; i < mdx_ctx::kOvSets; i++) {
+        if (c->ov_kernel_done[i]) (void)hipEventDestroy(c->ov_kernel_done[i]);
+        if (c->ov_set_free[i]) (void)hipEventDestroy(c->ov_set_free[i]);
+        if (c->ov_partials[i]) (void)hipFree(c->ov_partials[i]);
+    }
+    if (c->ov_fork) (void)hipEventDestroy(c->ov_fork);
+    if (c->t_base) (void)hipEventDestroy(c->t_base);
+    c->ov_lists.release();
     if (c->comm && c->comm_owned && rccl()) (void)rccl()->CommDestroy(c->comm);
     for (auto &ev : c->events) { (void)hipEventDestroy(ev.first); (void)hipEventDestroy(ev.second); }
     for (auto &ev : c->rs_events) { (void)hipEventDestroy(ev.first); (void)hipEventDestroy(ev.second); }
@@ -372,6 +435,8 @@
 
 int mdx_set_stream(mdx_ctx *c, void *hip_stream) {
     if (!c) return MDX_ERR_ARG;
+    HIP_TRY(c, hipSetDevice(c->cfg.device));
+    JOIN_TRY(c);
     HIP_TRY(c, hipStreamSynchronize(c->stream));
     c->stream = hip_stream ? (hipStream_t)hip_stream : c->own_stream;
     return MDX_OK;
@@ -380,6 +445,7 @@
 static const size_t kRefPad = 256;
 static int ref_begin(mdx_ctx *c, int64_t n, int32_t n_contig) {
     HIP_TRY(c, hipSetDevice(c->cfg.device));
+    JOIN_TRY(c);
     HIP_TRY(c, hipStreamSynchronize(c->stream));
     if (c->d_ref) { (void)hipFree(c->d_ref); c->d_ref = nullptr; }
     if (c->d_ref4) { (void)hipFree(c->d_ref4); c->d_ref4 = nullptr; }
@@ -437,6 +503,7 @@
     if (!c || !fasta_path || !names || n_contig < 1) return fail(c, MDX_ERR_ARG, "set_reference_fasta: bad arguments");
     try {
         HIP_TRY(c, hipSetDevice(c->cfg.device));
+        JOIN_TRY(c);
         struct Arg { mdx_ctx *c; int32_t n_contig; int rc; } arg{c, n_contig, MDX_OK};
         std::vector<int64_t> contig_off;
         std::string err;
@@ -536,6 +603,7 @@
     if (rc != MDX_OK) return rc;
     if (!dv) return MDX_ERR_ARG;
     HIP_TRY(c, hipSetDevice(c->cfg.device));
+    JOIN_TRY(c);
     std::memset(dv, 0, sizeof(*dv));
     dv->n_reads = h->n_reads; dv->n_cigar = h->n_cigar; dv->n_bases = h->n_bases;
     dv->seq_format = h->seq_format;
@@ -594,6 +662,7 @@
     if (b->libsort) return fail(c, MDX_ERR_ARG, "mdx_batch_fold: the batch brings mdx_batch::libsort, built from the column as it was");
     if (b->n_bases == 0) { b->seq_format = MDX_SEQ_4BITQ; return MDX_OK; }
     HIP_TRY(c, hipSetDevice(c->cfg.device));
+    JOIN_TRY(c);
     mdx_k_fold_mask(b->seq, const_cast<uint8_t *>(b->seq), b->qual, b->lowq, b->n_bases, c->cfg.minqual, c->stream);
     HIP_TRY(c, hipGetLastError());
     b->seq_format = MDX_SEQ_4BITQ;
@@ -602,6 +671,8 @@
 
 int mdx_batch_free(mdx_ctx *c, mdx_batch *dv) {
     if (!c || !dv) return MDX_ERR_ARG;
+    HIP_TRY(c, hipSetDevice(c->cfg.device));
+    JOIN_TRY(c);
     HIP_TRY(c, hipStreamSynchronize(c->stream));
     if (dv->libsort && dv->libsort == c->libsort_checked) c->libsort_checked = nullptr;
     const void *ptrs[] = {dv->flag, dv->lib, dv->tid, dv->pos, dv->tlen, dv->cigar_off,
@@ -628,6 +699,9 @@
     const bool pmask = packed && !fuse && want_mask;
     static const bool no_ml = [] { const char *e = getenv("MDX_NO_ML"); return e && *e && *e != '0'; }();
     const bool ml = packed && !fuse && c->cfg.nlib > 1 && !no_ml;
+    bool ov = c->overlap && c->stream == c->own_stream && packed && !pmask && !fuse && c->mode == MDX_MODE_LDS && c->cfg.nlib == 1 &&
+              c->n_groups == 0;
+    if (!ov) JOIN_TRY(c);
     mdx_batch b_key;
     if (c->n_groups > 0) {
         if (fuse) return fail(c, MDX_ERR_ARG, "the fused tabulate-and-rescale calls count one library: not on a context with mdx_set_strata");
@@ -695,6 +769,7 @@
         const int pools = (c->n_cu * per_cu) / 2;
         if (group > pools) group = pools > 0 ? pools : 1;
     }
+    int ov_slot = 0;
     for (int lo = 0; lo < c->cfg.nlib; lo += group) {
         const int gn = c->cfg.nlib - lo < group ? c->cfg.nlib - lo : group;
         a.lib_lo = lo;
@@ -756,23 +831,66 @@
             if (!c->d_tile_ctr) {
                 HIP_TRY(c, hipMalloc((void **)&c->d_tile_ctr, (size_t)MDX_CTR_WORDS * 4));
                 HIP_TRY(c, hipMemsetAsync(c->d_tile_ctr, 0, (size_t)MDX_CTR_WORDS * 4, c->stream));
+                c->tile_ctr_clean = true;
+            }
+            if (ov && (size_t)n_pools * MDX_CTR_PAD > (size_t)MDX_CTR_WORDS / 2 / mdx_ctx::kOvSets) {
+                JOIN_TRY(c);
+                ov = false;
             }
             if (n_pools * MDX_CTR_PAD > MDX_CTR_WORDS / 2 || n_pools * MDX_CTR_PAD > MDX_CTR_WORDS) return fail(c, MDX_ERR_STATE, "more blocks than tile counters");
             a.tile_ctr = c->d_tile_ctr;
             {
                 const size_t list_bytes = (size_t)nwaves * (size_t)MDX_WAVE_SCRATCH(a.ring_size) * 16;
-                if (c->lists.reserve(list_bytes) != hipSuccess)
+                if (ov && c->ov_open) {
+                    ov_slot = (int)(c->ov_turn & 1);
+                    const DevBuf &mine = ov_slot ? c->ov_lists : c->lists;
+                    if (mine.p && list_bytes > mine.cap) {
+                        JOIN_TRY(c);
+                        HIP_TRY(c, hipStreamSynchronize(c->stream));
+                        ov_slot = 0;
+                        if (c->ov_lists.p && c->ov_lists.reserve(list_bytes) != hipSuccess)
+                            return fail(c, MDX_ERR_HIP, "the per-wavefront lists of this launch (" + std::to_string(list_bytes >> 20) + " MiB, twice) could not be allocated");
+                    }
+                }
+                DevBuf &lists = ov_slot ? c->ov_lists : c->lists;
+                if (lists.reserve(list_bytes) != hipSuccess)
                     return fail(c, MDX_ERR_HIP, "the per-wavefront lists of this launch (" + std::to_string(list_bytes >> 20) + " MiB) could not be allocated" +
                                 (quota ? ": tabulate the batch in smaller pieces" : ""));
+                a.lists = (uint4 *)lists.p;
             }
-            a.lists = (uint4 *)c->lists.p;
             c->last_geom[0] = grid; c->last_geom[1] = wpb_l; c->last_geom[2] = (int32_t)n_tiles; c->last_geom[3] = (int32_t)n_pools;
+        }
+        hipStream_t ls = c->stream;
+        int ov_set = 0;
+        const size_t n_ctr = (size_t)mdx_n_pools((unsigned)grid);
+        const bool side = ov && c->ov_open;
+        if (ov && !side) {
+            c->ov_open = true;
+            c->ov_turn = 0;
+        }
+        if (side) {
+            ov_set = (int)(c->ov_set_turn % mdx_ctx::kOvSets);
+            rc = overlap_prepare(c, ov_set);
+            if (rc != MDX_OK) return rc;
+            if (ov_slot) {
+                ls = c->ov_stream;
+                if (!c->ov_slot1_forked) {
+                    HIP_TRY(c, hipEventRecord(c->ov_fork, c->stream));
+                    HIP_TRY(c, hipStreamWaitEvent(ls, c->ov_fork, 0));
+                }
+                c->ov_slot1_forked = true;
+            }
+            if (c->ov_set_used[ov_set]) HIP_TRY(c, hipStreamWaitEvent(ls, c->ov_set_free[ov_set], 0));
+            a.partials = c->ov_partials[ov_set];
+            a.tile_ctr = c->d_tile_ctr + MDX_CTR_WORDS / 2 + (size_t)ov_set * (MDX_CTR_WORDS / 2 / mdx_ctx::kOvSets);
+            c->n_overlapped++;
+            if (c->timing) c->t_side_by_side = true;
         }
         hipEvent_t e0 = nullptr, e1 = nullptr;
         if (c->timing) {
             HIP_TRY(c, hipEventCreate(&e0));
             HIP_TRY(c, hipEventCreate(&e1));
-            HIP_TRY(c, hipEventRecord(e0, c->stream));
+            HIP_TRY(c, hipEventRecord(e0, ls));
         }
         mdx_batch b_fold;
         const mdx_batch *bs = b;
@@ -826,9 +944,10 @@
             a.ml_plan = (const uint4 *)c->ml_partials.p;
             mdx_k_ml_plan(ls.lib_start, lo, gn, mdx_tile_records(a.dims, a.pfl_off != 0), grid, c->ml_partials.p, c->stream);
         }
-        const size_t n_ctr = (size_t)mdx_n_pools((unsigned)grid);
-        if (!c->tile_ctr_clean || n_ctr > 4096) HIP_TRY(c, hipMemsetAsync(c->d_tile_ctr, 0, n_ctr * MDX_CTR_PAD * 4, c->stream));
-        c->tile_ctr_clean = false;
+        if (!side) {
+            if (!c->tile_ctr_clean || n_ctr > 4096) HIP_TRY(c, hipMemsetAsync(c->d_tile_ctr, 0, n_ctr * MDX_CTR_PAD * 4, c->stream));
+            c->tile_ctr_clean = false;
+        }
         if (fuse) {
             HIP_TRY(c, hipMemsetAsync(fuse->mr_raw, 0xFF, (size_t)b->n_reads * 8, c->stream));
             const int64_t nwaves = (int64_t)grid * wpb_l;
@@ -841,17 +960,30 @@
             if (fused_grid) *fused_grid = grid;
         } else if (packed) {
             if (pmask) mdx_k_tabulate_packed_masked(a, grid, c->pk.threads, lds, c->stream);
-            else if (mdx_k_tabulate_packed(a, grid, c->pk.threads, lds, c->stream)) c->n_geo_spec++;
+            else if (mdx_k_tabulate_packed(a, grid, c->pk.threads, lds, ls)) c->n_geo_spec++;
             c->n_packed++;
         } else {
             mdx_k_tabulate(a, c->mode, mask, grid, lds, c->stream);
         }
         if (c->timing) {
-            HIP_TRY(c, hipEventRecord(e1, c->stream));
+            HIP_TRY(c, hipEventRecord(e1, ls));
             c->events.emplace_back(e0, e1);
         }
         HIP_TRY(c, hipGetLastError());
-        if (c->mode == MDX_MODE_LDS) {
+        if (side) {
+            HIP_TRY(c, hipEventRecord(c->ov_kernel_done[ov_set], ls));
+            HIP_TRY(c, hipStreamWaitEvent(c->red_stream, c->ov_kernel_done[ov_set], 0));
+            mdx_k_reduce_partials(a.partials, a.raw, c->d_raw + c->dims.w_total - 1, a.dims.w_total, grid, c->red_stream, nullptr);
+            HIP_TRY(c, hipGetLastError());
+            HIP_TRY(c, hipMemsetAsync(a.tile_ctr, 0, n_ctr * MDX_CTR_PAD * 4, c->red_stream));
+            HIP_TRY(c, hipEventRecord(c->ov_set_free[ov_set], c->red_stream));
+            c->ov_set_used[ov_set] = true;
+            c->ov_last_set = ov_set;
+            if (ov_slot) c->ov_slot1_last = ov_set;
+            c->ov_turn++;
+            c->ov_set_turn++;
+        } else if (c->mode == MDX_MODE_LDS) {
+            if (ov) c->ov_turn++;
             if (ml) mdx_k_reduce_partials(c->d_partials, a.raw, c->d_raw + c->dims.w_total - 1, a.dims.w_total, grid, c->stream, c->d_tile_ctr, gn, c->dims.w_lib, a.ml_plan);
             else
             mdx_k_reduce_partials(c->d_partials, a.raw, c->d_raw + c->dims.w_total - 1, a.dims.w_total, grid, c->stream, c->d_tile_ctr);
@@ -869,6 +1001,7 @@
     if (rc != MDX_OK) return rc;
     if (h->n_reads == 0) return MDX_OK;
     HIP_TRY(c, hipSetDevice(c->cfg.device));
+    JOIN_TRY(c);
     const int64_t n = h->n_reads;
     const void *src[10] = {h->flag, h->lib, h->tid, h->pos, h->tlen, h->cigar_off, h->cigar, h->seq_off, h->seq, h->qual};
     const size_t bytes[10] = {(size_t)n * 2, (size_t)n * 2, (size_t)n * 4, (size_t)n * 4, (size_t)n * 4,
@@ -921,10 +1054,11 @@
     dv.cigar = (const uint32_t *)st[6].p; dv.seq_off = (const uint32_t *)st[7].p;
     dv.seq = (const uint8_t *)st[8].p; dv.qual = h->qual ? (const uint8_t *)st[9].p : nullptr;
     rc = mdx_tabulate_device(c, &dv);
+    const int jrc = join_launches(c);
     HIP_TRY(c, hipEventRecord(c->st_done[s], c->stream));
     c->st_busy[s] = true;
     c->st_turn = s ^ 1;
-    return rc;
+    return rc != MDX_OK ? rc : jrc;
 }
 
 int mdx_set_record_base(mdx_ctx *c, int64_t base) {
@@ -936,6 +1070,7 @@
 int mdx_sync(mdx_ctx *c, int64_t *bad_read) {
     if (!c) return MDX_ERR_ARG;
     HIP_TRY(c, hipSetDevice(c->cfg.device));
+    JOIN_TRY(c);
     HIP_TRY(c, hipStreamSynchronize(c->stream));
     unsigned long long err = 0, nover = 0;
     HIP_TRY(c, hipMemcpy(&err, c->d_err, 8, hipMemcpyDeviceToHost));
@@ -959,6 +1094,7 @@
 int mdx_finish_device(mdx_ctx *c, uint64_t *d_tables) {
     if (!c || !d_tables) return MDX_ERR_ARG;
     HIP_TRY(c, hipSetDevice(c->cfg.device));
+    JOIN_TRY(c);
     mdx_k_finalize(c->d_raw, c->d_lgd_dense, c->d_n_lgd_over, c->dims, c->lgd_copies, (unsigned long long *)d_tables, c->stream);
     HIP_TRY(c, hipGetLastError());
     return MDX_OK;
@@ -980,6 +1116,7 @@
     const Rccl *r = rccl();
     if (!r) return fail(c, MDX_ERR_COMM, g_rccl.err);
     HIP_TRY(c, hipSetDevice(c->cfg.device));
+    JOIN_TRY(c);
     RcclId u;
     std::memcpy(u.internal, id, MDX_COMM_ID_BYTES);
     void *comm = nullptr;
@@ -992,6 +1129,8 @@
     if (!c || !rccl_comm || nranks < 1 || rank < 0 || rank >= nranks) return fail(c, MDX_ERR_ARG, "comm_adopt: bad arguments");
     if (c->comm) return fail(c, MDX_ERR_STATE, "a communicator is already attached");
     if (!rccl()) return fail(c, MDX_ERR_COMM, g_rccl.err);
+    HIP_TRY(c, hipSetDevice(c->cfg.device));
+    JOIN_TRY(c);
     c->comm = rccl_comm; c->comm_owned = false; c->comm_size = nranks; c->comm_rank = rank;
     return MDX_OK;
 }
@@ -1118,6 +1257,7 @@
 int mdx_reset(mdx_ctx *c) {
     if (!c) return MDX_ERR_ARG;
     HIP_TRY(c, hipSetDevice(c->cfg.device));
+    JOIN_TRY(c);
     int rc = zero_accumulators(c);
     if (rc != MDX_OK) return rc;
     HIP_TRY(c, hipStreamSynchronize(c->stream));
@@ -1138,6 +1278,7 @@
     if (c->counted) return fail(c, MDX_ERR_STATE, "set_strata: records have been counted already (mdx_reset first)");
     if (c->d_regions) return fail(c, MDX_ERR_STATE, "set_strata: the context has region strata (mdx_set_strata_regions); a context has one kind");
     HIP_TRY(c, hipSetDevice(c->cfg.device));
+    JOIN_TRY(c);
     HIP_TRY(c, hipStreamSynchronize(c->stream));
     if (c->d_group_of_tid) { (void)hipFree(c->d_group_of_tid); c->d_group_of_tid = nullptr; }
     c->n_groups = 0;
@@ -1179,6 +1320,7 @@
     if (c->counted) return fail(c, MDX_ERR_STATE, "set_strata_regions: records have been counted already (mdx_reset first)");
     if (c->d_group_of_tid) return fail(c, MDX_ERR_STATE, "set_strata_regions: the context has tid strata (mdx_set_strata); a context has one kind");
     HIP_TRY(c, hipSetDevice(c->cfg.device));
+    JOIN_TRY(c);
     HIP_TRY(c, hipStreamSynchronize(c->stream));
     if (c->d_regions) { (void)hipFree(c->d_regions); c->d_regions = nullptr; }
     c->n_groups = 0;
@@ -1210,6 +1352,7 @@
     if (!c || !kept) return MDX_ERR_ARG;
     if (c->n_groups <= 0) return fail(c, MDX_ERR_STATE, "strata_kept: mdx_set_strata has not been called");
     HIP_TRY(c, hipSetDevice(c->cfg.device));
+    JOIN_TRY(c);
     HIP_TRY(c, hipStreamSynchronize(c->stream));
     HIP_TRY(c, hipMemcpy(kept, c->d_strata_kept, (size_t)c->cfg.nlib * 8, hipMemcpyDeviceToHost));
     return MDX_OK;
@@ -1244,6 +1387,7 @@
     if (!c || !d_tables || !d_merged) return MDX_ERR_ARG;
     if (d_tables == d_merged) return fail(c, MDX_ERR_ARG, "finish_merged: the merged block needs a buffer of its own");
     HIP_TRY(c, hipSetDevice(c->cfg.device));
+    JOIN_TRY(c);
     const int g = c->n_groups > 0 ? c->n_groups : 1;
     mdx_k_merge_strata((const unsigned long long *)d_tables, (unsigned long long *)d_merged, c->cfg.nlib / g, g,
                        (int64_t)4 * c->cfg.length * MDX_N_MIS_COLS, (int64_t)4 * (c->cfg.length + c->cfg.around) * 4,
@@ -1254,22 +1398,47 @@
 
 int mdx_timing_enable(mdx_ctx *c, int enable) {
     if (!c) return MDX_ERR_ARG;
+    if (enable && !c->timing) {
+        HIP_TRY(c, hipSetDevice(c->cfg.device));
+        JOIN_TRY(c);
+        if (!c->t_base) HIP_TRY(c, hipEventCreate(&c->t_base));
+        HIP_TRY(c, hipEventRecord(c->t_base, c->stream));
+    }
     c->timing = enable != 0;
     return MDX_OK;
 }
 
 int mdx_timing_read(mdx_ctx *c, int64_t *n_launches, double *total_ms) {
     if (!c) return MDX_ERR_ARG;
+    HIP_TRY(c, hipSetDevice(c->cfg.device));
+    JOIN_TRY(c);
     HIP_TRY(c, hipStreamSynchronize(c->stream));
     double tot = 0;
     int64_t n = 0;
+    const bool stamped = c->t_side_by_side && c->t_base;
+    std::vector<std::pair<double, double>> iv;
     for (auto &ev : c->events) {
-        float ms = 0;
-        if (hipEventElapsedTime(&ms, ev.first, ev.second) == hipSuccess) { tot += ms; n++; }
+        float ms = 0, t0 = 0;
+        if (hipEventElapsedTime(&ms, ev.first, ev.second) == hipSuccess) {
+            if (!stamped) tot += ms;
+            else if (hipEventElapsedTime(&t0, c->t_base, ev.first) == hipSuccess) iv.emplace_back((double)t0, (double)t0 + ms);
+            n++;
+        }
         (void)hipEventDestroy(ev.first);
         (void)hipEventDestroy(ev.second);
     }
+    if (stamped) {
+        std::sort(iv.begin(), iv.end());
+        double end = -1.0e300;
+        for (auto &x : iv) {
+            if (x.second <= end) continue;
+            tot += x.second - (x.first > end ? x.first : end);
+            end = x.second;
+        }
+    }
+    c->t_side_by_side = false;
     c->events.clear();
+    if (c->timing && c->t_base) HIP_TRY(c, hipEventRecord(c->t_base, c->stream));
     if (n_launches) *n_launches = n;
     if (total_ms) *total_ms = tot;
     return MDX_OK;
@@ -1304,6 +1473,8 @@
 
 int mdx_ctx_stream(mdx_ctx *c, void **stream, int *device) {
     if (!c) return MDX_ERR_ARG;
+    HIP_TRY(c, hipSetDevice(c->cfg.device));
+    JOIN_TRY(c);
     if (stream) *stream = (void *)c->stream;
     if (device) *device = c->cfg.device;
     return MDX_OK;
@@ -1312,6 +1483,7 @@
 int mdx_rescale_set_model(mdx_ctx *c, const uint8_t *lut, const double *term, int32_t len5p, int32_t len3p) {
     if (!c || !lut || !term || len5p < 0 || len3p < 0 || len5p + len3p > 100000) return fail(c, MDX_ERR_ARG, "rescale model");
     HIP_TRY(c, hipSetDevice(c->cfg.device));
+    JOIN_TRY(c);
     HIP_TRY(c, hipStreamSynchronize(c->stream));
     if (c->d_lut) { (void)hipFree(c->d_lut); c->d_lut = nullptr; }
     if (c->d_term) { (void)hipFree(c->d_term); c->d_term = nullptr; }
@@ -1343,6 +1515,7 @@
     if (!c || !words) return MDX_ERR_ARG;
     if (!c->d_subs) return fail(c, MDX_ERR_STATE, "rescale_set_model first");
     HIP_TRY(c, hipSetDevice(c->cfg.device));
+    JOIN_TRY(c);
     HIP_TRY(c, hipStreamSynchronize(c->stream));
     const int64_t nw = mdx_rescale_summary_words(c);
     HIP_TRY(c, hipMemcpy(words, c->d_subs, (size_t)nw * 8, hipMemcpyDeviceToHost));
@@ -1375,6 +1548,7 @@
     uint8_t *const d_qual_out = o.qual_out;
     int rc = check_batch(c, b_in);
     if (rc != MDX_OK) return rc;
+    JOIN_TRY(c);
     mdx_batch b_ascii;
     rc = ascii_view(c, b_in, &b_ascii);
     if (rc != MDX_OK) return rc;
@@ -1432,6 +1606,7 @@
     if (rc != MDX_OK) return rc;
     if (!b->qual || !d_patch || !d_n_patch || !d_qual_out || patch_cap < 0 || !parts_ok(n_parts)) return fail(c, MDX_ERR_ARG, "null column");
     HIP_TRY(c, hipSetDevice(c->cfg.device));
+    JOIN_TRY(c);
     mdx_k_rescale_expand(b->qual, d_qual_out, b->n_bases, (const unsigned long long *)d_patch, (const unsigned long long *)d_n_patch, patch_cap, n_parts, c->stream);
     HIP_TRY(c, hipGetLastError());
     return MDX_OK;
@@ -1462,6 +1637,7 @@
     int rc = check_batch(c, b_in);
     if (rc != MDX_OK) return rc;
     if (c->n_groups > 0) return fail(c, MDX_ERR_ARG, "the fused tabulate-and-rescale calls count one library: not on a context with mdx_set_strata");
+    JOIN_TRY(c);
     const bool args_ok = c->d_ref && c->d_lut && b_in->qual && d_mtid && d_mpos && d_mr_raw && d_status &&
                          (o.patch ? (o.n_patch != nullptr && !d_qual_out && parts_ok(o.parts))
                                   : (d_qual_out && d_qual_out != b_in->qual && (((uintptr_t)d_qual_out ^ (uintptr_t)b_in->qual) & 15) == 0));
@@ -1578,6 +1754,8 @@
 
 int64_t mdx_fused_launches(const mdx_ctx *c) { return c ? c->n_fused : -1; }
 int64_t mdx_packed_launches(const mdx_ctx *c) { return c ? c->n_packed : -1; }
+int64_t mdx_overlapped_launches(const mdx_ctx *c) { return c ? c->n_overlapped : -1; }
+int mdx_ctx_join(mdx_ctx *c) { return c ? join_launches(c) : MDX_ERR_ARG; }
 int64_t mdx_geo_spec_launches(const mdx_ctx *c) { return c ? c->n_geo_spec : -1; }
 int64_t mdx_libsorts(const mdx_ctx *c) { return c ? c->n_libsorts : -1; }
 int mdx_last_launch_geometry(const mdx_ctx *c, int32_t out[4]) {
@@ -1588,6 +1766,8 @@
 
 int mdx_rescale_timing_read(mdx_ctx *c, int64_t *n_launches, double *total_ms) {
     if (!c) return MDX_ERR_ARG;
+    HIP_TRY(c, hipSetDevice(c->cfg.device));
+    JOIN_TRY(c);
     HIP_TRY(c, hipStreamSynchronize(c->stream));
     double tot = 0;
     int64_t n = 0;
@@ -1607,6 +1787,7 @@
     if (!c || !counts) return MDX_ERR_ARG;
     if (!c->d_ref) return fail(c, MDX_ERR_STATE, "mdx_set_reference has not been called");
     HIP_TRY(c, hipSetDevice(c->cfg.device));
+    JOIN_TRY(c);
     unsigned long long *d_out = nullptr;
     const size_t bytes = (size_t)c->n_contig * 4 * 8;
     HIP_TRY(c, hipMalloc((void **)&d_out, bytes));
diff --git a/mapdamage_amd/csrc/mdx_internal.h b/mapdamage_amd/csrc/mdx_internal.h
--- a/mapdamage_amd/csrc/mdx_internal.h
+++ b/mapdamage_amd/csrc/mdx_internal.h
@@ -300,6 +300,7 @@
 
 struct mdx_ctx;
 extern "C" int mdx_ctx_minqual(const mdx_ctx *c);
+extern "C" int mdx_ctx_join(mdx_ctx *c);
 extern "C" void mdx_ctx_scratch_give(mdx_ctx *c, void *arena, size_t cap, void *tables, void *stream, void *event);
 extern "C" void mdx_ctx_scratch_take(mdx_ctx *c, void **arena, size_t *cap, void **tables, void **stream, void **event);
 
diff --git a/mapdamage_amd/csrc/mdx_samio.cpp b/mapdamage_amd/csrc/mdx_samio.cpp
--- a/mapdamage_amd/csrc/mdx_samio.cpp
+++ b/mapdamage_amd/csrc/mdx_samio.cpp
@@ -183,7 +183,9 @@
     int carry(Slot &s, Slot *nx);
     int parse(Slot &s, mdx_batch *view);
     bool drain() {
-        bool ok = hipStreamSynchronize(copy_stream) == hipSuccess;
+        bool ok = hipSetDevice(device) == hipSuccess;
+        ok = hipStreamSynchronize(copy_stream) == hipSuccess && ok;
+        if (ctx) ok = mdx_ctx_join(ctx) == MDX_OK && ok;
         return hipStreamSynchronize(stream) == hipSuccess && ok;
     }
 };
@@ -629,7 +631,7 @@
         for (int i = 0; i < n_rg; i++) { ids.emplace_back(rg_ids[i]); libs.push_back(lib_of_rg[i]); }
         g->lib_default = lib_default;
         g->want_qual = want_qual != 0;
-        if (hipSetDevice(g->device) != hipSuccess) return MDX_ERR_HIP;
+        if (hipSetDevice(g->device) != hipSuccess || (g->ctx && mdx_ctx_join(g->ctx) != MDX_OK)) return MDX_ERR_HIP;
         if (!upload_names(ids, libs, g->d_rgs, g->rgs)) { g->error = "upload of the read-group tables failed"; return MDX_ERR_HIP; }
         return MDX_OK;
     } catch (...) {
@@ -660,7 +662,7 @@
         std::memset(view, 0, sizeof(*view));
         g->view_reads = 0;
         if (g->ended) return MDX_OK;
-        if (hipSetDevice(g->device) != hipSuccess) return MDX_ERR_HIP;
+        if (hipSetDevice(g->device) != hipSuccess || (g->ctx && mdx_ctx_join(g->ctx) != MDX_OK)) return MDX_ERR_HIP;
         for (;;) {
             mdx_source_release_to(g->src, g->bgzf ? (size_t)g->tell[0] : g->pos);
             mdx_gsam::Slot &s = g->slot[g->cur], &nx = g->slot[g->cur ^ 1];
@@ -729,7 +731,7 @@
 int mdx_gsam_view_flags(mdx_gsam *g, uint16_t *flags, int64_t n) {
     if (!g || n < 0 || n != g->view_reads || (n > 0 && !flags)) return MDX_ERR_ARG;
     if (n == 0) return MDX_OK;
-    if (hipSetDevice(g->device) != hipSuccess) return MDX_ERR_HIP;
+    if (hipSetDevice(g->device) != hipSuccess || (g->ctx && mdx_ctx_join(g->ctx) != MDX_OK)) return MDX_ERR_HIP;
     if (hipMemcpyAsync(flags, g->flag.p, (size_t)n * 2, hipMemcpyDeviceToHost, g->stream) != hipSuccess ||
         hipStreamSynchronize(g->stream) != hipSuccess) { g->error = "copy of the flag column failed"; return MDX_ERR_HIP; }
     return MDX_OK;
@@ -738,7 +740,7 @@
 int mdx_gsam_view_set_flags(mdx_gsam *g, const uint16_t *flags, int64_t n) {
     if (!g || n < 0 || n != g->view_reads || (n > 0 && !flags)) return MDX_ERR_ARG;
     if (n == 0) return MDX_OK;
-    if (hipSetDevice(g->device) != hipSuccess) return MDX_ERR_HIP;
+    if (hipSetDevice(g->device) != hipSuccess || (g->ctx && mdx_ctx_join(g->ctx) != MDX_OK)) return MDX_ERR_HIP;
     if (hipMemcpyAsync(g->flag.p, flags, (size_t)n * 2, hipMemcpyHostToDevice, g->stream) != hipSuccess ||
         hipStreamSynchronize(g->stream) != hipSuccess) { g->error = "copy of the flag column failed"; return MDX_ERR_HIP; }
     return MDX_OK;
diff --git a/mapdamage_amd/engine.py b/mapdamage_amd/engine.py
--- a/mapdamage_amd/engine.py
+++ b/mapdamage_amd/engine.py
@@ -28,7 +28,7 @@
     "mdx_bam_stream_keep_raw", "mdx_bam_raw", "mdx_bam_patch_rescaled", "mdx_bam_qmin",
     "mdx_ctx_stream", "mdx_gbam_open", "mdx_gbam_header", "mdx_gbam_error", "mdx_gbam_configure", "mdx_gbam_next",
     "mdx_gbam_at_end", "mdx_gbam_close", "mdx_gbam_set_min_basequal", "mdx_gbam_missing_qualities",
-    "mdx_gbam_inflate_blocks", "mdx_set_record_base", "mdx_pack_seq", "mdx_gbam_set_seq_format", "mdx_packed_launches", "mdx_geo_spec_launches",
+    "mdx_gbam_inflate_blocks", "mdx_set_record_base", "mdx_pack_seq", "mdx_gbam_set_seq_format", "mdx_packed_launches", "mdx_overlapped_launches", "mdx_geo_spec_launches",
     "mdx_gbam_skip", "mdx_comm_count", "mdx_gbam_tell", "mdx_gbam_fixups", "mdx_bam_seek", "mdx_libsorts",
     "mdx_gbam_view_flags", "mdx_gbam_view_set_flags",
     "mdx_rescale_patches_device", "mdx_tabulate_rescale_patches_device", "mdx_rescale_expand_device", "mdx_mr_round", "mdx_batch_fold", "mdx_bgzf_deflate",
@@ -116,6 +116,8 @@
     lib.mdx_fused_launches.argtypes = [ctypes.c_void_p]
     lib.mdx_packed_launches.restype = ctypes.c_int64
     lib.mdx_packed_launches.argtypes = [ctypes.c_void_p]
+    lib.mdx_overlapped_launches.restype = ctypes.c_int64
+    lib.mdx_overlapped_launches.argtypes = [ctypes.c_void_p]
     lib.mdx_geo_spec_launches.restype = ctypes.c_int64
     lib.mdx_geo_spec_launches.argtypes = [ctypes.c_void_p]
     lib.mdx_libsorts.restype = ctypes.c_int64
@@ -559,6 +561,9 @@
     def packed_launches(self):
         return int(self._lib.mdx_packed_launches(self._ctx))
 
+    def overlapped_launches(self):
+        return int(self._lib.mdx_overlapped_launches(self._ctx))
+
     def geo_spec_launches(self):
         return int(self._lib.mdx_geo_spec_launches(self._ctx))
 
```
